# AILab-UniFI/GNN-TableExtraction

Hardware: AMD Instinct MI355X
Metric: nodes/sec (fwd+bwd node classification) on PubLayNet page graphs (higher is better)
Workload: dtype f32 (GEMM operands split exactly into 3 bf16 pieces, fp32 accumulate)

## Files before the change

### gnn-tableextraction_amd/_lib.py

```python
from __future__ import annotations

import ctypes
import os
from ctypes import POINTER, c_char_p, c_float, c_int, c_int64, c_uint64, c_void_p

_HERE = os.path.dirname(os.path.abspath(__file__))
LIB_PATH = os.environ.get("GTE_LIB_PATH") or os.path.join(_HERE, "libgte_hip.so")

SIGNATURES = {
    "gte_version": (c_int, []),
    "gte_last_error": (c_char_p, []),
    "gte_device_info": (c_int, [c_void_p, c_void_p, c_void_p, c_void_p, c_int]),
    "gte_spmm_csr": (c_int, [c_void_p, c_void_p, c_void_p, c_void_p, c_int64, c_void_p, c_int64,
                             c_int64, c_int64, c_int, c_int, c_void_p]),
    "gte_spmm_csr_accumulate": (c_int, [c_void_p, c_void_p, c_void_p, c_void_p, c_int64, c_void_p, c_int64,
                                        c_int64, c_int64, c_int, c_int, c_void_p]),
    "gte_spmm_csr_edge_workspace_bytes": (c_int64, [c_int64, c_int64]),
    "gte_spmm_csr_edge": (c_int, [c_void_p, c_void_p, c_void_p, c_void_p, c_int64, c_void_p, c_int64, c_int64, c_int64, c_int64, c_int,
                                  c_void_p, c_int64, c_void_p]),
    "gte_spmm_tile_rows": (c_int, []),
    "gte_spmm_csr_tiled": (c_int, [c_void_p, c_void_p, c_void_p, c_void_p, c_void_p, c_void_p, c_void_p, c_int64,
                                   c_void_p, c_int64, c_int64, c_int64, c_int, c_int, c_void_p]),
    "gte_coo_to_csr_workspace_bytes": (c_int64, [c_int64, c_int64]),
    "gte_coo_to_csr": (c_int, [c_void_p, c_void_p, c_void_p, c_void_p, c_int64, c_int64,
                               c_void_p, c_void_p, c_void_p, c_void_p, c_void_p, c_int64, c_void_p]),
    "gte_batch_csr": (c_int, [c_void_p, c_int64] + [c_void_p] * 10 + [c_int64, c_int64, c_void_p]),
    "gte_cast_bf16": (c_int, [c_void_p, c_int64, c_void_p, c_int64, c_int64, c_int64, c_int, c_void_p]),
    "gte_gemm_bf16_nt": (c_int, [c_void_p, c_int64, c_void_p, c_int64, c_void_p, c_int64, c_int64, c_int64, c_int64, c_void_p]),
    "gte_knn_max_k": (c_int, []),
    "gte_knn_max_page_nodes": (c_int, []),
    "gte_knn_select": (c_int, [c_void_p, c_void_p, c_void_p, c_int64, c_int64, c_int64, c_int, c_int, c_void_p, c_void_p]),
    "gte_visibility_select": (c_int, [c_void_p, c_void_p, c_void_p, c_int64, c_int64, c_int64, c_int, c_void_p, c_void_p]),
    "gte_knn_csr_workspace_bytes": (c_int64, [c_int64]),
    "gte_knn_csr": (c_int, [c_void_p, c_void_p, c_void_p, c_int64, c_int, c_int, c_int, c_void_p, c_void_p, c_void_p, c_void_p,
                            c_int64, c_void_p]),
    "gte_island_mask": (c_int, [c_void_p, c_void_p, c_void_p, c_int64, c_int, c_int, c_void_p, c_void_p, c_int64, c_void_p]),
    "gte_batch_assemble": (c_int, [c_void_p, c_int64, c_void_p, c_void_p, c_void_p, c_void_p, c_void_p, c_int64, c_int64,
                                   c_void_p, c_void_p, c_void_p, c_int64, c_void_p]),
    "gte_batch_assemble_rows": (c_int, [c_void_p, c_int64, c_void_p, c_void_p, c_void_p, c_void_p, c_void_p, c_int64, c_int64,
                                        c_void_p, c_void_p, c_void_p, c_int64, c_void_p, c_int64, c_int64, c_void_p]),
    "gte_batch_rows": (c_int, [c_void_p, c_int64, c_void_p, c_void_p, c_void_p, c_int64, c_void_p, c_int64, c_int64,
                               c_int64, c_void_p]),
    "gte_edge_weights_workspace_bytes": (c_int64, [c_int64, c_int64]),
    "gte_edge_weights_bbox": (c_int, [c_void_p, c_void_p, c_void_p, c_void_p, c_int64, c_int64, c_void_p, c_void_p,
                                      c_int64, c_void_p]),
    "gte_bbox_features": (c_int, [c_void_p, c_void_p, c_void_p, c_int64, c_int64, c_void_p]),
    "gte_inv_degree": (c_int, [c_void_p, c_void_p, c_int64, c_void_p]),
    "gte_sage_linear_fwd": (c_int, [c_void_p, c_int64, c_int64, c_void_p, c_int64, c_int64,
                                    c_void_p, c_int64, c_void_p, c_void_p, c_void_p, c_float, c_int,
                                    c_void_p, c_int64, c_void_p, c_void_p, c_int64, c_int64, c_int64, c_void_p]),
    "gte_sage_linear_fwd_fuses_ln": (c_int, [c_int64, c_int64]),
    "gte_sage_linear_fwd_p3": (c_int, [c_void_p, c_int64, c_int64, c_void_p, c_int64, c_int64,
                                       c_void_p, c_int64, c_void_p, c_void_p, c_void_p, c_float, c_int,
                                       c_void_p, c_int64, c_void_p, c_void_p, c_int64, c_void_p, c_int64, c_int64, c_int64, c_void_p]),
    "gte_sage_linear_dw_workspace_bytes": (c_int64, [c_int64, c_int64, c_int64, c_int64]),
    "gte_sage_linear_dw": (c_int, [c_void_p, c_int64, c_void_p, c_int64, c_int64, c_void_p, c_int64, c_int64, c_void_p,
                                   c_int64, c_int64, c_int64, c_void_p, c_int64, c_void_p]),
    "gte_spmm_csr_accumulate_ln_supported": (c_int, [c_int64]),
    "gte_spmm_csr_accumulate_ln": (c_int, [c_void_p, c_void_p, c_void_p, c_void_p, c_int64, c_void_p, c_int64, c_int64, c_int64,
                                           c_int, c_void_p, c_void_p, c_float, c_int, c_void_p, c_int64, c_void_p, c_void_p]),
    "gte_gemm_tail_workspace_bytes": (c_int64, []),
    "gte_gemm_set_tail_workspace": (c_int, [c_void_p, c_int64]),
    "gte_gemm_set_mode": (c_int, [c_int]),
    "gte_gemm_get_mode": (c_int, []),
    "gte_gemm_set_thread_mode": (c_int, [c_int]),
    "gte_p3_row_bytes": (c_int64, [c_int64]),
    "gte_p3_from_f32": (c_int, [c_void_p, c_int64, c_int64, c_int64, c_int, c_void_p, c_int64, c_void_p]),
    "gte_p3_to_f32": (c_int, [c_void_p, c_int64, c_int64, c_int64, c_void_p, c_int64, c_void_p]),
    "gte_p3_from_f32_batch": (c_int, [c_void_p, c_int, c_void_p]),
    "gte_spmm_csr_p3": (c_int, [c_void_p, c_void_p, c_void_p, c_void_p, c_int64, c_void_p, c_int64, c_int64, c_int64, c_int, c_void_p]),
    "gte_spmm_csr_accumulate_ln_p3": (c_int, [c_void_p, c_void_p, c_void_p, c_void_p, c_int64, c_void_p, c_int64, c_int64, c_int64,
                                              c_int, c_void_p, c_void_p, c_float, c_int, c_void_p, c_int64, c_void_p, c_int64,
                                              c_void_p, c_void_p]),
    "gte_ln_relu_bwd_p3": (c_int, [c_void_p, c_int64, c_void_p, c_int64, c_void_p, c_void_p, c_void_p, c_int,
                                   c_void_p, c_int64, c_void_p, c_int64, c_void_p, c_void_p, c_void_p, c_int64, c_int64,
                                   c_void_p, c_int64, c_void_p]),
    "gte_sage_smallk_bwd_supported": (c_int, [c_int64, c_int64]),
    "gte_sage_smallk_bwd_workspace_bytes": (c_int64, [c_int64, c_int64, c_int64]),
    "gte_sage_smallk_bwd": (c_int, [c_void_p, c_int64, c_void_p, c_int64, c_int64, c_void_p, c_int64, c_int64, c_void_p, c_int64,
                                    c_void_p, c_void_p, c_void_p, c_void_p, c_int, c_void_p, c_int64, c_void_p, c_void_p, c_void_p,
                                    c_int64, c_int64, c_void_p, c_int64, c_void_p]),
    "gte_gemm_p3_nt": (c_int, [c_void_p, c_int64, c_int64, c_void_p, c_int64, c_int64, c_void_p, c_int64, c_void_p, c_int64,
                               c_void_p, c_int64, c_int64, c_int64, c_int, c_int, c_void_p]),
    "gte_sage_narrow_bwd_ln_p3": (c_int, [c_void_p, c_int64, c_void_p, c_int64, c_void_p, c_int64, c_int64, c_void_p, c_int64, c_int64,
                                          c_void_p, c_int64, c_void_p, c_int64, c_void_p, c_int64, c_void_p, c_int64, c_void_p, c_int64,
                                          c_void_p, c_float, c_void_p, c_void_p, c_int64, c_void_p, c_void_p, c_void_p, c_int,
                                          c_void_p, c_void_p, c_void_p, c_void_p, c_int64, c_void_p]),
    "gte_sage_narrow_pad_supported": (c_int, [c_int64, c_int64, c_int64]),
    "gte_sage_narrow_fwd_pad": (c_int, [c_void_p, c_int64, c_int64, c_int64, c_void_p, c_int64, c_void_p, c_int64, c_void_p, c_int64,
                                        c_void_p, c_int64, c_int64, c_void_p]),
    "gte_sage_narrow_bwd_ln_p3_pad": (c_int, [c_void_p, c_int64, c_void_p, c_int64, c_void_p, c_int64, c_int64, c_int64, c_void_p, c_int64,
                                              c_int64, c_void_p, c_int64, c_void_p, c_int64, c_void_p, c_int64, c_void_p, c_int64, c_void_p,
                                              c_int64, c_void_p, c_float, c_void_p, c_void_p, c_int64, c_void_p, c_void_p, c_void_p, c_int,
                                              c_void_p, c_void_p, c_void_p, c_void_p, c_int64, c_void_p]),
    "gte_gemm_p3_nt_ln_bwd_supported": (c_int, [c_int64]),
    "gte_gemm_p3_nt_ln_bwd_workspace_bytes": (c_int64, [c_int64, c_int64]),
    "gte_gemm_p3_nt_ln_bwd": (c_int, [c_void_p, c_int64, c_int64, c_void_p, c_int64, c_int64, c_void_p, c_int64, c_void_p, c_int64,
                                      c_void_p, c_void_p, c_void_p, c_int, c_void_p, c_int64, c_void_p, c_int64, c_void_p, c_void_p,
                                      c_void_p, c_int64, c_int64, c_void_p, c_int64, c_void_p]),
    "gte_gemm_p3_nt_smallk_bwd_supported": (c_int, [c_int64, c_int64]),
    "gte_gemm_p3_nt_smallk_bwd_workspace_bytes": (c_int64, [c_int64, c_int64, c_int64]),
    "gte_gemm_p3_nt_smallk_bwd": (c_int, [c_void_p, c_int64, c_int64, c_void_p, c_int64, c_int64, c_void_p, c_int64, c_void_p, c_int64,
                                          c_int64, c_void_p, c_int64, c_int64, c_void_p, c_int64, c_void_p, c_void_p, c_void_p, c_void_p,
                                          c_int, c_void_p, c_int64, c_void_p, c_void_p, c_void_p, c_int64, c_int64, c_void_p, c_int64,
                                          c_void_p]),
    "gte_gemm_p3_nt_rows": (c_int, [c_void_p, c_int64, c_int64, c_void_p, c_int64, c_void_p, c_int64, c_void_p, c_int64,
                                    c_void_p, c_int64, c_int64, c_int64, c_int, c_int, c_void_p]),
    "gte_gemm_p3_tn_rows": (c_int, [c_void_p, c_int64, c_void_p, c_int64, c_void_p, c_int64, c_void_p, c_int64, c_int64, c_void_p,
                                    c_int64, c_int64, c_int64, c_int64, c_void_p, c_int64, c_void_p]),
    "gte_gemm_p3_nt_rows2": (c_int, [c_void_p, c_int64, c_void_p, c_int64, c_int64, c_void_p, c_int64, c_void_p, c_int64, c_void_p,
                                     c_int64, c_void_p, c_int64, c_int64, c_int64, c_int, c_int, c_void_p]),
    "gte_gemm_p3_tn_rows2": (c_int, [c_void_p, c_int64, c_void_p, c_int64, c_void_p, c_int64, c_void_p, c_int64, c_int64, c_void_p,
                                     c_int64, c_int64, c_int64, c_int64, c_void_p, c_int64, c_void_p]),
    "gte_gemm_p3_nt_ln_fwd_supported": (c_int, [c_int64]),
    "gte_gemm_p3_nt_ln_fwd": (c_int, [c_void_p, c_int64, c_int64, c_void_p, c_int64, c_int64, c_void_p, c_int64, c_void_p, c_void_p,
                                      c_void_p, c_float, c_int, c_void_p, c_int64, c_void_p, c_int64, c_void_p, c_int64, c_void_p,
                                      c_int64, c_int64, c_void_p]),
    "gte_gemm_p3_nt_rows2_ln_fwd": (c_int, [c_void_p, c_int64, c_void_p, c_int64, c_int64, c_void_p, c_int64, c_void_p, c_int64, c_void_p,
                                            c_void_p, c_void_p, c_float, c_int, c_void_p, c_int64, c_void_p, c_int64, c_void_p, c_int64,
                                            c_void_p, c_int64, c_int64, c_void_p]),
    "gte_gemm_p3_set_rows64": (c_int, [c_int]),
    "gte_gemm_p3_nt_plan": (c_int, [c_int64, c_int64, c_int64, c_int64, c_int, c_int, c_int, ctypes.POINTER(c_int)]),
    "gte_gemm_p3_set_nt_cfg": (c_int, [c_int]),
    "gte_gemm_p3_set_ln_rows": (c_int, [c_int]),
    "gte_batch_assemble_defer": (c_int, [c_int]),
    "gte_head_dlq_finish_workspace_bytes": (c_int64, [c_int64]),
    "gte_head_dlq_finish": (c_int, [c_void_p, c_void_p, c_void_p, c_void_p, c_int64, c_int64, c_int64, c_void_p, c_float, c_void_p,
                                    c_void_p, c_int64, c_void_p, c_void_p, c_int64, c_void_p]),
    "gte_gemm_p3_tn_workspace_bytes": (c_int64, [c_int64, c_int64, c_int64, c_int64]),
    "gte_gemm_p3_tn": (c_int, [c_void_p, c_int64, c_void_p, c_int64, c_void_p, c_int64, c_void_p, c_int64, c_int64, c_void_p,
                               c_int64, c_int64, c_int64, c_int64, c_void_p, c_int64, c_void_p]),
    "gte_adam_ticket_bytes": (c_int64, []),
    "gte_gcnsage_step": (c_int, [c_void_p, c_int, POINTER(c_int), c_void_p]),
    "gte_gcnsage_step_wide_layers": (c_int, [c_void_p]),
    "gte_gcnsage_forward": (c_int, [c_void_p, c_void_p]),
    "gte_fold_defer_begin": (c_int, [c_void_p]),
    "gte_fold_defer_flush": (c_int, []),
    "gte_fold_defer_flush_adam": (c_int, [c_void_p, c_void_p, c_void_p, c_void_p, c_int64, c_void_p, c_void_p, c_void_p, POINTER(c_int)]),
    "gte_fold_defer_flush_adam_images": (c_int, [c_void_p, c_void_p, c_void_p, c_void_p, c_int64, c_void_p, c_void_p, c_void_p, c_void_p,
                                                 c_int, POINTER(c_int)]),
    "gte_sage_transform_fwd": (c_int, [c_void_p, c_int64, c_int64, c_void_p, c_int64, c_void_p, c_int64, c_void_p, c_int64,
                                       c_int64, c_void_p]),
    "gte_sage_qform_dw_workspace_bytes": (c_int64, [c_int64, c_int64, c_int64]),
    "gte_sage_qform_dw": (c_int, [c_void_p, c_int64, c_void_p, c_int64, c_void_p, c_int64, c_int64, c_void_p, c_int64,
                                  c_int64, c_int64, c_void_p, c_int64, c_void_p]),
    "gte_sage_qform_dx": (c_int, [c_void_p, c_int64, c_void_p, c_int64, c_void_p, c_int64, c_int64, c_int64, c_void_p,
                                  c_int64, c_int64, c_void_p]),
    "gte_sage_narrow_supported": (c_int, [c_int64, c_int64]),
    "gte_sage_narrow_fwd": (c_int, [c_void_p, c_int64, c_int64, c_void_p, c_int64, c_void_p, c_int64, c_void_p, c_int64,
                                    c_void_p, c_int64, c_int64, c_void_p]),
    "gte_sage_narrow_fwd_ln_supported": (c_int, [c_int64, c_int64]),
    "gte_sage_narrow_fwd_ln": (c_int, [c_void_p, c_int64, c_int64, c_void_p, c_void_p, c_float, c_int, c_void_p, c_int64, c_void_p,
                                       c_void_p, c_int64, c_void_p, c_int64, c_void_p, c_int64, c_void_p, c_int64, c_int64,
                                       c_void_p]),
    "gte_sage_narrow_bwd_workspace_bytes": (c_int64, [c_int64, c_int64, c_int64]),
    "gte_sage_narrow_bwd": (c_int, [c_void_p, c_int64, c_void_p, c_int64, c_void_p, c_int64, c_int64, c_void_p, c_int64,
                                    c_int64, c_void_p, c_int64, c_void_p, c_int64, c_void_p, c_int64, c_void_p, c_int64,
                                    c_void_p]),
    "gte_head_supported": (c_int, [c_int64, c_int64]),
    "gte_head_agg_ce_workspace_bytes": (c_int64, [c_int64]),
    "gte_head_agg_ce": (c_int, [c_void_p, c_void_p, c_void_p, c_void_p, c_int64, c_void_p, c_int64, c_void_p, c_int, c_void_p,
                                c_int64, c_int64, c_int, c_void_p, c_int64, c_void_p, c_int64, c_void_p]),
    "gte_sage_narrow_bwd_ce": (c_int, [c_void_p, c_int64, c_void_p, c_int64, c_void_p, c_int64, c_int64, c_void_p, c_int64,
                                       c_int64, c_void_p, c_int64, c_void_p, c_int64, c_void_p, c_int64, c_void_p, c_int64,
                                       c_void_p, c_float, c_void_p, c_void_p]),
    "gte_sage_narrow_bwd_ln_workspace_bytes": (c_int64, [c_int64, c_int64]),
    "gte_ln_relu_fwd": (c_int, [c_void_p, c_int64, c_void_p, c_void_p, c_float, c_int, c_void_p, c_int64, c_void_p,
                                c_int64, c_int64, c_void_p]),
    "gte_ln_relu_fwd_p3": (c_int, [c_void_p, c_int64, c_void_p, c_void_p, c_float, c_int, c_void_p, c_int64, c_void_p, c_int64,
                                   c_void_p, c_int64, c_int64, c_void_p]),
    "gte_colsum_workspace_bytes": (c_int64, [c_int64, c_int64]),
    "gte_colsum": (c_int, [c_void_p, c_int64, c_int64, c_int64, c_void_p, c_void_p, c_int64, c_void_p]),
    "gte_ln_relu_bwd_workspace_bytes": (c_int64, [c_int64, c_int64]),
    "gte_ln_relu_bwd": (c_int, [c_void_p, c_int64, c_void_p, c_int64, c_void_p, c_void_p, c_void_p, c_int,
                                c_void_p, c_int64, c_void_p, c_void_p, c_void_p, c_int64, c_int64,
                                c_void_p, c_int64, c_void_p]),
    "gte_gemm_workspace_bytes": (c_int64, [c_int64, c_int64, c_int64]),
    "gte_gemm_f32": (c_int, [c_int, c_int, c_int64, c_int64, c_int64, c_void_p, c_int64, c_void_p, c_int64,
                             c_void_p, c_int64, c_int, c_void_p, c_int64, c_void_p]),
    "gte_gat_scores": (c_int, [c_void_p, c_int64, c_void_p, c_void_p, c_void_p, c_void_p, c_void_p, c_int64, c_int64,
                               c_int, c_int, c_void_p]),
    "gte_gat_aggregate_fwd": (c_int, [c_void_p, c_void_p, c_void_p, c_int64, c_int, c_void_p, c_void_p, c_void_p,
                                      c_void_p, c_int64, c_void_p, c_void_p, c_int64, c_int, c_int, c_void_p]),
    "gte_gat_aggregate_fwd_ex": (c_int, [c_void_p, c_void_p, c_void_p, c_int64, c_int, c_void_p, c_void_p, c_void_p,
                                         c_void_p, c_int64, c_void_p, c_void_p, c_int64, c_int, c_int, c_int, c_void_p, c_int64,
                                         c_void_p, c_int64, c_void_p, c_void_p]),
    "gte_gat_dout_prepare": (c_int, [c_void_p, c_int64, c_void_p, c_int64, c_void_p, c_int64, c_int64, c_int, c_int, c_int,
                                     c_void_p]),
    "gte_gat_bwd_workspace_bytes": (c_int64, [c_int64, c_int, c_int]),
    "gte_gat_aggregate_bwd": (c_int, [c_void_p] * 6 + [c_int64, c_int, c_void_p, c_int64] + [c_void_p] * 7 +
                              [c_int64] + [c_void_p] * 4 + [c_int64] + [c_void_p] * 3 + [c_int64, c_int, c_int,
                                                                                        c_void_p, c_int64, c_void_p]),
    "gte_gat_aggregate_bwd_ex": (c_int, [c_void_p] * 6 + [c_int64, c_int, c_void_p, c_int64] + [c_void_p] * 7 +
                                 [c_int64, c_void_p, c_int64, c_int, c_void_p, c_int64] + [c_void_p] * 4 + [c_int64] +
                                 [c_void_p] * 3 + [c_int64, c_int, c_int, c_void_p, c_int64, c_void_p]),
    "gte_weighted_ce_workspace_bytes": (c_int64, [c_int64]),
    "gte_weighted_ce": (c_int, [c_void_p, c_int64, c_void_p, c_int, c_void_p, c_int64, c_int, c_float,
                                c_void_p, c_int64, c_void_p, c_void_p, c_int64, c_void_p]),
    "gte_adam_step": (c_int, [c_void_p, c_void_p, c_void_p, c_void_p, c_int64, c_float, c_float, c_float,
                              c_float, c_float, c_int64, c_float, c_void_p]),
    "gte_adam_step_dev": (c_int, [c_void_p, c_void_p, c_void_p, c_void_p, c_int64, c_void_p, c_void_p, c_void_p, c_void_p]),
    "gte_adam_step_dev_images": (c_int, [c_void_p, c_void_p, c_void_p, c_void_p, c_int64, c_void_p, c_void_p, c_void_p, c_void_p,
                                         c_int, c_void_p, c_void_p]),
    "gte_dropout_set_wide": (c_int, [c_int]),
    "gte_dropout_get_wide": (c_int, []),
    "gte_dropout_mask": (c_int, [c_float, c_uint64, c_int, c_int64, c_int, c_int64, c_int64, c_void_p, c_int64, c_void_p]),
    "gte_dropout_mask_host": (c_int, [c_float, c_uint64, c_int, c_int64, c_int, c_int64, c_int64, c_void_p, c_int64]),
    "gte_spmm_dropout_p3": (c_int, [c_void_p, c_void_p, c_void_p, c_void_p, c_int64, c_void_p, c_int64, c_void_p, c_int64, c_int,
                                    c_float, c_uint64, c_int, c_void_p, c_int, c_void_p, c_int64, c_void_p, c_int64, c_int64, c_int64,
                                    c_void_p]),
    "gte_spmm_dropout_bwd": (c_int, [c_void_p, c_void_p, c_void_p, c_void_p, c_int64, c_int64, c_float, c_uint64, c_int, c_void_p,
                                     c_int, c_void_p, c_int64, c_int64, c_int64, c_void_p]),
}

class P3Desc(ctypes.Structure):
    _fields_ = [("src", c_void_p), ("ld", c_int64), ("rows", c_int64), ("cols", c_int64), ("transpose", c_int),
                ("dst", c_void_p), ("ldp", c_int64)]
# ... 91 lines not shown
```

### gnn-tableextraction_amd/csrc/gemm_p3.hip

```cpp
#include "gte_common.h"
#include "gemm_p3_host.h"
#include "p3.h"
#include "smallk_step.h"

#include <stdlib.h>
#include <type_traits>
#include <utility>

namespace {

typedef __bf16 bf16x8 __attribute__((ext_vector_type(8)));
typedef float f32x16 __attribute__((ext_vector_type(16)));
typedef short s16x4 __attribute__((ext_vector_type(4)));
typedef __attribute__((address_space(3))) void* lds_ptr_t;
constexpr unsigned SRD_FLAGS = 0x00020000u;

template <typename F, int... I>
__device__ __forceinline__ void static_for_impl(F&& f, std::integer_sequence<int, I...>) {
    (f(std::integral_constant<int, I>{}), ...);
}
template <int N, typename F>
__device__ __forceinline__ void static_for(F&& f) {
    static_for_impl(static_cast<F&&>(f), std::make_integer_sequence<int, N>{});
}

struct P3Gemm {
    const char* A1; const char* A2; const char* B;
    const char* An2; const char* Bn2;
    long long lda1, lda2, ldb, ldan2, ldbn2;
    long long bsa1, bsa2, bsb, bsan2, bsbn2;
    int KB1, KB2;
    int M, N, K;
    int Nseg;
    float* C; long long ldc;
    const float* bias; int bias_cols;
    int relu, accumulate;
    int splits, stages_per_split;
    float* slab;
    const int* rowsA; const int* rowsB; long long res_bytes;
    int rows64;
    int rows_both; long long res_bytes2;
    int wide_c;
    const float* ln_z; long long ln_ldz; const float* ln_stats; const float* ln_gamma; const float* ln_beta; int ln_relu;
    float* ln_dz; long long ln_lddz; char* ln_dzp3; long long ln_ldp3; float* ln_part;
    float* lnf_y; long long lnf_ldy; char* lnf_yp3; long long lnf_ldp; float* lnf_stats; float lnf_eps;
    const float* sk_x; long long sk_ldx; int sk_k1; const float* sk_ahn; long long sk_ldahn; int sk_k2;
    const float* sk_W; long long sk_ldw; const float* sk_bias; float* sk_part_dw;
};


__device__ __forceinline__ void dma16(__amdgpu_buffer_rsrc_t srd, char* dst, int voffset) {
    __builtin_amdgcn_raw_ptr_buffer_load_lds(srd, (lds_ptr_t)dst, 16, voffset, 0, 0, 0);
}

typedef const void __attribute__((address_space(1))) * global_cptr_t;
__device__ __forceinline__ void gdma16(const char* src, char* dst) {
    __builtin_amdgcn_global_load_lds((global_cptr_t)src, (lds_ptr_t)dst, 16, 0, 0);
}

struct __attribute__((packed, aligned(4))) f4u { float x, y, z, w; };

template <int TM, int TN>
struct Frags { bf16x8 a[3][TM], b[3][TN]; };

template <int TM, int TN>
__device__ __forceinline__ void products(f32x16 (&acc)[TM][TN], const Frags<TM, TN>& f) {
#ifndef P3_ORDER
#define P3_ORDER 0
#endif
#if P3_ORDER == 0
    constexpr int PA[6] = {0, 2, 1, 0, 1, 0};
    constexpr int PB[6] = {2, 0, 1, 1, 0, 0};
#pragma unroll
    for (int q = 0; q < 6; ++q)
#pragma unroll
        for (int a = 0; a < TM; ++a)
#pragma unroll
            for (int b = 0; b < TN; ++b)
                acc[a][b] = __builtin_amdgcn_mfma_f32_32x32x16_bf16(f.a[PA[q]][a], f.b[PB[q]][b], acc[a][b], 0, 0, 0);
#elif P3_ORDER == 1
    constexpr int PA[6] = {2, 1, 1, 0, 0, 0};
    constexpr int PB[6] = {0, 1, 0, 2, 1, 0};
#pragma unroll
    for (int a = 0; a < TM; ++a)
#pragma unroll
        for (int q = 0; q < 6; ++q)
#pragma unroll
            for (int b = 0; b < TN; ++b)
                acc[a][b] = __builtin_amdgcn_mfma_f32_32x32x16_bf16(f.a[PA[q]][a], f.b[PB[q]][b], acc[a][b], 0, 0, 0);
#else
    constexpr int PA[6] = {0, 1, 0, 2, 1, 0};
    constexpr int PB[6] = {2, 1, 1, 0, 0, 0};
#pragma unroll
    for (int b = 0; b < TN; ++b)
#pragma unroll
        for (int q = 0; q < 6; ++q)
#pragma unroll
            for (int a = 0; a < TM; ++a)
                acc[a][b] = __builtin_amdgcn_mfma_f32_32x32x16_bf16(f.a[PA[q]][a], f.b[PB[q]][b], acc[a][b], 0, 0, 0);
#endif
}

template <int TM, int TN>
__device__ __forceinline__ void keep_frags(const Frags<TM, TN>& f) {
#pragma unroll
    for (int pl = 0; pl < 3; ++pl) {
#pragma unroll
        for (int a = 0; a < TM; ++a) asm volatile("" ::"v"(f.a[pl][a]));
#pragma unroll
        for (int b = 0; b < TN; ++b) asm volatile("" ::"v"(f.b[pl][b]));
    }
}

template <int TM, int TN>
__device__ __forceinline__ void store_tile(const f32x16 (&acc)[TM][TN], float* outp, long long ldo, int M, int cols_total,
                                           int row0, int col0, int cols_valid_end, const float* bias, int bias_cols, int relu,
                                           int accumulate, int lane, int wide) {
    const int col_l = lane & 31, hrow = (lane >> 5) * 4;
    const int rb = wide ? row0 : 0;
    const int rows_w = wide ? min(M - rb, TM * 32) : M;
    const __amdgpu_buffer_rsrc_t c_srd = __builtin_amdgcn_make_buffer_rsrc(
        outp + (long long)rb * ldo, 0, rows_w > 0 ? (int)(((long long)(rows_w - 1) * ldo + cols_total) * 4) : 0, SRD_FLAGS);
    const int ld4 = (int)ldo * 4;
    const bool post = accumulate || relu;
#pragma unroll
    for (int b = 0; b < TN; ++b) {
        const int col = col0 + b * 32 + col_l;
// ... 467 lines not shown
#pragma unroll
            for (int k = 0; k < PD; ++k) request_row(k, k);
        }
        for (int sl = 0; sl < WM; ++sl) {
            asm volatile("s_barrier" ::: "memory");
            if (wm == sl) {
#pragma unroll
                for (int b = 0; b < TN; ++b)
#pragma unroll
                    for (int a = 0; a < TM; ++a)
#pragma unroll
                        for (int r = 0; r < 16; ++r)
                            tile[(a * 32 + hrow + (r & 3) + 8 * (r >> 2)) * LDT + wn * (TN * 32) + b * 32 + col_l] = acc[a][b][r];
            }
            asm volatile("s_waitcnt lgkmcnt(0)\n\ts_barrier" ::: "memory");
            const int row_base = m0 + sl * SR;
            constexpr int ROUNDS = (SR + RF * NW - 1) / (RF * NW);
#pragma unroll
            for (int rd = 0; rd < ROUNDS; ++rd) {
                const int rl = wave + rd * RF * NW;
                if (rl >= SR) break;
                float gy[RF][4], zz[RF][4], mean[RF], rstd[RF];
                bool rok[RF];
#pragma unroll
                for (int u = 0; u < RF; ++u) {
                    const int rloc = rl + u * NW, rg = row_base + rloc;
                    rok[u] = rloc < SR && rg < M;
                    const int rc = rok[u] ? rg : min(row_base, M - 1);
                    float4 a = make_float4(0.f, 0.f, 0.f, 0.f), bz = a;
                    if (okc) {
                        if (rok[u]) a = *reinterpret_cast<const float4*>(tile + rloc * LDT + j4);
                        if constexpr (!PRE) {
                            const f4u zt = *reinterpret_cast<const f4u*>(p.ln_z + (long long)rc * p.ln_ldz + j4);
                            bz = make_float4(zt.x, zt.y, zt.z, zt.w);
                        }
                    }
                    gy[u][0] = a.x; gy[u][1] = a.y; gy[u][2] = a.z; gy[u][3] = a.w;
                    if constexpr (PRE) {
                        const int k = rd * RF + u;
                        const int e_ = (k < RPW ? k : 0) % PD;
#pragma unroll
                        for (int e = 0; e < 4; ++e) zz[u][e] = zpre[e_][e];
                        mean[u] = mpre[e_]; rstd[u] = rpre[e_];
                        if (k + PD < RPW) request_row(e_, k + PD);
                    } else {
                        zz[u][0] = bz.x; zz[u][1] = bz.y; zz[u][2] = bz.z; zz[u][3] = bz.w;
                        mean[u] = p.ln_stats[rc]; rstd[u] = p.ln_stats[M + rc];
                    }
                }
                float dd[RF][4];
#pragma unroll
                for (int u = 0; u < RF; ++u) {
#pragma unroll
                    for (int e = 0; e < 4; ++e) dd[u][e] = 0.f;
                    if (!rok[u]) continue;
                    const long long rg = row_base + rl + u * NW;
                    float xh[4], g[4];
                    float a = 0.f, b = 0.f;
                    if constexpr (MSK) gte_ln_bwd_pre4m(gy[u], zz[u], mean[u], rstd[u], gam, bet, oke, p.ln_relu, xh, g, a, b);
                    else gte_ln_bwd_pre4(gy[u], zz[u], mean[u], rstd[u], gam, bet, okc, p.ln_relu, xh, g, a, b);
                    const float c1 = gte_group_sum<64>(a) * inv_n, c2 = gte_group_sum<64>(b) * inv_n;
                    if constexpr (MSK) gte_ln_bwd_post4m(g, xh, gam, rstd[u], c1, c2, oke, dd[u], s_dg, s_db, s_dbias);
                    else gte_ln_bwd_post4(g, xh, gam, rstd[u], c1, c2, okc, dd[u], s_dg, s_db, s_dbias);
                    if (okc && p.ln_dz) {
                        f4u o; o.x = dd[u][0]; o.y = dd[u][1]; o.z = dd[u][2]; o.w = dd[u][3];
                        *reinterpret_cast<f4u*>(p.ln_dz + rg * p.ln_lddz + j4) = o;
                    }
                }
                if (p.ln_dzp3) {
                    const bool odd = lane & 1;
                    const int col0 = 4 * (lane & ~1);
                    const bool im8 = MSK ? col0 < ((n + 15) & ~15) : col0 < n;
#pragma unroll
                    for (int u = 0; u < RF; u += 2) {
                        float x[8];
#pragma unroll
                        for (int e = 0; e < 4; ++e) {
                            const float got = gte_quad_swap1(odd ? dd[u][e] : dd[u + 1][e]);
                            x[e] = odd ? got : dd[u][e];
                            x[4 + e] = odd ? dd[u + 1][e] : got;
                        }
                        if (im8 && rok[odd ? u + 1 : u])
                            p3::store8(p.ln_dzp3 + (long long)(row_base + rl + (odd ? u + 1 : u) * NW) * p.ln_ldp3, col0, x);
                    }
                }
            }
        }
        asm volatile("s_waitcnt lgkmcnt(0)\n\ts_barrier" ::: "memory");
        float* red = reinterpret_cast<float*>(lds);
#pragma unroll
        for (int e = 0; e < 4; ++e) {
            red[(wave * 3 + 0) * 256 + j4 + e] = s_dg[e];
            red[(wave * 3 + 1) * 256 + j4 + e] = s_db[e];
            red[(wave * 3 + 2) * 256 + j4 + e] = s_dbias[e];
        }
        asm volatile("s_waitcnt lgkmcnt(0)\n\ts_barrier" ::: "memory");
        float* pp = p.ln_part + (long long)lb * 3 * n;
        for (int i = tid; i < 3 * 256; i += NW * 64) {
            const int q = i >> 8, j = i & 255;
            float v = 0.f;
#pragma unroll
            for (int w = 0; w < NW; ++w) v += red[(w * 3 + q) * 256 + j];
            if (j < n) pp[q * n + j] = v;
        }
    }
}

template <int WM, int WN, int TM, int TN, int NL, int LNB = 0, bool BIG = false>
__global__ void __launch_bounds__((WM * WN + NL) * 64, (WM * WN + NL + 3) / 4)
gemm_p3_nt_lw_kernel(const P3Gemm p) {
    constexpr int NW = WM * WN, NBUF = 3;
    constexpr int BM = WM * TM * 32, BN = WN * TN * 32;
    constexpr int A_INST = BM * 96 / 1024, B_INST = BN * 96 / 1024, N_INST = A_INST + B_INST;
    constexpr int A_BYTES = BM * 96;
    constexpr int NI = (N_INST + NL - 1) / NL;
    constexpr int STAGE = NI * NL * 1024;
    extern __shared__ __attribute__((aligned(16))) char lds[];

    const int tid = threadIdx.x, lane = tid & 63;
    const int wave = __builtin_amdgcn_readfirstlane(tid >> 6);

    const int tiles_n = (p.N + BN - 1) / BN;
    const unsigned lb = gte_xcd_remap(blockIdx.x, gridDim.x);
    const int tm = (int)(lb / (unsigned)tiles_n), tn = (int)(lb % (unsigned)tiles_n);
    const int m0 = tm * BM, n0 = tn * BN;
    const int T = p.KB1 + p.KB2;

    if (wave >= NW) {
        const int lw = wave - NW;
        const int rowsA = min(BM, p.M - m0), rowsB = min(BN, p.N - n0);
        const int lda1 = (int)p.lda1, lda2 = (int)(p.A2 ? p.lda2 : p.lda1), ldb = (int)p.ldb;
        const char* baseA1 = p.rowsA ? p.A1 : p.A1 + (long long)m0 * p.lda1;
        const char* baseA2 = p.A2 ? (p.rows_both ? p.A2 : p.A2 + (long long)m0 * p.lda2) : baseA1;
        const int recA1 = p.rowsA ? (int)(unsigned)p.res_bytes : rowsA * (int)p.lda1;
        const int recA2 = p.rows_both ? (int)(unsigned)p.res_bytes2 : rowsA * lda2;
        const char* baseB = p.B + (long long)n0 * p.ldb;
        const long long bsa1 = p.bsa1, bsa2 = p.A2 ? p.bsa2 : p.bsa1, bsb = p.bsb;
        constexpr int OOB = 0x7f000000;
        int vo1[NI], vo2[NI], isb[NI];
        static_for<NI>([&](auto I) {
            constexpr int i = decltype(I)::value;
            const int ii = i * NL + lw;
            const bool b = ii >= A_INST;
            const int s = (b ? ii - A_INST : ii) * 64 + lane, row = s / 6, part = s - row * 6, sp = part ^ ((row >> 3) & 1);
            isb[i] = b ? 1 : 0;
            vo1[i] = ii >= N_INST ? OOB : row * (b ? ldb : lda1) + sp * 16;
            vo2[i] = ii >= N_INST ? OOB : row * (b ? ldb : lda2) + sp * 16;
            if (p.rowsA && !b && ii < N_INST) {
                const int rr = row < rowsA ? p.rowsA[m0 + row] : -1;
                vo1[i] = rr < 0 ? (int)0xfffffff0u : (int)((unsigned)rr * (unsigned)lda1 + (unsigned)(sp * 16));
                if (p.rows_both) vo2[i] = rr < 0 ? (int)0xfffffff0u : (int)((unsigned)rr * (unsigned)lda2 + (unsigned)(sp * 16));
            }
        });
        const int KB1 = p.KB1;
        const char* ap[NI];
        long long ap2d[NI];
        if constexpr (BIG)
            static_for<NI>([&](auto I) {
                constexpr int i = decltype(I)::value;
                const int ii = i * NL + lw;
                const int s = ii * 64 + lane, row = s / 6, part = s - row * 6, sp = part ^ ((row >> 3) & 1);
                const int rr = (ii < A_INST) ? p.rowsA[m0 + (row < rowsA ? row : 0)] : 0;
                ap[i] = p.A1 + (long long)rr * p.lda1 + sp * 16;
                ap2d[i] = p.rows_both ? (long long)(reinterpret_cast<uintptr_t>(p.A2) + (unsigned long long)((long long)rr * p.lda2 + sp * 16)) -
                                            (long long)reinterpret_cast<uintptr_t>(ap[i]) : 0;
            });
// ... 188 lines not shown
    bf16x8 bq[4][3];
    auto load_b = [&](bf16x8 (&dst)[3], int t, bool valid) {
        const __amdgpu_buffer_rsrc_t sb = __builtin_amdgcn_make_buffer_rsrc(const_cast<char*>(baseB + (long long)min(t, T - 1) * bsb), 0,
                                                                            valid ? rowsB * 96 : 0, SRD_FLAGS);
        static_for<3>([&](auto PL) {
            constexpr int pl = decltype(PL)::value;
            dst[pl] = __builtin_bit_cast(bf16x8, __builtin_amdgcn_raw_buffer_load_b128(sb, b_vo + pl * 32, 0, 0));
        });
    };
    f32x16 acc[TM][1];
#pragma unroll
    for (int a = 0; a < TM; ++a)
#pragma unroll
        for (int e = 0; e < 16; ++e) acc[a][0][e] = 0.f;
    auto block = [&](const char* blk, const bf16x8 (&b)[3]) {
        bf16x8 fa[3][TM];
        static_for<3>([&](auto GQ) {
            constexpr int g = decltype(GQ)::value;
            constexpr int oa = g == 0 ? 0 : (g == 1 ? 2 : 1);
            static_for<TM>([&](auto A) {
                constexpr int a = decltype(A)::value;
                fa[oa][a] = *reinterpret_cast<const bf16x8*>(blk + a_rd + a * 32 * 96 + oa * 32);
            });
        });
#if P3_ABL & 8
#pragma unroll
        for (int pl = 0; pl < 3; ++pl) {
#pragma unroll
            for (int a = 0; a < TM; ++a) asm volatile("" ::"v"(fa[pl][a]));
            asm volatile("" ::"v"(b[pl]));
        }
#else
        constexpr int PA[6] = {0, 2, 1, 0, 1, 0}, PB[6] = {2, 0, 1, 1, 0, 0};
        static_for<6>([&](auto QQ) {
            constexpr int q = decltype(QQ)::value;
            static_for<TM>([&](auto A) {
                constexpr int a = decltype(A)::value;
                acc[a][0] = __builtin_amdgcn_mfma_f32_32x32x16_bf16(fa[PA[q]][a], b[PB[q]], acc[a][0], 0, 0, 0);
            });
        });
#endif
        __builtin_amdgcn_sched_barrier(0);
    };
    auto kfirst = [&](int s) { return s * SQ; };
    auto nvalid = [&](int s) { return s >= S ? 0 : min(SQ, T - s * SQ); };
    int k0 = 0, nv = nvalid(0);
    load_b(bq[0], 0, 0 < nv);
    load_b(bq[1], 1, 1 < nv);
    load_b(bq[2], 2, 2 < nv);
    asm volatile("s_barrier" ::: "memory");
#if P3_ABL & 16
    const long long c0 = __builtin_amdgcn_s_memtime(), r0 = __builtin_amdgcn_s_memrealtime();
#endif
    int rd = 0;
    for (int s = 0; s < S; ++s) {
        const char* slot = lds + rd * SLOT;
        const int k1 = kfirst(s + 1), nv1 = nvalid(s + 1);
        static_for<SQ>([&](auto J) {
            constexpr int j = decltype(J)::value;
            if constexpr (j + 3 < SQ) load_b(bq[(j + 3) & 3], k0 + j + 3, j + 3 < nv);
            else load_b(bq[(j + 3) & 3], k1 + j + 3 - SQ, j + 3 - SQ < nv1);
            block(slot + j * BLK, bq[j]);
        });
        asm volatile("s_waitcnt lgkmcnt(0)\n\ts_barrier" ::: "memory");
        rd = rd + 1 == NSLOT ? 0 : rd + 1;
        k0 = k1; nv = nv1;
    }
#if P3_ABL & 16
    if (tid == 0 && p.slab) {
        long long* st = reinterpret_cast<long long*>(p.slab) + 2 * blockIdx.x;
        st[0] = __builtin_amdgcn_s_memtime() - c0;
        st[1] = __builtin_amdgcn_s_memrealtime() - r0;
    }
#endif
#if P3_ABL & 32
    if (p.K != 12345) return;
#endif
    lw_epilogue<WM, WN, TM, TN, LNB>(acc, lds, p, m0, n0, lb, wave, lane, tid);
}

#ifndef P3_TN_ABL
#define P3_TN_ABL 0
#endif
template <int WM, int WN, int WGS, bool MAP = false, bool BIG = false>
__global__ void __launch_bounds__(WM * WN * 64, (WM * WN * WGS + 3) / 4)
gemm_p3_tn_kernel(const P3Gemm p) {
    static_assert(!BIG || MAP, "64-bit rows: the row-mapped kernel");
    static_assert(!MAP || (WM == 2 && WN == 2), "row map: the 128 x 128 tile");
    constexpr int NW = WM * WN, TM = 2, TN = 2;
    constexpr int BM = WM * 64, BN = WN * 64, NBA = BM / 16, NBB = BN / 16;
    constexpr int RSA = NBA * 96, RSB = NBB * 96;
    constexpr int A_BYTES = 16 * RSA, B_BYTES = 16 * RSB;
    constexpr int A_INST = A_BYTES / 1024, B_INST = B_BYTES / 1024, N_INST = A_INST + B_INST;
    constexpr int NI = (N_INST + NW - 1) / NW;
    constexpr int STAGE = NI * NW * 1024;
    static_assert((NBA & (NBA - 1)) == 0 && (NBB & (NBB - 1)) == 0 && NBA >= 8 && NBB >= 8, "blocks per row: a power of two >= 8");
    extern __shared__ __attribute__((aligned(16))) char lds[];

    const int tid = threadIdx.x, lane = tid & 63;
    const int wave = __builtin_amdgcn_readfirstlane(tid >> 6);
    const int wm = wave / WN, wn = wave % WN;

    const int nsegs = p.Nseg > 0 ? 2 : 1, seg_cols = p.Nseg > 0 ? p.Nseg : p.N;
    const int seg_tiles = (seg_cols + BN - 1) / BN, tiles_n = nsegs * seg_tiles, tiles_m = (p.M + BM - 1) / BM;
    const unsigned ntile = (unsigned)(tiles_m * tiles_n);
    const unsigned lu = gte_xcd_remap(blockIdx.x, gridDim.x);
    const int split = (int)(lu / ntile);
    const unsigned lb = lu % ntile;
    const int tm = (int)(lb / (unsigned)tiles_n), tn = (int)(lb % (unsigned)tiles_n);
    const int nseg = tn / seg_tiles;
    const int m0 = tm * BM, n0 = (tn % seg_tiles) * BN;
    const char* Am = (nseg && p.An2) ? p.An2 : p.A1;
    const char* Bm = (nseg && p.Bn2) ? p.Bn2 : p.B;
    const int lda = (int)((nseg && p.An2) ? p.ldan2 : p.lda1), ldb = (int)((nseg && p.Bn2) ? p.ldbn2 : p.ldb);

    const int total_stages = (p.K + 15) / 16;
    const int st_begin = split * p.stages_per_split;
    const int st_end = min(total_stages, st_begin + p.stages_per_split);
    const int coa = (m0 >> 4) * 96, cob = (n0 >> 4) * 96;

    constexpr int OOB = 0x7f000000;
    int vo[NI], isb[NI], kb[NI], vc[NI];
    static_for<NI>([&](auto I) {
        constexpr int i = decltype(I)::value;
        const int ii = i * NW + wave;
        const bool b = ii >= A_INST;
        const int nb = b ? NBB : NBA;
        const int s = (b ? ii - A_INST : ii) * 64 + lane, k = s / (6 * nb), w = s - k * (6 * nb), jb = w / 6, part = w - jb * 6;
        const int fb = (jb - 2 * (k & 3)) & (nb - 1);
        isb[i] = (b && ii < N_INST) ? 1 : 0;
        vo[i] = ii >= N_INST ? OOB : k * (b ? ldb : lda) + fb * 96 + part * 16;
        kb[i] = k;
        vc[i] = fb * 96 + part * 16;
    });
    const int* rmap = p.rowsB;
    int rid[3] = {0, 0, 0};
    if constexpr (MAP)
        if (st_begin < st_end) {
            rid[0] = rmap[st_begin * 16 + kb[3]];
            rid[1] = rmap[st_begin * 16 + kb[4]];
            rid[2] = rmap[st_begin * 16 + kb[5]];
        }
    auto issue = [&](int st, char* buf) {
        const int k0 = st * 16;
        const int rows = st < st_end ? min(16, p.K - k0) : 0;
        const __amdgpu_buffer_rsrc_t sa =
            __builtin_amdgcn_make_buffer_rsrc(const_cast<char*>(Am + (long long)k0 * lda + coa), 0, max(rows * lda - coa, 0), SRD_FLAGS);
        if constexpr (MAP) {
            {
                static_assert(!MAP || (A_INST == 12 && NI == 6), "row map: 128 x 128 tile");
                const int live = rows > 0 ? 1 : 0;
                const __amdgpu_buffer_rsrc_t sb = __builtin_amdgcn_make_buffer_rsrc(
                    const_cast<char*>(Bm + cob), 0, (int)(unsigned)max(p.res_bytes - cob, 0ll) * live, SRD_FLAGS);
                asm volatile("s_waitcnt vmcnt(6)" : "+v"(rid[0]), "+v"(rid[1]), "+v"(rid[2])::"memory");
                if constexpr (BIG) {
                    const char* g0 = Bm + cob + (long long)rid[0] * ldb + vc[3];
                    const char* g1 = Bm + cob + (long long)rid[1] * ldb + vc[4];
                    const char* g2 = Bm + cob + (long long)rid[2] * ldb + vc[5];
                    const int kn_ = st + 1 < st_end ? k0 + 16 : 0;
                    const int* r0 = rmap + kn_ + kb[3];
                    const int* r1 = rmap + kn_ + kb[4];
                    const int* r2 = rmap + kn_ + kb[5];
                    asm volatile("global_load_dword %0, %3, off\n\tglobal_load_dword %1, %4, off\n\tglobal_load_dword %2, %5, off"
                                 : "=&v"(rid[0]), "=&v"(rid[1]), "=&v"(rid[2])
                                 : "v"(r0), "v"(r1), "v"(r2), "v"(g0), "v"(g1), "v"(g2)
                                 : "memory");
                    dma16(sa, buf + (0 * NW + wave) * 1024, vo[0]);
                    dma16(sa, buf + (1 * NW + wave) * 1024, vo[1]);
                    dma16(sa, buf + (2 * NW + wave) * 1024, vo[2]);
                    gdma16(g0, buf + (3 * NW + wave) * 1024);
                    gdma16(g1, buf + (4 * NW + wave) * 1024);
                    gdma16(g2, buf + (5 * NW + wave) * 1024);
                    return;
                }
                const int o0 = (int)((unsigned)rid[0] * (unsigned)ldb + (unsigned)vc[3]);
                const int o1 = (int)((unsigned)rid[1] * (unsigned)ldb + (unsigned)vc[4]);
                const int o2 = (int)((unsigned)rid[2] * (unsigned)ldb + (unsigned)vc[5]);
                const int kn = st + 1 < st_end ? k0 + 16 : 0;
                const int* q0 = rmap + kn + kb[3];
                const int* q1 = rmap + kn + kb[4];
                const int* q2 = rmap + kn + kb[5];
                asm volatile("global_load_dword %0, %3, off\n\tglobal_load_dword %1, %4, off\n\tglobal_load_dword %2, %5, off"
                             : "=&v"(rid[0]), "=&v"(rid[1]), "=&v"(rid[2])
                             : "v"(q0), "v"(q1), "v"(q2), "v"(o0), "v"(o1), "v"(o2)
                             : "memory");
                dma16(sa, buf + (0 * NW + wave) * 1024, vo[0]);
                dma16(sa, buf + (1 * NW + wave) * 1024, vo[1]);
                dma16(sa, buf + (2 * NW + wave) * 1024, vo[2]);
                dma16(sb, buf + (3 * NW + wave) * 1024, o0);
                dma16(sb, buf + (4 * NW + wave) * 1024, o1);
                dma16(sb, buf + (5 * NW + wave) * 1024, o2);
                return;
            }
        }
        const __amdgpu_buffer_rsrc_t sb =
            __builtin_amdgcn_make_buffer_rsrc(const_cast<char*>(Bm + (long long)k0 * ldb + cob), 0, max(rows * ldb - cob, 0), SRD_FLAGS);
        static_for<NI>([&](auto I) {
            constexpr int i = decltype(I)::value;
            dma16(isb[i] ? sb : sa, buf + (i * NW + wave) * 1024, vo[i]);
        });
    };

    const int h = lane >> 5, g = (lane >> 4) & 1, q = (lane >> 2) & 3, pp = lane & 3;
    int a_rd[TM], b_rd[TN];
#pragma unroll
    for (int a = 0; a < TM; ++a) a_rd[a] = (8 * h + q) * RSA + ((2 * (wm * TM + a) + g + 2 * q) & (NBA - 1)) * 96 + pp * 8;
#pragma unroll
    for (int b = 0; b < TN; ++b) b_rd[b] = A_BYTES + (8 * h + q) * RSB + ((2 * (wn * TN + b) + g + 2 * q) & (NBB - 1)) * 96 + pp * 8;
    using F = Frags<TM, TN>;
    typedef char __attribute__((address_space(3))) * lds_char;
    const unsigned lds_base = (unsigned)(__SIZE_TYPE__)(lds_char)lds;
    static_assert(TM == 2 && TN == 2, "the waits below name four fragments per plane pair");
    auto read_pair = [&](F& f, unsigned sbase, auto PA_, auto PB_) {
        static_for<TM + TN>([&](auto X) {
            constexpr int x = decltype(X)::value;
            constexpr bool isb = x >= TM;
            constexpr int pc = isb ? decltype(PB_)::value : decltype(PA_)::value;
            constexpr int lo_off = pc * 32, hi_off = pc * 32 + 4 * (isb ? RSB : RSA);
            const unsigned at = sbase + (unsigned)(isb ? b_rd[isb ? x - TM : 0] : a_rd[isb ? 0 : x]);
            s16x4 lo, hi;
            asm volatile("ds_read_b64_tr_b16 %0, %1 offset:%2" : "=v"(lo) : "v"(at), "n"(lo_off) : "memory");
            asm volatile("ds_read_b64_tr_b16 %0, %1 offset:%2" : "=v"(hi) : "v"(at), "n"(hi_off) : "memory");
            const bf16x8 v = __builtin_bit_cast(bf16x8, __builtin_shufflevector(lo, hi, 0, 1, 2, 3, 4, 5, 6, 7));
            if constexpr (isb) f.b[pc][isb ? x - TM : 0] = v; else f.a[pc][isb ? 0 : x] = v;
        });
    };
    auto wait_pair = [&](F& f, auto N_, auto PA_, auto PB_) {
        constexpr int pa = decltype(PA_)::value, pb = decltype(PB_)::value;
        if constexpr (decltype(N_)::value == 8)
            asm volatile("s_waitcnt lgkmcnt(8)" : "+v"(f.a[pa][0]), "+v"(f.a[pa][1]), "+v"(f.b[pb][0]), "+v"(f.b[pb][1])::"memory");
        else
            asm volatile("s_waitcnt lgkmcnt(0)" : "+v"(f.a[pa][0]), "+v"(f.a[pa][1]), "+v"(f.b[pb][0]), "+v"(f.b[pb][1])::"memory");
    };
    f32x16 acc[TM][TN];
    auto mfma_pair = [&](const F& f, auto PA_, auto PB_) {
        constexpr int pa = decltype(PA_)::value, pb = decltype(PB_)::value;
#pragma unroll
        for (int a = 0; a < TM; ++a)
#pragma unroll
            for (int b = 0; b < TN; ++b) acc[a][b] = __builtin_amdgcn_mfma_f32_32x32x16_bf16(f.a[pa][a], f.b[pb][b], acc[a][b], 0, 0, 0);
    };
    using I0 = std::integral_constant<int, 0>; using I1 = std::integral_constant<int, 1>; using I2 = std::integral_constant<int, 2>;
    using I8 = std::integral_constant<int, 8>;
    auto stage_products = [&](int slot) {
        const unsigned sbase = lds_base + (unsigned)slot * STAGE;
        F f;
#if P3_TN_ABL & 4
        static_for<3>([&](auto PC) { f.a[PC.value][0] = f.a[PC.value][1] = f.b[PC.value][0] = f.b[PC.value][1] = bf16x8{}; });
        asm volatile("" : "+v"(f.a[0][0]), "+v"(f.b[0][0]));
#else
        read_pair(f, sbase, I0{}, I2{});
        read_pair(f, sbase, I2{}, I0{});
        wait_pair(f, I8{}, I0{}, I2{});
#endif
        __builtin_amdgcn_sched_barrier(0);
#if !(P3_TN_ABL & 2)
        mfma_pair(f, I0{}, I2{});
#endif
        __builtin_amdgcn_sched_barrier(0);
#if !(P3_TN_ABL & 4)
        read_pair(f, sbase, I1{}, I1{});
        wait_pair(f, I8{}, I2{}, I0{});
#endif
        __builtin_amdgcn_sched_barrier(0);
#if !(P3_TN_ABL & 2)
        mfma_pair(f, I2{}, I0{});
#endif
        __builtin_amdgcn_sched_barrier(0);
#if !(P3_TN_ABL & 4)
        wait_pair(f, I0{}, I1{}, I1{});
#endif
        __builtin_amdgcn_sched_barrier(0);
#if !(P3_TN_ABL & 2)
        mfma_pair(f, I1{}, I1{});
        mfma_pair(f, I0{}, I1{});
        mfma_pair(f, I1{}, I0{});
        mfma_pair(f, I0{}, I0{});
#else
        asm volatile("" ::"v"(f.a[0][0]), "v"(f.a[1][1]), "v"(f.a[2][0]), "v"(f.b[0][0]), "v"(f.b[1][1]), "v"(f.b[2][1]));
#endif
        __builtin_amdgcn_sched_barrier(0);
    };

#pragma unroll
    for (int a = 0; a < TM; ++a)
#pragma unroll
        for (int b = 0; b < TN; ++b)
#pragma unroll
            for (int e = 0; e < 16; ++e) acc[a][b][e] = 0.f;

    constexpr int NBUF = 3;
    int next = st_begin, wr = 0;
#pragma unroll
    for (int d = 0; d < NBUF - 1; ++d) {
        issue(next, lds + wr * STAGE);
        ++next;
        wr = wr + 1 == NBUF ? 0 : wr + 1;
    }
    wait_dma_barrier<(NBUF - 2) * NI>();
    int rd = 0;
    for (int st = st_begin; st < st_end; ++st) {
#if !(P3_TN_ABL & 1)
        issue(next, lds + wr * STAGE);
#endif
        ++next;
        wr = wr + 1 == NBUF ? 0 : wr + 1;
        stage_products(rd);
        wait_dma_barrier<(NBUF - 2) * NI>();
        rd = rd + 1 == NBUF ? 0 : rd + 1;
    }
    float* outp = p.splits > 1 ? p.slab + (long long)split * p.M * p.N : p.C;
    const long long ldo = p.splits > 1 ? p.N : p.ldc;
    const int cbase = nseg * seg_cols;
#if P3_TN_ABL & 8
    if (p.K == 12345)
#endif
    store_tile<TM, TN>(acc, outp, ldo, p.M, p.N, m0 + wm * TM * 32, cbase + n0 + wn * TN * 32, cbase + seg_cols, nullptr, 0,
                       p.splits > 1 ? 0 : p.relu, p.splits > 1 ? 0 : p.accumulate, lane, 0);
}

__global__ void __launch_bounds__(256)
p3_from_f32_kernel(const float* __restrict__ src, long long ld, int rows, int cols, int transpose, char* __restrict__ dst,
                   long long ldp, long long bsp) {
    const int hb = (int)((cols + 7) / 8);
    const int hbt = (int)p3::blocks(cols) * 2;
    const long long idx = (long long)blockIdx.x * 256 + threadIdx.x;
    if (idx >= (long long)rows * hbt) return;
    const int r = (int)(idx / hbt), j = (int)(idx - (long long)r * hbt);
    float x[8];
#pragma unroll
    for (int e = 0; e < 8; ++e) {
        const int c = j * 8 + e;
        x[e] = 0.f;
        if (j < hb && c < cols) x[e] = transpose ? src[(long long)c * ld + r] : src[(long long)r * ld + c];
    }
    p3::store8(dst + (long long)r * ldp + (long long)(j >> 1) * bsp, (j & 1) * 8, x);
}

constexpr int kMaxP3Batch = 16;
struct P3BatchArgs { gte_p3_desc d[kMaxP3Batch]; };
__global__ void __launch_bounds__(256)
p3_from_f32_batch_kernel(const P3BatchArgs a) {
    const gte_p3_desc d = a.d[blockIdx.y];
    const long long ldp = d.ldp < 0 ? 96 : d.ldp, bsp = d.ldp < 0 ? -d.ldp : 96;
    const int hb = (int)((d.cols + 7) / 8), hbt = (int)p3::blocks(d.cols) * 2;
    for (long long idx = (long long)blockIdx.x * 256 + threadIdx.x; idx < (long long)d.rows * hbt; idx += (long long)gridDim.x * 256) {
        const int r = (int)(idx / hbt), j = (int)(idx - (long long)r * hbt);
        float x[8];
#pragma unroll
        for (int e = 0; e < 8; ++e) {
            const long long c = j * 8 + e;
            x[e] = 0.f;
            if (j < hb && c < d.cols) x[e] = d.transpose ? d.src[c * d.ld + r] : d.src[(long long)r * d.ld + c];
        }
        p3::store8(reinterpret_cast<char*>(d.dst) + (long long)r * ldp + (long long)(j >> 1) * bsp, (j & 1) * 8, x);
    }
}

__global__ void __launch_bounds__(256)
p3_to_f32_kernel(const char* __restrict__ src, long long ldp, long long bsp, int rows, int cols, float* __restrict__ dst, long long ld) {
    const long long idx = (long long)blockIdx.x * 256 + threadIdx.x;
    if (idx >= (long long)rows * cols) return;
    const int r = (int)(idx / cols), c = (int)(idx - (long long)r * cols);
    dst[(long long)r * ld + c] = p3::load1(src + (long long)r * ldp + (long long)(c >> 4) * bsp, c & 15);
}

struct TnPlan { int splits, stages_per_split, splits_bound; };
TnPlan tn_plan(int64_t M, int64_t N, int64_t Nseg, int64_t K) {
    const int cus = gte::device_props().cus;
    const int64_t bm = 128, slots = 2 * cus;
    const int64_t tiles = gte::ceil_div(M, bm) * (Nseg > 0 ? 2 * gte::ceil_div(Nseg, 128) : gte::ceil_div(N, 128));
    const int64_t stages = gte::ceil_div(K > 0 ? K : 1, 16);
    int64_t splits = slots / tiles;
    static const int forced = GTE_MEASURE_INT("GTE_P3_TN_SPLITS", 0);
    if (forced > 0) splits = forced;
    static const int min_stages = GTE_MEASURE_INT("GTE_P3_TN_MIN_STAGES", 8);
    if (splits > stages / min_stages) splits = stages / min_stages;
    if (splits < 1) splits = 1;
    TnPlan pl;
    pl.splits_bound = (int)splits;
    pl.stages_per_split = (int)gte::ceil_div(stages, splits);
    pl.splits = (int)gte::ceil_div(stages, pl.stages_per_split);
    return pl;
}

template <typename K>
inline void set_lds_once(bool& done, K* kernel, int bytes) {
    if (done) return;
    (void)hipFuncSetAttribute(reinterpret_cast<const void*>(kernel), hipFuncAttributeMaxDynamicSharedMemorySize, bytes);
    done = true;
}

// ... 244 lines not shown
        gte::defer_fold(part + n, 3 * n, nb, 1, (int)n, outs[1], n);
        gte::defer_fold(part + 2 * n, 3 * n, nb, 1, (int)n, outs[2], n);
        return GTE_OK;
    }
    for (int i = 0; i < 3; ++i)
        if (outs[i])
            hipLaunchKernelGGL(p3_colsum_fold_kernel, dim3((unsigned)gte::ceil_div(n, 256)), dim3(256), 0, s, part + i * n, (long long)3 * n, nb,
                               (int)n, outs[i]);
    return gte::check_launch(what);
}
}

int gte::gemm_p3_nt(const P3NtOperands& op, const float* bias, int64_t bias_cols, float* c, int64_t ldc, int64_t m, int64_t n, int relu,
                    int accumulate, void* stream, const char* name) {
    const bool wide = gte::wide_forced() || (m + 256) * ldc * 4 >= ((int64_t)1 << 31);
    NtLimits lim = {};
    lim.max_ld = 1 << 22; lim.rows_ok = true;
    lim.own_sizes = n < 0 || n > INT32_MAX || op.k1 + op.k2 > INT32_MAX;
    lim.own_null = !c; lim.own_ld = ldc < n; lim.own_stride = wide && ldc >= (1 << 20);
    P3Gemm p = {};
    const int rc = nt_prepare(name, op, m, n, lim, p);
    if (rc != GTE_OK || p.M == 0) return rc;
    p.wide_c = wide ? 1 : 0;
    p.C = c; p.ldc = ldc; p.bias = bias; p.bias_cols = (int)bias_cols; p.relu = relu; p.accumulate = accumulate;
    return launch_nt(p, gte::as_stream(stream));
}

extern "C" int gte_gemm_p3_nt(const void* a1, int64_t lda1, int64_t k1, const void* a2, int64_t lda2, int64_t k2, const void* b,
                              int64_t ldb, const float* bias, int64_t bias_cols, float* c, int64_t ldc, int64_t m, int64_t n,
                              int relu, int accumulate, void* stream) {
    return gte::gemm_p3_nt({a1, lda1, k1, a2, lda2, k2, b, ldb, nullptr, 0}, bias, bias_cols, c, ldc, m, n, relu, accumulate, stream);
}

extern "C" int gte_gemm_p3_nt_rows(const void* a_res, int64_t ldpa, int64_t k, const int32_t* a_rows, int64_t n_res_rows, const void* b,
                                   int64_t ldpb, const float* bias, int64_t bias_cols, float* c, int64_t ldc, int64_t m, int64_t n,
                                   int relu, int accumulate, void* stream) {
    if (!a_rows) return gte::fail(GTE_ERR_INVALID_ARGUMENT, "gemm_p3_nt_rows: null row map");
    return gte::gemm_p3_nt({a_res, ldpa, k, nullptr, 0, 0, b, ldpb, a_rows, n_res_rows}, bias, bias_cols, c, ldc, m, n, relu, accumulate,
                           stream, "gemm_p3_nt_rows");
}

extern "C" int gte_gemm_p3_nt_rows2(const void* a_res, int64_t ldpa, const void* a2_res, int64_t ldpa2, int64_t k, const int32_t* a_rows,
                                    int64_t n_res_rows, const void* b, int64_t ldpb, const float* bias, int64_t bias_cols, float* c,
                                    int64_t ldc, int64_t m, int64_t n, int relu, int accumulate, void* stream) {
    if (!a_rows || !a2_res) return gte::fail(GTE_ERR_INVALID_ARGUMENT, "gemm_p3_nt_rows2: null row map / second image");
    return gte::gemm_p3_nt({a_res, ldpa, k, a2_res, ldpa2, k, b, ldpb, a_rows, n_res_rows}, bias, bias_cols, c, ldc, m, n, relu, accumulate,
                           stream, "gemm_p3_nt_rows2");
}

extern "C" int gte_gemm_p3_nt_plan(int64_t m, int64_t n, int64_t k1, int64_t k2, int weights_block_major, int epilogue, int cus,
                                   int* row_tile) {
    if (row_tile) *row_tile = 0;
    if (m <= 0 || n <= 0 || k1 <= 0 || k2 < 0 || (epilogue != 0 && epilogue != 1 && epilogue != 3 && epilogue != 4))
        return gte::fail(GTE_ERR_INVALID_ARGUMENT, "gemm_p3_nt_plan: bad arguments (epilogue: 0 plain, 1 / 3 LayerNorm backward, 4 LayerNorm forward)");
    P3Gemm p = {};
    p.M = (int)m; p.N = (int)n; p.KB1 = (int)p3::blocks(k1); p.KB2 = (int)p3::blocks(k2);
    p.bsa1 = p.bsa2 = 96;
    p.ldb = weights_block_major ? 96 : (p.KB1 + p.KB2) * 96; p.bsb = weights_block_major ? gte::round_up(n, 16) * 96 : 96;
    const NtPick k = nt_pick(p, epilogue, cus);
    const bool sq = k.family == NtFamily::sq;
    if (row_tile && n <= 256 && (epilogue != 0 || sq)) *row_tile = k.bm;
    return sq ? 1 : 0;
}

extern "C" int gte_gemm_p3_set_nt_cfg(int cfg) {
    if (cfg < -1 || cfg > 7) return gte::fail(GTE_ERR_INVALID_ARGUMENT, "gemm_p3_set_nt_cfg: -1 (chooser) or a configuration id 0 ... 7");
    g_nt_cfg = cfg;
    return GTE_OK;
}

extern "C" int gte_gemm_p3_set_ln_rows(int rows) {
    if (rows != 0 && rows != 32 && rows != 64 && rows != 96 && rows != 128)
        return gte::fail(GTE_ERR_INVALID_ARGUMENT, "gemm_p3_set_ln_rows: 0 (chooser), 32, 64, 96 or 128");
    g_ln_rows = rows;
    return GTE_OK;
}
extern "C" int gte_gemm_p3_nt_ln_bwd_supported(int64_t n) { return (n >= 1 && n <= 256) ? 1 : 0; }
extern "C" int64_t gte_gemm_p3_nt_ln_bwd_workspace_bytes(int64_t m, int64_t n) {
    if (m <= 0 || n <= 0) return 256;
    return gte::round_up(gte::ceil_div(m, 32) * 3 * n * 4, 256);
}
int gte::gemm_p3_nt_ln_bwd(const P3NtOperands& op, const float* z, int64_t ldz, const float* stats, const float* gamma, const float* beta,
                           int relu, float* dz, int64_t lddz, void* dzp3, int64_t ldp3, float* dgamma, float* dbeta, float* dbias,
                           int64_t m, int64_t n, void* workspace, int64_t workspace_bytes, void* stream) {
    const char* name = "gemm_p3_nt_ln_bwd";
    const int64_t n4 = gte::round_up(n, 4);
    NtLimits lim = {};
    lim.max_ld = 1 << 23; lim.below_2gb = true;
    lim.own_sizes = n <= 0 || op.k1 > INT32_MAX || op.k2 > INT32_MAX;
    lim.unsupported = gte_gemm_p3_nt_ln_bwd_supported(n) ? nullptr : "needs n <= 256";
    lim.own_null = !z || !stats || !gamma || !beta || (!dz && !dzp3) || !workspace;
    lim.own_ld = ldz < n4 || (dz && lddz < n4) || (dzp3 && (ldp3 < p3::row_bytes(n) || ldp3 % 16 != 0));
    P3Gemm p = {};
    int rc = nt_prepare(name, op, m, n, lim, p);
    if (rc != GTE_OK || p.M == 0) return rc;
    const int64_t need = gte_gemm_p3_nt_ln_bwd_workspace_bytes(m, n);
    if (workspace_bytes < need)
        return gte::fail(GTE_ERR_WORKSPACE_TOO_SMALL, "%s: needs %lld workspace bytes, got %lld", name, (long long)need, (long long)workspace_bytes);
    p.ln_z = z; p.ln_ldz = ldz; p.ln_stats = stats; p.ln_gamma = gamma; p.ln_beta = beta; p.ln_relu = relu;
    p.ln_dz = dz; p.ln_lddz = lddz; p.ln_dzp3 = reinterpret_cast<char*>(dzp3); p.ln_ldp3 = ldp3;
    p.ln_part = reinterpret_cast<float*>(workspace);
    hipStream_t s = gte::as_stream(stream);
    const NtPick k = nt_pick(p, n % 16 == 0 ? 1 : 3);
    if (n % 16 == 0) launch_one_column<1>(p, k, s); else launch_one_column<3>(p, k, s);
    rc = gte::check_launch(name);
    if (rc != GTE_OK) return rc;
    return fold_ln_partials("gemm_p3_nt_ln_bwd fold", p.ln_part, n, (int)gte::ceil_div(m, k.bm), dgamma, dbeta, dbias, s);
}
extern "C" int gte_gemm_p3_nt_ln_bwd(const void* a1, int64_t lda1, int64_t k1, const void* a2, int64_t lda2, int64_t k2, const void* b,
                                     int64_t ldb, const float* z, int64_t ldz, const float* stats, const float* gamma,
                                     const float* beta, int relu, float* dz, int64_t lddz, void* dzp3, int64_t ldp3, float* dgamma,
                                     float* dbeta, float* dbias, int64_t m, int64_t n, void* workspace, int64_t workspace_bytes,
                                     void* stream) {
    return gte::gemm_p3_nt_ln_bwd({a1, lda1, k1, a2, lda2, k2, b, ldb, nullptr, 0}, z, ldz, stats, gamma, beta, relu, dz, lddz, dzp3, ldp3,
                                  dgamma, dbeta, dbias, m, n, workspace, workspace_bytes, stream);
}

int gte::gemm_p3_nt_ln_fwd(const P3NtOperands& op, const float* bias, const float* gamma, const float* beta, float eps, int relu, float* z,
                           int64_t ldz, float* y, int64_t ldy, void* yp3, int64_t ldyp3, float* stats, int64_t m, int64_t n, void* stream,
                           const char* name) {
    const int64_t n4 = gte::round_up(n, 4);
    NtLimits lim = {};
    lim.max_ld = 1 << 22; lim.rows_ok = true;
    lim.own_sizes = n <= 0 || n > 256 || op.k1 > INT32_MAX || op.k2 > INT32_MAX;
    lim.own_null = !z || !gamma || !beta || (!y && !yp3);
    lim.own_ld = ldz < n4 || (y && ldy < n4) || (yp3 && (ldyp3 < p3::row_bytes(n) || ldyp3 % 16 != 0));
    P3Gemm p = {};
    const int rc = nt_prepare(name, op, m, n, lim, p);
    if (rc != GTE_OK || p.M == 0) return rc;
    p.C = z; p.ldc = ldz; p.bias = bias;
    p.ln_gamma = gamma; p.ln_beta = beta; p.ln_relu = relu;
    p.lnf_y = y; p.lnf_ldy = ldy; p.lnf_yp3 = reinterpret_cast<char*>(yp3); p.lnf_ldp = ldyp3; p.lnf_stats = stats; p.lnf_eps = eps;
    launch_one_column<4>(p, nt_pick(p, 4), gte::as_stream(stream));
    return gte::check_launch("gemm_p3_nt_ln_fwd");
}
extern "C" int gte_gemm_p3_nt_ln_fwd_supported(int64_t n) { return (n >= 1 && n <= 256) ? 1 : 0; }
extern "C" int gte_gemm_p3_nt_ln_fwd(const void* a1, int64_t lda1, int64_t k1, const void* a2, int64_t lda2, int64_t k2, const void* b,
                                     int64_t ldb, const float* bias, const float* gamma, const float* beta, float eps, int relu, float* z,
                                     int64_t ldz, float* y, int64_t ldy, void* yp3, int64_t ldyp3, float* stats, int64_t m, int64_t n,
                                     void* stream) {
    return gte::gemm_p3_nt_ln_fwd({a1, lda1, k1, a2, lda2, k2, b, ldb, nullptr, 0}, bias, gamma, beta, eps, relu, z, ldz, y, ldy, yp3, ldyp3,
                                  stats, m, n, stream);
}
extern "C" int gte_gemm_p3_nt_rows2_ln_fwd(const void* a_res, int64_t ldpa, const void* a2_res, int64_t ldpa2, int64_t k,
                                           const int32_t* a_rows, int64_t n_res_rows, const void* b, int64_t ldb, const float* bias,
                                           const float* gamma, const float* beta, float eps, int relu, float* z, int64_t ldz, float* y,
                                           int64_t ldy, void* yp3, int64_t ldyp3, float* stats, int64_t m, int64_t n, void* stream) {
    if (!a_rows || !a2_res) return gte::fail(GTE_ERR_INVALID_ARGUMENT, "gemm_p3_nt_rows2_ln_fwd: null row map / second image");
    return gte::gemm_p3_nt_ln_fwd({a_res, ldpa, k, a2_res, ldpa2, k, b, ldb, a_rows, n_res_rows}, bias, gamma, beta, eps, relu, z, ldz, y, ldy,
                                  yp3, ldyp3, stats, m, n, stream, "gemm_p3_nt_rows2_ln_fwd");
}

extern "C" int gte_gemm_p3_nt_smallk_bwd_supported(int64_t k_total, int64_t n) {
    return (n >= 4 && n <= 256 && n % 4 == 0 && k_total >= 1 && k_total <= 28) ? 1 : 0;
}
extern "C" int64_t gte_gemm_p3_nt_smallk_bwd_workspace_bytes(int64_t m, int64_t k_total, int64_t n) {
    if (m <= 0 || n <= 0 || k_total <= 0) return 256;
    return gte::round_up(gte::ceil_div(m, 128) * n * (k_total + 3) * 4, 256);
}
int gte::gemm_p3_nt_smallk_bwd(const P3NtOperands& op, const float* x, int64_t ldx, int64_t k1, const float* ahn, int64_t ldahn, int64_t k2,
                               const float* W, int64_t ldw, const float* bias, const float* gamma, const float* beta, const float* stats,
                               int relu, float* dW, int64_t lddw, float* dbias, float* dgamma, float* dbeta, int64_t m, int64_t n,
                               void* workspace, int64_t workspace_bytes, void* stream) {
    const char* name = "gemm_p3_nt_smallk_bwd";
    const int64_t K = k1 + k2;
    NtLimits lim = {};
    lim.max_ld = 1 << 23; lim.below_2gb = true;
    lim.own_sizes = n <= 0 || k1 <= 0 || k2 < 0 || op.k1 > INT32_MAX || op.k2 > INT32_MAX;
    lim.unsupported = gte_gemm_p3_nt_smallk_bwd_supported(K, n) ? nullptr : "needs n <= 256, n % 4 == 0, k1 + k2 <= 28";
    lim.own_null = !x || (k2 > 0 && !ahn) || !W || !bias || !gamma || !beta || !stats || !dW || !workspace;
    lim.own_ld = ldx < k1 || (k2 > 0 && ldahn < k2) || ldw < K || lddw < K;
    P3Gemm p = {};
    int rc = nt_prepare(name, op, m, n, lim, p);
    if (rc != GTE_OK || p.M == 0) return rc;
    const int64_t need = gte_gemm_p3_nt_smallk_bwd_workspace_bytes(m, K, n);
    if (workspace_bytes < need)
        return gte::fail(GTE_ERR_WORKSPACE_TOO_SMALL, "%s: needs %lld workspace bytes, got %lld", name, (long long)need, (long long)workspace_bytes);
    const int bm = 128;
    const int nb = (int)gte::ceil_div(m, bm);
    p.ln_stats = stats; p.ln_gamma = gamma; p.ln_beta = beta; p.ln_relu = relu;
    p.sk_x = x; p.sk_ldx = ldx; p.sk_k1 = (int)k1; p.sk_ahn = k2 > 0 ? ahn : nullptr; p.sk_ldahn = ldahn; p.sk_k2 = (int)k2;
    p.sk_W = W; p.sk_ldw = ldw; p.sk_bias = bias;
    p.sk_part_dw = reinterpret_cast<float*>(workspace);
    p.ln_part = p.sk_part_dw + (int64_t)nb * n * K;
    hipStream_t s = gte::as_stream(stream);
    constexpr int shm = 160 * 1024;
    static bool configured = false;
    set_lds_once(configured, &gemm_p3_nt_ring_kernel<2, 4, 2, 2, 3, 1, 2>, shm);
    hipLaunchKernelGGL((gemm_p3_nt_ring_kernel<2, 4, 2, 2, 3, 1, 2>), dim3((unsigned)nb), dim3(512), shm, s, p);
    rc = gte::check_launch(name);
    if (rc != GTE_OK) return rc;
    if (!gte::defer_fold(p.sk_part_dw, n * K, nb, (int)n, (int)K, dW, lddw)) {
        if (lddw != K) return gte::fail(GTE_ERR_UNSUPPORTED, "%s: outside a fold deferral dW must be packed (lddw == k1 + k2)", name);
        hipLaunchKernelGGL(p3_colsum_fold_kernel, dim3((unsigned)gte::ceil_div(n * K, 256)), dim3(256), 0, s, p.sk_part_dw, (long long)n * K,
                           nb, (int)(n * K), dW);
    }
    return fold_ln_partials("gemm_p3_nt_smallk_bwd fold", p.ln_part, n, nb, dgamma, dbeta, dbias, s);
}
extern "C" int gte_gemm_p3_nt_smallk_bwd(const void* a1, int64_t lda1, int64_t kg1, const void* a2, int64_t lda2, int64_t kg2,
                                         const void* b, int64_t ldb, const float* x, int64_t ldx, int64_t k1, const float* ahn,
                                         int64_t ldahn, int64_t k2, const float* W, int64_t ldw, const float* bias, const float* gamma,
                                         const float* beta, const float* stats, int relu, float* dW, int64_t lddw, float* dbias,
                                         float* dgamma, float* dbeta, int64_t m, int64_t n, void* workspace, int64_t workspace_bytes,
                                         void* stream) {
    return gte::gemm_p3_nt_smallk_bwd({a1, lda1, kg1, a2, lda2, kg2, b, ldb, nullptr, 0}, x, ldx, k1, ahn, ldahn, k2, W, ldw, bias, gamma, beta,
                                      stats, relu, dW, lddw, dbias, dgamma, dbeta, m, n, workspace, workspace_bytes, stream);
}

extern "C" int64_t gte_gemm_p3_tn_workspace_bytes(int64_t m, int64_t n, int64_t nseg, int64_t k) {
    if (m <= 0 || n <= 0) return 256;
    const TnPlan pl = tn_plan(m, n, nseg, k);
    return pl.splits_bound > 1 ? gte::round_up((int64_t)pl.splits_bound * m * n * 4, 256) : 256;
}

namespace {
__global__ void __launch_bounds__(256)
p3_fold_kernel(const float* __restrict__ slab, int splits, long long mn, int N, float* __restrict__ C, long long ldc) {
    const long long i = (long long)blockIdx.x * 256 + threadIdx.x;
    if (i >= mn) return;
    float s = 0.f;
    for (int k = 0; k < splits; ++k) s += slab[(long long)k * mn + i];
    const long long r = i / N;
    C[r * ldc + (i - r * N)] = s;
}
}

int gte::gemm_p3_tn(const P3TnOperands& o, float* c, int64_t ldc, int64_t m, int64_t n, int64_t k, void* workspace, int64_t workspace_bytes,
                    void* stream, const char* name) {
    const int64_t nseg = o.nseg;
    if (m <= 0 || n <= 0 || k < 0 || nseg < 0 || m > INT32_MAX || n > INT32_MAX || k > INT32_MAX || (nseg > 0 && n != 2 * nseg))
        return gte::fail(GTE_ERR_INVALID_ARGUMENT, "%s: bad sizes", name);
    if (!o.a || !o.b || !c) return gte::fail(GTE_ERR_INVALID_ARGUMENT, "%s: null pointer", name);
    const int64_t bcols = nseg > 0 ? nseg : n;
    if (o.lda < p3::row_bytes(m) || o.ldb < p3::row_bytes(bcols) || (o.a2 && o.lda2 < p3::row_bytes(m)) ||
        (o.b2 && o.ldb2 < p3::row_bytes(bcols)) || ldc < n)
        return gte::fail(GTE_ERR_INVALID_ARGUMENT, "%s: leading dimension too small", name);
    if (o.lda >= (1 << 23) || o.ldb >= (1 << 23) || o.lda2 >= (1 << 23) || o.ldb2 >= (1 << 23) || (m + 128) * n * 4 >= ((int64_t)1 << 31) ||
        (m + 128) * ldc * 4 >= ((int64_t)1 << 31))
        return gte::fail(GTE_ERR_UNSUPPORTED, "%s: row strides must be < 8 MB and the output < 2 GB", name);
    hipStream_t s = gte::as_stream(stream);
    if (k == 0) {
        for (int64_t r = 0; r < m; ++r)
            if (hipMemsetAsync(c + r * ldc, 0, (size_t)n * 4, s) != hipSuccess) return gte::fail(GTE_ERR_LAUNCH, "%s: memset failed", name);
        return GTE_OK;
    }
    const TnPlan pl = tn_plan(m, n, nseg, k);
    P3Gemm p = {};
    p.A1 = (const char*)o.a; p.lda1 = o.lda; p.An2 = (const char*)o.a2; p.ldan2 = o.lda2;
    p.B = (const char*)o.b; p.ldb = o.ldb; p.Bn2 = (const char*)o.b2; p.ldbn2 = o.ldb2;
    p.Nseg = (int)nseg; p.M = (int)m; p.N = (int)n; p.K = (int)k; p.C = c; p.ldc = ldc;
    p.splits = pl.splits; p.stages_per_split = pl.stages_per_split;
    if (o.rows) {
        if (o.b2 && o.ldb2 != o.ldb) return gte::fail(GTE_ERR_UNSUPPORTED, "%s: both resident images need the same row stride", name);
        if (o.n_res_rows <= 0) return gte::fail(GTE_ERR_INVALID_ARGUMENT, "%s: empty resident image", name);
        p.rowsB = o.rows; p.res_bytes = o.n_res_rows * o.ldb;
        p.rows64 = rows64_needed((o.n_res_rows + 1) * o.ldb);
    }
    if (pl.splits > 1) {
        const int64_t need = (int64_t)pl.splits * m * n * 4;
        if (!workspace || workspace_bytes < need)
            return gte::fail(GTE_ERR_WORKSPACE_TOO_SMALL, "%s: split-K needs %lld workspace bytes, got %lld", name, (long long)need,
                             (long long)workspace_bytes);
        p.slab = reinterpret_cast<float*>(workspace);
    }
    const int64_t tiles = gte::ceil_div(m, 128) * (nseg > 0 ? 2 * gte::ceil_div(nseg, 128) : gte::ceil_div(n, 128));
    constexpr int shm_small = 3 * 6 * 4 * 1024;
    static bool configured[3] = {};
    set_lds_once(configured[0], &gemm_p3_tn_kernel<2, 2, 2>, shm_small);
    set_lds_once(configured[1], &gemm_p3_tn_kernel<2, 2, 2, true>, shm_small);
    set_lds_once(configured[2], &gemm_p3_tn_kernel<2, 2, 2, true, true>, shm_small);
    const dim3 grid((unsigned)(tiles * pl.splits));
    if (p.rowsB && p.rows64) hipLaunchKernelGGL((gemm_p3_tn_kernel<2, 2, 2, true, true>), grid, dim3(256), shm_small, s, p);
    else if (p.rowsB) hipLaunchKernelGGL((gemm_p3_tn_kernel<2, 2, 2, true>), grid, dim3(256), shm_small, s, p);
    else hipLaunchKernelGGL((gemm_p3_tn_kernel<2, 2, 2>), grid, dim3(256), shm_small, s, p);
    int rc = gte::check_launch("gemm_p3_tn");
    if (rc != GTE_OK || pl.splits <= 1) return rc;
    const int64_t mn = m * n;
    if (gte::defer_fold(p.slab, mn, pl.splits, (int)m, (int)n, c, ldc)) return GTE_OK;
    hipLaunchKernelGGL(p3_fold_kernel, dim3((unsigned)gte::ceil_div(mn, 256)), dim3(256), 0, s, p.slab, pl.splits, (long long)mn, (int)n,
                       c, (long long)ldc);
    return gte::check_launch("gemm_p3_tn fold");
}

extern "C" int gte_gemm_p3_tn(const void* a, int64_t lda, const void* a2, int64_t lda2, const void* b, int64_t ldb, const void* b2,
                              int64_t ldb2, int64_t nseg, float* c, int64_t ldc, int64_t m, int64_t n, int64_t k, void* workspace,
                              int64_t workspace_bytes, void* stream) {
    return gte::gemm_p3_tn({a, lda, a2, lda2, b, ldb, b2, ldb2, nseg, nullptr, 0}, c, ldc, m, n, k, workspace, workspace_bytes, stream);
}

extern "C" int gte_gemm_p3_tn_rows(const void* a, int64_t ldpa, const void* a2, int64_t ldpa2, const void* b_res, int64_t ldpb,
                                   const int32_t* b_rows, int64_t n_res_rows, int64_t nseg, float* c, int64_t ldc, int64_t m, int64_t n,
                                   int64_t k, void* workspace, int64_t workspace_bytes, void* stream) {
    if (!b_rows) return gte::fail(GTE_ERR_INVALID_ARGUMENT, "gemm_p3_tn_rows: null row map");
    return gte::gemm_p3_tn({a, ldpa, a2, ldpa2, b_res, ldpb, nullptr, 0, nseg, b_rows, n_res_rows}, c, ldc, m, n, k, workspace, workspace_bytes,
                           stream, "gemm_p3_tn_rows");
}

extern "C" int gte_gemm_p3_tn_rows2(const void* a, int64_t ldpa, const void* b_res, int64_t ldpb, const void* b2_res, int64_t ldpb2,
                                    const int32_t* b_rows, int64_t n_res_rows, int64_t nseg, float* c, int64_t ldc, int64_t m, int64_t n,
                                    int64_t k, void* workspace, int64_t workspace_bytes, void* stream) {
    if (!b_rows || !b2_res || nseg <= 0) return gte::fail(GTE_ERR_INVALID_ARGUMENT, "gemm_p3_tn_rows2: null row map / second image, or nseg <= 0");
    return gte::gemm_p3_tn({a, ldpa, nullptr, 0, b_res, ldpb, b2_res, ldpb2, nseg, b_rows, n_res_rows}, c, ldc, m, n, k, workspace,
                           workspace_bytes, stream, "gemm_p3_tn_rows2");
}
```

### gnn-tableextraction_amd/csrc/gemm_p3_host.h

```cpp
#pragma once
#include <stdint.h>

namespace gte {

struct P3NtOperands {
    const void* a1; int64_t lda1, k1;
    const void* a2; int64_t lda2, k2;
    const void* b; int64_t ldb;
    const int32_t* rows; int64_t n_res_rows;
};

struct P3TnOperands {
    const void* a; int64_t lda; const void* a2; int64_t lda2;
    const void* b; int64_t ldb; const void* b2; int64_t ldb2; int64_t nseg;
    const int32_t* rows; int64_t n_res_rows;
};

int gemm_p3_nt(const P3NtOperands& op, const float* bias, int64_t bias_cols, float* c, int64_t ldc, int64_t m, int64_t n, int relu,
               int accumulate, void* stream, const char* name = "gemm_p3_nt");
int gemm_p3_nt_ln_fwd(const P3NtOperands& op, const float* bias, const float* gamma, const float* beta, float eps, int relu, float* z,
                      int64_t ldz, float* y, int64_t ldy, void* yp3, int64_t ldyp3, float* stats, int64_t m, int64_t n, void* stream,
                      const char* name = "gemm_p3_nt_ln_fwd");
int gemm_p3_nt_ln_bwd(const P3NtOperands& op, const float* z, int64_t ldz, const float* stats, const float* gamma, const float* beta,
                      int relu, float* dz, int64_t lddz, void* dzp3, int64_t ldp3, float* dgamma, float* dbeta, float* dbias, int64_t m,
                      int64_t n, void* workspace, int64_t workspace_bytes, void* stream);
int gemm_p3_nt_smallk_bwd(const P3NtOperands& op, const float* x, int64_t ldx, int64_t k1, const float* ahn, int64_t ldahn, int64_t k2,
                          const float* W, int64_t ldw, const float* bias, const float* gamma, const float* beta, const float* stats,
                          int relu, float* dW, int64_t lddw, float* dbias, float* dgamma, float* dbeta, int64_t m, int64_t n,
                          void* workspace, int64_t workspace_bytes, void* stream);
int gemm_p3_tn(const P3TnOperands& op, float* c, int64_t ldc, int64_t m, int64_t n, int64_t k, void* workspace, int64_t workspace_bytes,
               void* stream, const char* name = "gemm_p3_tn");

}
```

### gnn-tableextraction_amd/csrc/step.hip

```cpp
#include "gte_common.h"
#include "gemm_p3_host.h"

#include <stdlib.h>

namespace {

#define GTE_TRY(call)            \
    do {                         \
        const int rc_ = (call);  \
        if (rc_ != GTE_OK) return rc_; \
    } while (0)

inline int64_t ldf(const gte_step_layer& L) { return L.ldf > 0 ? L.ldf : L.fout; }
inline int64_t ld_lg(const gte_step_plan& p) { return p.ld_lg > 0 ? p.ld_lg : p.n_classes; }

bool head_gemm_fused(const gte_step_plan& p) {
    return p.out_gemm && (p.fuse_ln_dx & 4) && p.n_classes <= 16 && ld_lg(p) >= 32 && p.n_nodes > 0 &&
           p.ws_ce_bytes >= gte_head_agg_ce_workspace_bytes(p.n_nodes) && p.ws_cs_bytes >= gte_head_dlq_finish_workspace_bytes(p.n_nodes);
}


bool narrow_padded(const gte_step_plan& p) {
    return !p.out_gemm && p.out_fin % 8 != 0 && p.ld_h_out > p.out_fin && gte_sage_narrow_pad_supported(p.out_fin, p.ld_h_out, p.n_classes);
}

inline int64_t c16(int64_t v) { return (v + 15) / 16 * 16; }
bool layer_wide(const gte_step_plan& p, int i) {
    const gte_step_layer& L = p.layer[i];
    if (L.kind != GTE_LAYER_DROPOUT) return false;
    if (gte::wide_forced()) return true;
    const int64_t ld = c16(L.fout) > c16(L.fin) ? c16(L.fout) : c16(L.fin);
    return (p.n_nodes + 256) * 2 * ld * 4 >= ((int64_t)1 << 31);
}

inline bool two_images(const gte_step_layer& L) { return L.kind != GTE_LAYER_PLANES; }
inline const int32_t* rows_of(const gte_step_layer& L) { return (L.kind == GTE_LAYER_PLANES || L.kind == GTE_LAYER_CACHED) ? L.h_rows : nullptr; }
inline gte::P3NtOperands fwd_operands(const gte_step_layer& L) {
    const bool two = two_images(L);
    return {L.hp, L.ldp_h, L.fin, two ? L.ahnp : nullptr, two ? L.ldp_ahn : 0, two ? L.fin : 0, L.wimg_fwd, L.ldp_wfwd, rows_of(L), L.n_res_rows};
}
inline gte::P3TnOperands dw_operands(const gte_step_layer& L) {
    const bool two = two_images(L);
    return {L.dzp, L.ldp_o, two ? nullptr : L.qp, two ? 0 : L.ldp_o, L.hp, L.ldp_h, two ? L.ahnp : nullptr, two ? L.ldp_ahn : 0, L.fin,
            rows_of(L), L.n_res_rows};
}
inline int layer_dw(const gte_step_layer& L, int64_t n, void* st) {
    return gte::gemm_p3_tn(dw_operands(L), L.gW, 2 * L.fin, L.fout, 2 * L.fin, n, L.ws_dw, L.ws_dw_bytes, st);
}

int forward_hidden(const gte_step_plan& p, void* st, bool fwd_only = false) {
    const int64_t n = p.n_nodes;
    if (p.n_wimg_descs > 0 && !p.wimg_fresh) {
        const gte_p3_desc* d = reinterpret_cast<const gte_p3_desc*>(p.wimg_descs);
        for (int k = 0; k < p.n_wimg_descs; k += 16)
            GTE_TRY(gte_p3_from_f32_batch(d + k, p.n_wimg_descs - k < 16 ? p.n_wimg_descs - k : 16, st));
    }
    auto mark = [&](int k) {
        if (p.fwd_events && p.fwd_events[k]) (void)hipEventRecord(reinterpret_cast<hipEvent_t>(p.fwd_events[k]), gte::as_stream(st));
    };
    auto y_unread = [&](int i) {
        if (i + 1 < p.n_hidden) return p.layer[i + 1].kind == GTE_LAYER_PLANES && !p.layer[i + 1].make_hp;
        return fwd_only && p.out_gemm != 0;
    };
    for (int i = 0; i < p.n_hidden; ++i) {
        const gte_step_layer& L = p.layer[i];
        const int64_t ld = ldf(L);
        const gte::WideScope wide(layer_wide(p, i));
        if (L.kind == GTE_LAYER_SMALLK) {
            GTE_TRY(gte_spmm_csr(p.indptr, p.indices, p.w_in, L.x, L.ldx, L.ahn, L.fin, n, L.fin, GTE_F32, GTE_REDUCE_MEAN, st));
            float* zs = gte_sage_smallk_bwd_supported(2 * L.fin, L.fout) ? nullptr : L.t;
            if (L.yp)
                GTE_TRY(gte_sage_linear_fwd_p3(L.x, L.ldx, L.fin, L.ahn, L.fin, L.fin, L.W, 2 * L.fin, L.bias, L.gamma, L.beta, L.eps, L.relu,
                                               zs, L.fout, L.stats, L.y, L.fout, L.yp, L.ldp_y, n, L.fout, st));
            else
                GTE_TRY(gte_sage_linear_fwd(L.x, L.ldx, L.fin, L.ahn, L.fin, L.fin, L.W, 2 * L.fin, L.bias, L.gamma, L.beta, L.eps, L.relu, zs,
                                            L.fout, L.stats, L.y, L.fout, n, L.fout, st));
            continue;
        }
        if (two_images(L)) {
            if (L.kind == GTE_LAYER_DROPOUT) {
                GTE_TRY(gte_spmm_dropout_p3(p.indptr, p.indices, p.w_in, L.x, L.ldx, L.xp, L.ldp_x, L.h_rows, L.n_res_rows, i == 0,
                                            p.dropout_p, p.dropout_seed, p.rank, p.step_counter, i + 1, L.hp, L.ldp_h, L.ahnp,
                                            L.ldp_ahn, n, L.fin, st));
            } else if (L.kind == GTE_LAYER_AGGFIRST) {
                GTE_TRY(gte_p3_from_f32(L.x, L.ldx, n, L.fin, 0, L.hp, L.ldp_h, st));
                GTE_TRY(gte_spmm_csr_p3(p.indptr, p.indices, p.w_in, L.x, L.ldx, L.ahnp, L.ldp_ahn, n, L.fin, GTE_REDUCE_MEAN, st));
            }
            mark(2 * i);
            float* const y = (L.kind == GTE_LAYER_CACHED && L.yp && (fwd_only || y_unread(i))) ? nullptr : L.y;
            if ((p.fuse_ln_dx & 16) && gte_gemm_p3_nt_ln_fwd_supported(L.fout)) {
                GTE_TRY(gte::gemm_p3_nt_ln_fwd(fwd_operands(L), L.bias, L.gamma, L.beta, L.eps, L.relu, L.t, ld, y, ld, L.yp, L.ldp_y, L.stats, n,
                                               L.fout, st));
                mark(2 * i + 1);
                continue;
            }
            GTE_TRY(gte::gemm_p3_nt(fwd_operands(L), L.bias, L.fout, L.t, ld, n, L.fout, 0, 0, st));
            mark(2 * i + 1);
            GTE_TRY(gte_ln_relu_fwd_p3(L.t, ld, L.gamma, L.beta, L.eps, L.relu, y, ld, L.yp, L.ldp_y, L.stats, n, L.fout, st));
            continue;
        }
        if (L.make_hp) GTE_TRY(gte_p3_from_f32(L.x, L.ldx, n, L.fin, 0, L.hp, L.ldp_h, st));
        mark(2 * i);
        GTE_TRY(gte::gemm_p3_nt(fwd_operands(L), L.bias, L.fout, L.t, 2 * ld, n, 2 * ld, 0, 0, st));
        mark(2 * i + 1);
        float* const y = (L.yp && y_unread(i)) ? nullptr : L.y;
        GTE_TRY(gte_spmm_csr_accumulate_ln_p3(p.indptr, p.indices, p.w_in, L.t + ld, 2 * ld, L.t, 2 * ld, n, L.fout,
                                              GTE_REDUCE_MEAN, L.gamma, L.beta, L.eps, L.relu, y, ld, L.yp, L.ldp_y, L.stats, st));
    }
    return GTE_OK;
}

int forward_out_products(const gte_step_plan& p, void* st) {
    const int64_t n = p.n_nodes, C = p.n_classes, lg = ld_lg(p);
    if (p.out_gemm)
        return gte_gemm_p3_nt(p.hp_out, p.ldp_hout, p.out_fin, nullptr, 0, 0, p.wimg_out_fwd, p.ldp_wout_fwd, p.b_out, C, p.logits, lg, n,
                              32, 0, 0, st);
    if (narrow_padded(p))
        return gte_sage_narrow_fwd_pad(p.h_out, p.ld_h_out, p.out_fin, p.ld_h_out, p.W_out, 2 * p.out_fin, p.b_out, C, p.logits, lg, p.tn,
                                       lg, n, st);
    return gte_sage_narrow_fwd(p.h_out, p.ld_h_out, p.out_fin, p.W_out, 2 * p.out_fin, p.b_out, C, p.logits, lg, p.tn, lg, n, st);
}

int forward(const gte_step_plan& p, void* st) {
    const int64_t n = p.n_nodes;
    GTE_TRY(forward_hidden(p, st));
    const int64_t C = p.n_classes, lg = ld_lg(p);
    GTE_TRY(forward_out_products(p, st));
    if (p.out_gemm) {
        if (head_gemm_fused(p))
            return gte_head_agg_ce(p.indptr, p.indices, p.w_in, p.tn, lg, p.logits, lg, p.labels, p.labels_f32, p.class_weights, n, C,
                                   GTE_REDUCE_MEAN, p.dl, lg, p.ws_ce, p.ws_ce_bytes, st);
        GTE_TRY(gte_spmm_csr_accumulate(p.indptr, p.indices, p.w_in, p.tn, lg, p.logits, lg, n, C, GTE_F32, GTE_REDUCE_MEAN, st));
        return gte_weighted_ce(p.logits, lg, p.labels, p.labels_f32, p.class_weights, n, (int)C, p.grad_scale, p.dl, lg, p.out3, p.ws_ce,
                               p.ws_ce_bytes, st);
    }
    GTE_TRY(gte_head_agg_ce(p.indptr, p.indices, p.w_in, p.tn, lg, p.logits, lg, p.labels, p.labels_f32, p.class_weights, n, C,
                            GTE_REDUCE_MEAN, p.dl, lg, p.ce_part, p.ce_part_bytes, st));
    return GTE_OK;
}

bool smallk_in_dx(const gte_step_plan& p) {
    if (!(p.fuse_ln_dx & 8) || p.n_hidden < 2) return false;
    const gte_step_layer& B = p.layer[0];
    const gte_step_layer& L = p.layer[1];
    return B.kind == GTE_LAYER_SMALLK && L.kind == GTE_LAYER_PLANES && gte_sage_smallk_bwd_supported(2 * B.fin, B.fout) &&
           gte_gemm_p3_nt_smallk_bwd_supported(2 * B.fin, L.fin) && ldf(B) == B.fout;
}

inline const float* z_of(const gte_step_layer& L) { return L.t; }
inline int64_t ldz_of(const gte_step_layer& L) { return L.kind == GTE_LAYER_PLANES ? 2 * ldf(L) : ldf(L); }

int backward_a(const gte_step_plan& p, void* st) {
    static const bool keep_dz0 = GTE_MEASURE_INT("GTE_STEP_KEEP_DZ0", 0) != 0;
    const int64_t n = p.n_nodes, C = p.n_classes, lg = ld_lg(p);
    bool ln_done = false, smallk_done = false;
    const gte_step_layer& T = p.layer[p.n_hidden - 1];
    const gte::WideScope wide_out(layer_wide(p, p.n_hidden - 1));
    if (p.out_gemm) {
        GTE_TRY(gte_spmm_csr(p.rindptr, p.rindices, p.w_out, p.dl, lg, p.q_out, lg, n, C, GTE_F32, GTE_REDUCE_SUM, st));
        if (head_gemm_fused(p)) {
            GTE_TRY(gte_head_dlq_finish(nullptr, nullptr, nullptr, p.dl, lg, n, C, p.ws_ce, p.grad_scale, p.out3, p.dlqp, p.ldp_dlq,
                                        p.gb_out, p.ws_cs, p.ws_cs_bytes, st));
        } else {
            GTE_TRY(gte_p3_from_f32(p.dl, lg, n, 32, 0, p.dlqp, p.ldp_dlq, st));
            GTE_TRY(gte_colsum(p.dl, lg, n, C, p.gb_out, p.ws_cs, p.ws_cs_bytes, st));
        }
        GTE_TRY(gte_gemm_p3_tn(p.dlqp, p.ldp_dlq, static_cast<const char*>(p.dlqp) + 96, p.ldp_dlq, p.hp_out, p.ldp_hout, nullptr, 0,
                               p.out_fin, p.gW_out, 2 * p.out_fin, C, 2 * p.out_fin, n, p.ws_out, p.ws_out_bytes, st));
        if ((p.fuse_ln_dx & 1) && T.kind != GTE_LAYER_SMALLK && gte_gemm_p3_nt_ln_bwd_supported(p.out_fin) && T.dy == p.dh_out &&
            (n + 256) * p.ldp_dlq < ((int64_t)1 << 31) &&
            (p.out_fin % 16 == 0 || ldf(T) >= ((p.out_fin + 3) & ~(int64_t)3))) {
            GTE_TRY(gte_gemm_p3_nt_ln_bwd(p.dlqp, p.ldp_dlq, 32, nullptr, 0, 0, p.wimg_out_bwd, p.ldp_wout_bwd, z_of(T), ldz_of(T), T.stats,
                                          T.gamma, T.beta, T.relu, T.dy, ldf(T), T.dzp, T.ldp_o, T.ggamma, T.gbeta, T.gbias, n, p.out_fin,
                                          T.ws_ln, T.ws_ln_bytes, st));
            ln_done = true;
        } else {
            GTE_TRY(gte_gemm_p3_nt(p.dlqp, p.ldp_dlq, 32, nullptr, 0, 0, p.wimg_out_bwd, p.ldp_wout_bwd, nullptr, 0, p.dh_out, p.ld_h_out, n,
                                   p.out_fin, 0, 0, st));
        }
    } else if (narrow_padded(p)) {
        GTE_TRY(gte_spmm_csr(p.rindptr, p.rindices, p.w_out, p.dl, C, p.q_out, C, n, C, GTE_F32, GTE_REDUCE_SUM, st));
        GTE_TRY(gte_sage_narrow_bwd_ln_p3_pad(p.dl, C, p.q_out, C, p.h_out, p.ld_h_out, p.out_fin, p.ld_h_out, p.W_out, 2 * p.out_fin, C,
                                              p.dh_out, p.ld_h_out, T.dzp, T.ldp_o, p.gW_out, 2 * p.out_fin, p.gb_out, n, p.ws_nar,
                                              p.ws_nar_bytes, p.ce_part, p.grad_scale, p.out3, z_of(T), ldz_of(T), T.stats, T.gamma, T.beta,
                                              T.relu, T.ggamma, T.gbeta, T.gbias, T.ws_ln, T.ws_ln_bytes, st));
        ln_done = true;
    } else if ((p.fuse_ln_dx & 2) && T.kind == GTE_LAYER_PLANES && T.fout % 16 == 0 && gte_head_supported(p.out_fin, C)) {
        GTE_TRY(gte_spmm_csr(p.rindptr, p.rindices, p.w_out, p.dl, C, p.q_out, C, n, C, GTE_F32, GTE_REDUCE_SUM, st));
        GTE_TRY(gte_sage_narrow_bwd_ln_p3(p.dl, C, p.q_out, C, p.h_out, p.ld_h_out, p.out_fin, p.W_out, 2 * p.out_fin, C,
                                          p.dh_out, p.ld_h_out, T.dzp, T.ldp_o, p.gW_out, 2 * p.out_fin, p.gb_out, n, p.ws_nar, p.ws_nar_bytes,
                                          p.ce_part, p.grad_scale, p.out3, T.t, 2 * ldf(T), T.stats, T.gamma, T.beta, T.relu, T.ggamma,
                                          T.gbeta, T.gbias, T.ws_ln, T.ws_ln_bytes, st));
        ln_done = true;
    } else {
        GTE_TRY(gte_spmm_csr(p.rindptr, p.rindices, p.w_out, p.dl, C, p.q_out, C, n, C, GTE_F32, GTE_REDUCE_SUM, st));
        GTE_TRY(gte_sage_narrow_bwd_ce(p.dl, C, p.q_out, C, p.h_out, p.ld_h_out, p.out_fin, p.W_out, 2 * p.out_fin, C, p.dh_out, p.ld_h_out,
                                       p.gW_out, 2 * p.out_fin, p.gb_out, n, p.ws_nar, p.ws_nar_bytes, p.ce_part, p.grad_scale, p.out3, st));
    }
    for (int i = p.n_hidden - 1; i >= 0; --i) {
        const gte_step_layer& L = p.layer[i];
        const int64_t ld = ldf(L);
        const gte::WideScope wide(layer_wide(p, i));
        if (L.kind == GTE_LAYER_SMALLK) {
            if (smallk_done) continue;
            if (!gte_sage_smallk_bwd_supported(2 * L.fin, L.fout))
                GTE_TRY(gte_ln_relu_bwd(L.dy, L.fout, L.t, L.fout, L.stats, L.gamma, L.beta, L.relu, L.dy, L.fout, L.ggamma, L.gbeta, L.gbias, n,
                                        L.fout, L.ws_ln, L.ws_ln_bytes, st));
            continue;
        }
        if (!ln_done)
            GTE_TRY(gte_ln_relu_bwd_p3(L.dy, ld, z_of(L), ldz_of(L), L.stats, L.gamma, L.beta, L.relu, L.dy, ld, L.dzp, L.ldp_o, L.ggamma,
                                       L.gbeta, L.gbias, n, L.fout, L.ws_ln, L.ws_ln_bytes, st));
        ln_done = false;
        if (L.kind == GTE_LAYER_AGGFIRST || L.kind == GTE_LAYER_CACHED) break;
        if (L.kind == GTE_LAYER_DROPOUT) {
            if (i == 0) break;
            GTE_TRY(layer_dw(L, n, st));
            GTE_TRY(gte_gemm_p3_nt(L.dzp, L.ldp_o, L.fout, nullptr, 0, 0, L.wimg_bwd, L.ldp_wbwd, nullptr, 0, L.g, L.ldg, n, L.ldg, 0, 0, st));
            const gte_step_layer& B = p.layer[i - 1];
            GTE_TRY(gte_spmm_dropout_bwd(p.rindptr, p.rindices, p.w_out, L.g, L.ldg, L.ldg / 2, p.dropout_p, p.dropout_seed, p.rank,
                                         p.step_counter, i + 1, B.dy, ldf(B), n, L.fin, st));
            continue;
        }
        GTE_TRY(gte_spmm_csr_p3(p.rindptr, p.rindices, p.w_out, L.dy, ld, L.qp, L.ldp_o, n, L.fout, GTE_REDUCE_SUM, st));
        if (i == 0) break;
        GTE_TRY(gte_gemm_p3_tn(L.dzp, L.ldp_o, L.qp, L.ldp_o, L.hp, L.ldp_h, nullptr, 0, L.fin, L.gW, 2 * L.fin, L.fout, 2 * L.fin, n, L.ws_dw,
                               L.ws_dw_bytes, st));
        const gte_step_layer& B = p.layer[i - 1];
        if (i == 1 && smallk_in_dx(p)) {
            smallk_done = true;
            break;
        } else if ((p.fuse_ln_dx & 1) && B.kind != GTE_LAYER_SMALLK && gte_gemm_p3_nt_ln_bwd_supported(L.fin) &&
                   (L.fin % 16 == 0 || ldf(B) >= ((L.fin + 3) & ~(int64_t)3))) {
            GTE_TRY(gte_gemm_p3_nt_ln_bwd(L.dzp, L.ldp_o, L.fout, L.qp, L.ldp_o, L.fout, L.wimg_bwd, L.ldp_wbwd, z_of(B), ldz_of(B), B.stats,
                                          B.gamma, B.beta, B.relu, (B.kind == GTE_LAYER_CACHED && B.dzp && !keep_dz0) ? nullptr : B.dy, ldf(B), B.dzp, B.ldp_o,
                                          B.ggamma, B.gbeta, B.gbias, n, L.fin, B.ws_ln, B.ws_ln_bytes, st));
            ln_done = true;
        } else {
            GTE_TRY(gte_gemm_p3_nt(L.dzp, L.ldp_o, L.fout, L.qp, L.ldp_o, L.fout, L.wimg_bwd, L.ldp_wbwd, nullptr, 0, B.dy, ldf(B), n, L.fin, 0,
                                   0, st));
        }
    }
    return GTE_OK;
}

int backward_b(const gte_step_plan& p, void* st) {
    const int64_t n = p.n_nodes;
    const gte_step_layer& L = p.layer[0];
    const gte::WideScope wide(layer_wide(p, 0));
    if (smallk_in_dx(p)) {
        const gte_step_layer& U = p.layer[1];
        return gte_gemm_p3_nt_smallk_bwd(U.dzp, U.ldp_o, U.fout, U.qp, U.ldp_o, U.fout, U.wimg_bwd, U.ldp_wbwd, L.x, L.ldx, L.fin, L.ahn,
                                         L.fin, L.fin, L.W, 2 * L.fin, L.bias, L.gamma, L.beta, L.stats, L.relu, L.gW, 2 * L.fin, L.gbias,
                                         L.ggamma, L.gbeta, n, U.fin, L.ws_dw, L.ws_dw_bytes, st);
    }
    if (L.kind == GTE_LAYER_SMALLK && gte_sage_smallk_bwd_supported(2 * L.fin, L.fout))
        return gte_sage_smallk_bwd(L.dy, L.fout, L.x, L.ldx, L.fin, L.ahn, L.fin, L.fin, L.W, 2 * L.fin, L.bias, L.gamma, L.beta, L.stats,
                                   L.relu, L.gW, 2 * L.fin, L.gbias, L.ggamma, L.gbeta, n, L.fout, L.ws_dw, L.ws_dw_bytes, st);
    if (L.kind == GTE_LAYER_SMALLK)
        return gte_sage_linear_dw(L.dy, L.fout, L.x, L.ldx, L.fin, L.ahn, L.fin, L.fin, L.gW, 2 * L.fin, L.fout, n, L.ws_dw, L.ws_dw_bytes, st);
    return layer_dw(L, n, st);
}

int flush(const gte_step_plan& p, int* adam_fused) {
    if (adam_fused) *adam_fused = 0;
    if (p.param) {
        int fused = 0;
        const bool img = p.wimg_in_fold && p.n_wimg_descs > 0;
        const int rc = gte_fold_defer_flush_adam_images(p.param, p.grad, p.exp_avg, p.exp_avg_sq, p.n_param, p.hyper, p.step_counter, p.ticket,
                                                        img ? reinterpret_cast<const gte_p3_desc*>(p.wimg_descs) : nullptr,
                                                        img ? p.n_wimg_descs : 0, &fused);
        if (adam_fused) *adam_fused = fused;
        return rc;
    }
    return gte_fold_defer_flush();
}

int check_plan(const gte_step_plan& p) {
    if (p.n_hidden < 1 || p.n_hidden > 7 || p.n_nodes < 0) return gte::fail(GTE_ERR_INVALID_ARGUMENT, "gcnsage_step: bad plan");
    for (int i = 0; i < p.n_hidden; ++i) {
        const gte_step_layer& L = p.layer[i];
        if (L.kind != GTE_LAYER_PLANES && L.kind != GTE_LAYER_SMALLK && L.kind != GTE_LAYER_AGGFIRST && L.kind != GTE_LAYER_CACHED &&
            L.kind != GTE_LAYER_DROPOUT)
            return gte::fail(GTE_ERR_INVALID_ARGUMENT, "gcnsage_step: layer kind");
        if ((L.kind == GTE_LAYER_DROPOUT) != (p.dropout_p != 0.f))
            return gte::fail(GTE_ERR_INVALID_ARGUMENT, "gcnsage_step: a plan with dropout_p != 0 runs every hidden layer as GTE_LAYER_DROPOUT, "
                                                       "and only such a plan");
        if (L.kind == GTE_LAYER_DROPOUT) {
            if (!(p.dropout_p > 0.f && p.dropout_p < 1.f) || !p.step_counter || !L.hp || !L.ahnp || !L.wimg_fwd || !L.dzp)
                return gte::fail(GTE_ERR_INVALID_ARGUMENT, "gcnsage_step: a dropout layer needs 0 < dropout_p < 1, the step counter, its "
                                                           "operand / weight / dz images");
            if (i == 0 ? (!L.x == !L.xp) : (!L.x || !L.g || !L.wimg_bwd || L.ldg != 2 * ((L.fin + 15) / 16 * 16)))
                return gte::fail(GTE_ERR_INVALID_ARGUMENT, "gcnsage_step: dropout layer input (layer 0: x or xp) / G [n][2 ceil16(fin)] / "
                                                           "backward weight image");
            if (i > 0 && (!p.layer[i - 1].y || !p.layer[i - 1].dy))
                return gte::fail(GTE_ERR_INVALID_ARGUMENT, "gcnsage_step: the layer below a dropout layer writes y as fp32 rows");
        }
        if (L.kind == GTE_LAYER_CACHED && (!L.hp || !L.ahnp || (L.h_rows && L.n_res_rows <= 0)))
            return gte::fail(GTE_ERR_INVALID_ARGUMENT, "gcnsage_step: a cached-aggregate layer needs the images of the input and of its aggregate");
        if (L.kind != GTE_LAYER_PLANES && L.kind != GTE_LAYER_DROPOUT && i != 0)
            return gte::fail(GTE_ERR_UNSUPPORTED, "gcnsage_step: a short-input / aggregate-first layer must be layer 0");
        if (!L.gamma || !L.beta || !L.bias) return gte::fail(GTE_ERR_UNSUPPORTED, "gcnsage_step: hidden layers need bias and LayerNorm");
        if (L.ldf != 0 && (L.ldf < L.fout || L.ldf % 4 != 0)) return gte::fail(GTE_ERR_INVALID_ARGUMENT, "gcnsage_step: ldf < fout or not a multiple of 4");
        if (L.kind == GTE_LAYER_SMALLK && ldf(L) != L.fout) return gte::fail(GTE_ERR_UNSUPPORTED, "gcnsage_step: a short-input layer takes unpadded rows");
    }
    if (p.out_gemm && (p.n_classes > 16 || ld_lg(p) != 32 || !p.hp_out || !p.wimg_out_fwd || !p.wimg_out_bwd || !p.dlqp || p.tn != p.logits + 16 ||
                       p.q_out != p.dl + 16))
        return gte::fail(GTE_ERR_INVALID_ARGUMENT, "gcnsage_step: the GEMM output layer needs n_classes <= 16, [n][32] logits / dl buffers and its images");
    if (p.n_nodes == 0) return gte::fail(GTE_ERR_UNSUPPORTED, "gcnsage_step: empty batch");
    if (p.dropout_p != 0.f && p.n_nodes > GTE_DROPOUT_MAX_ROWS)
        return gte::fail(GTE_ERR_UNSUPPORTED, "gcnsage_step: %lld nodes; a dropout plan holds at most 2^30 rows (32-bit row indices and "
                                              "mask row words; no byte bound on its buffers)", (long long)p.n_nodes);
    return GTE_OK;
}

}

extern "C" int gte_gcnsage_step_wide_layers(const gte_step_plan* plan) {
    if (!plan) return gte::fail(GTE_ERR_INVALID_ARGUMENT, "gcnsage_step_wide_layers: null plan");
    const gte_step_plan& p = *plan;
    if (p.n_hidden < 1 || p.n_hidden > 7 || p.n_nodes < 0) return gte::fail(GTE_ERR_INVALID_ARGUMENT, "gcnsage_step_wide_layers: bad plan");
    int mask = 0;
    for (int i = 0; i < p.n_hidden; ++i)
        if (layer_wide(p, i)) mask |= 1 << i;
    return mask;
}

extern "C" int gte_gcnsage_step(const gte_step_plan* plan, int phase, int* adam_fused, void* stream) {
    if (!plan) return gte::fail(GTE_ERR_INVALID_ARGUMENT, "gcnsage_step: null plan");
    const gte_step_plan& p = *plan;
    if (phase < 0 || phase > 2) return gte::fail(GTE_ERR_INVALID_ARGUMENT, "gcnsage_step: phase must be 0, 1 or 2");
    GTE_TRY(check_plan(p));
    if (phase != 2) {
        GTE_TRY(gte_gemm_set_tail_workspace(p.tail_ws, p.tail_ws ? p.tail_ws_bytes : 0));
        int rc = forward(p, stream);
        if (rc == GTE_OK) rc = gte_fold_defer_begin(stream);
        if (rc == GTE_OK) {
            rc = backward_a(p, stream);
            if (rc != GTE_OK) (void)gte_fold_defer_flush();
        }
        if (rc != GTE_OK) { (void)gte_gemm_set_tail_workspace(nullptr, 0); return rc; }
        if (phase == 1) return GTE_OK;
    }
    int rc = backward_b(p, stream);
    if (rc != GTE_OK) { (void)gte_fold_defer_flush(); (void)gte_gemm_set_tail_workspace(nullptr, 0); return rc; }
    rc = flush(p, adam_fused);
    (void)gte_gemm_set_tail_workspace(nullptr, 0);
    return rc;
}

extern "C" int gte_gcnsage_forward(const gte_step_plan* plan, void* stream) {
    if (!plan) return gte::fail(GTE_ERR_INVALID_ARGUMENT, "gcnsage_forward: null plan");
    const gte_step_plan& p = *plan;
    GTE_TRY(check_plan(p));
    if (p.dropout_p != 0.f)
        return gte::fail(GTE_ERR_UNSUPPORTED, "gcnsage_forward: the forward alone is the evaluation forward and applies no dropout; "
                                             "the plan has dropout_p != 0");
    GTE_TRY(gte_gemm_set_tail_workspace(p.tail_ws, p.tail_ws ? p.tail_ws_bytes : 0));
    const int64_t n = p.n_nodes, C = p.n_classes;
    int rc = forward_hidden(p, stream, true);
    if (rc == GTE_OK) rc = forward_out_products(p, stream);
    if (rc == GTE_OK)
        rc = gte_spmm_csr_accumulate(p.indptr, p.indices, p.w_in, p.tn, ld_lg(p), p.logits, ld_lg(p), n, C, GTE_F32, GTE_REDUCE_MEAN, stream);
    (void)gte_gemm_set_tail_workspace(nullptr, 0);
    return rc;
}
```

### gnn-tableextraction_amd/models/engine.py

```python
from __future__ import annotations

import ctypes
import os
from typing import Optional

import numpy as np
import torch

from .. import ops


class TrainStep:
    def __init__(self, model: torch.nn.Module, lr: float = 0.01, weight_decay: float = 5e-4,
                 class_weights: Optional[torch.Tensor] = None, betas=(0.9, 0.999), eps: float = 1e-8,
                 process_group=None, distributed: bool = False):
        self.model = model
        self.lr, self.weight_decay, self.betas, self.eps = lr, weight_decay, betas, eps
        self.class_weights = class_weights
        self.distributed = distributed
        self.group = process_group
        params = [p for p in model.parameters() if p.requires_grad]
        dev = params[0].device
        total = sum(p.numel() for p in params)
        self.flat_param = torch.empty(total, dtype=torch.float32, device=dev)
# ... 126 lines not shown
        self.fwd_events = None
        self._fwd_ev_arr = None
        if self.dropout_p > 0 and self._plan_kinds(model.layers[0].in_feats, 0) is None:
            raise ValueError(f"FusedGcnSageStep: dropout {self.dropout_p} runs on the one-call plan, which does not cover this model / "
                             "configuration; use TrainStep")

    def _alloc(self, cap: int, f0: int):
        dev = self.flat_param.device
        new = lambda *s: torch.empty(*s, dtype=torch.float32, device=dev)
        layers = self.model.layers
        dims = [f0] + [l.out_feats for l in layers]
        tf = [self._transform_first(l, dims[i]) for i, l in enumerate(layers)]
        qf = [self._qform(i, l, dims[i]) for i, l in enumerate(layers)]
        b = {"cap": cap,
             "ahn": [None if tf[i] else new(cap, dims[i]) for i in range(len(layers))],
             "t": [new(cap, 2 * dims[i + 1]) if tf[i] else None for i in range(len(layers))],
             "z": [new(cap, dims[i + 1]) if (isinstance(l.lynorm, nn.LayerNorm) and not tf[i]) else None
                   for i, l in enumerate(layers)],
             "stats": [new(2 * cap) if isinstance(l.lynorm, nn.LayerNorm) else None for l in layers],
             "y": [new(cap, dims[i + 1]) for i in range(len(layers))],
             "dy": [new(cap, dims[i + 1]) for i in range(len(layers))],
             "dahn": new(cap, max([dims[i] for i in range(1, len(layers)) if not qf[i] and not self._narrow(layers[i], dims[i])]
                                  + [1])),
             "tn": new(cap, dims[-1]), "q": new(cap, dims[-1]),
             "out3": new(3)}
        lib = self.lib
        pl = [self._planes_layer(i, l, dims[i]) for i, l in enumerate(layers)]
        b["pl"] = pl
        b["hp"] = [ops.P3.empty(cap, dims[i], dev) if pl[i] else None for i in range(len(layers))]
        b["dzp"] = [ops.P3.empty(cap, dims[i + 1], dev) if pl[i] else None for i in range(len(layers))]
        b["qp"] = [ops.P3.empty(cap, dims[i + 1], dev) if pl[i] else None for i in range(len(layers))]
        b["ws_p3"] = [torch.empty(int(lib.gte_gemm_p3_tn_workspace_bytes(dims[i + 1], 2 * dims[i], dims[i], cap)), dtype=torch.uint8,
                                  device=dev) if pl[i] else None for i in range(len(layers))]
        for i in range(len(layers)):
            if pl[i] and b["t"][i] is None:
                b["t"][i] = new(cap, 2 * dims[i + 1])
        ws = max([lib.gte_weighted_ce_workspace_bytes(cap)] +
                 [lib.gte_ln_relu_bwd_workspace_bytes(cap, d) for d in dims[1:]] +
                 [lib.gte_gemm_workspace_bytes(dims[i + 1], dims[i], cap) for i in range(len(layers))] +
                 [lib.gte_sage_narrow_bwd_workspace_bytes(cap, min(dims[-2], 256), min(dims[-1], 16))])
        b["ws"] = torch.empty(int(ws), dtype=torch.uint8, device=dev)
        b["ws_ln"] = [torch.empty(int(max(lib.gte_ln_relu_bwd_workspace_bytes(cap, dims[i + 1]),
                                          lib.gte_gemm_p3_nt_ln_bwd_workspace_bytes(cap, dims[i + 1]),
                                          lib.gte_sage_narrow_bwd_ln_workspace_bytes(cap, min(dims[i + 1], 256)))),
                                  dtype=torch.uint8, device=dev) for i in range(len(layers))]
        b["ce_part"] = torch.empty(int(lib.gte_head_agg_ce_workspace_bytes(cap)), dtype=torch.uint8, device=dev)
        b["ws_nar"] = torch.empty(int(lib.gte_sage_narrow_bwd_workspace_bytes(cap, min(dims[-2], 256), min(dims[-1], 16))),
                                  dtype=torch.uint8, device=dev)
        b["ws_dw"] = [torch.empty(int(self._ws_dw_bytes(i, dims, cap)), dtype=torch.uint8, device=dev) for i in range(len(layers))]
        return b

    def _ws_dw_bytes(self, i: int, dims, cap: int) -> int:
        lib = self.lib
        need = [lib.gte_sage_linear_dw_workspace_bytes(dims[i + 1], dims[i], dims[i], cap),
                lib.gte_sage_qform_dw_workspace_bytes(dims[i + 1], dims[i], cap)]
        if i == 0 and lib.gte_sage_smallk_bwd_supported(2 * dims[0], dims[1]):
            need.append(lib.gte_sage_smallk_bwd_workspace_bytes(cap, 2 * dims[0], dims[1]))
        if i == 0 and len(dims) > 2 and lib.gte_gemm_p3_nt_smallk_bwd_supported(2 * dims[0], dims[1]):
            need.append(lib.gte_gemm_p3_nt_smallk_bwd_workspace_bytes(cap, 2 * dims[0], dims[1]))
        return max(need)

    def _alloc_plan(self, cap: int, f0: int, kinds, out_gemm: bool):
        dev, lib = self.flat_param.device, self.lib
        layers = list(self.model.layers)
        dims = [f0] + [l.out_feats for l in layers]
        nh = len(layers) - 1
        ld = [_c16(d) for d in dims[1:nh + 1]]
        z32 = lambda *s: torch.zeros(*s, dtype=torch.float32, device=dev)
        u8 = lambda nbytes: torch.empty(int(nbytes), dtype=torch.uint8, device=dev)

        def img(rows, cols):
            t = ops.P3.empty(rows, cols, dev)
            t.data.zero_()
            return t
        b = {"cap": cap, "ld": ld}
        b["t"] = [z32(cap, 2 * ld[i]) if kinds[i] == LAYER_PLANES else z32(cap, ld[i]) for i in range(nh)]
        b["y"] = [z32(cap, ld[i]) for i in range(nh)]
        b["dy"] = [z32(cap, ld[i]) for i in range(nh)]
        b["stats"] = [z32(2 * cap) for _ in range(nh)]
        b["ahn"] = [z32(cap, dims[0]) if kinds[i] == LAYER_SMALLK else None for i in range(nh)]
        b["ahnp"] = [img(cap, dims[i]) if kinds[i] in (LAYER_AGGFIRST, LAYER_DROPOUT) else None for i in range(nh)]
        b["g"] = [z32(cap, 2 * _c16(dims[i])) if (kinds[i] == LAYER_DROPOUT and i > 0) else None for i in range(nh)]
        b["hp"] = [img(cap, dims[i]) if kinds[i] not in (LAYER_SMALLK, LAYER_CACHED) else None for i in range(nh)]
        b["dzp"] = [img(cap, dims[i + 1]) if kinds[i] != LAYER_SMALLK else None for i in range(nh)]
        b["qp"] = [img(cap, dims[i + 1]) if kinds[i] == LAYER_PLANES else None for i in range(nh)]
        b["ws_dw"] = [u8(lib.gte_gemm_p3_tn_workspace_bytes(dims[i + 1], 2 * dims[i], dims[i], cap) if kinds[i] != LAYER_SMALLK
                         else self._ws_dw_bytes(i, dims, cap)) for i in range(nh)]
        b["ws_ln"] = [u8(max(lib.gte_ln_relu_bwd_workspace_bytes(cap, dims[i + 1]),
                             lib.gte_gemm_p3_nt_ln_bwd_workspace_bytes(cap, dims[i + 1]) if dims[i + 1] <= 256 else 0,
                             lib.gte_sage_narrow_bwd_ln_workspace_bytes(cap, min(_c16(dims[i + 1]), 256)))) for i in range(nh)]
        C = dims[-1]
        b["out3"] = z32(3)
        if out_gemm:
            b["hp_out"] = img(cap, dims[-2])
            b["t_out"], b["dlq"] = z32(cap, 32), z32(cap, 32)
            b["dlqp"] = img(cap + 8, 32)
            b["ws_out"] = u8(lib.gte_gemm_p3_tn_workspace_bytes(C, 2 * dims[-2], dims[-2], cap))
            b["ws_ce"] = u8(max(lib.gte_weighted_ce_workspace_bytes(cap), lib.gte_head_agg_ce_workspace_bytes(cap)))
            b["ws_cs"] = u8(max(lib.gte_colsum_workspace_bytes(cap, C), lib.gte_head_dlq_finish_workspace_bytes(cap)))
        else:
            b["logits"], b["tn"], b["q"], b["dl"] = z32(cap, C), z32(cap, C), z32(cap, C), z32(cap, C)
            b["ce_part"] = u8(lib.gte_head_agg_ce_workspace_bytes(cap))
            b["ws_nar"] = u8(lib.gte_sage_narrow_bwd_workspace_bytes(cap, min(_c16(dims[-2]), 256), min(C, 16)))
        return b

    def _private_set(self, key, n: int, alloc):
        k2 = (self._private_key, key)
        full = self._graph_bufs.get(k2)
        if full is None:
            full = self._graph_bufs[k2] = alloc(n)
        if full["cap"] < n:
            raise RuntimeError(f"captured batch buffers hold {full['cap']} nodes; asked for {n} (a captured batch must not change)")
        return full

    @staticmethod
    def _plan_key(f0: int, kinds, out_gemm: bool):
        return ("gen", f0, tuple(kinds), bool(out_gemm))

    def _buffers_plan(self, n: int, f0: int, kinds, out_gemm: bool):
        key = self._plan_key(f0, kinds, out_gemm)
        if self._private_key is not None:
            return self._private_set(key, n, lambda m: self._alloc_plan(m, f0, kinds, out_gemm))
        full = self._bufs.get(key)
        if full is None or full["cap"] < n:
            cap = max(-(-int(n * 1.125) // 4096) * 4096, getattr(self, "_reserved", {}).get(f0, 0))
            self._bufs.pop(key, None)
            full = self._bufs[key] = self._alloc_plan(cap, f0, kinds, out_gemm)
        return full

    def plan_buffers(self, batch, private_key=None):
        xp = getattr(batch, "feat_p3", None)
        n, f0 = (xp.rows, xp.cols) if xp is not None else batch.ndata['feat'].shape
        kinds = self._plan_kinds(f0, n, self._batch_cached(batch))
        if kinds is None:
            return None
        out_gemm = self._plan_mode(kinds, f0)[1]
        key = self._plan_key(f0, kinds, out_gemm)
        full = self._bufs.get(key) if private_key is None else self._graph_bufs.get((private_key, key))
        return None if full is None else (full, kinds, out_gemm)

    def _buffers(self, n: int, f0: int):
        key = (f0, self._planes_on())
        if self._private_key is not None:
            full = self._private_set(key, n, lambda m: self._alloc(m, f0))
        else:
            full = self._bufs.get(key)
            if full is None or full["cap"] < n:
                cap = max(-(-int(n * 1.125) // 4096) * 4096, getattr(self, "_reserved", {}).get(f0, 0))
                self._bufs = {k: v for k, v in self._bufs.items() if k[0] != f0}
                full = self._bufs[key] = self._alloc(cap, f0)
        v = lambda t: None if t is None else t[:n]
        return {"ahn": [v(t) for t in full["ahn"]], "t": [v(t) for t in full["t"]], "z": [v(t) for t in full["z"]],
                "stats": [None if t is None else t[:2 * n] for t in full["stats"]], "y": [v(t) for t in full["y"]],
                "dy": [v(t) for t in full["dy"]], "dahn": v(full["dahn"]), "tn": v(full["tn"]), "q": v(full["q"]),
                "out3": full["out3"], "ws": full["ws"], "ws_ln": full["ws_ln"], "ws_nar": full["ws_nar"],
                "ce_part": full["ce_part"],
                "ws_dw": full["ws_dw"], "pl": full["pl"], "ws_p3": full["ws_p3"], "_full": full,
                "hp": [None if t is None else t.view_rows(n) for t in full["hp"]],
                "dzp": [None if t is None else t.view_rows(n) for t in full["dzp"]],
                "qp": [None if t is None else t.view_rows(n) for t in full["qp"]]}

    def reserve(self, n_nodes: int, f0: int, cached: bool = False) -> None:
        cap = -(-int(n_nodes) // 4096) * 4096
        if not hasattr(self, "_reserved"):
            self._reserved = {}
        self._reserved[f0] = max(self._reserved.get(f0, 0), cap)
        if self._plan_kinds(f0, 0, cached) is not None:
# ... 77 lines not shown
        st = _lib.current_stream()
        for k in range(0, len(descs), 16):
            chunk = descs[k:k + 16]
            arr = (_lib.P3Desc * len(chunk))(*chunk)
            _lib.check(self.lib.gte_p3_from_f32_batch(ctypes.addressof(arr), len(chunk), st), "gte_p3_from_f32_batch")

    def _smallk_bwd(self, i: int, layer, fin: int) -> bool:
        return (i == 0 and isinstance(layer.lynorm, nn.LayerNorm) and layer.linear.bias is not None
                and not self._transform_first(layer, fin) and not self._planes_layer(i, layer, fin, 1 << 20)
                and bool(self.lib.gte_sage_linear_fwd_fuses_ln(2 * fin, layer.out_feats))
                and bool(self.lib.gte_sage_smallk_bwd_supported(2 * fin, layer.out_feats)))

    def _cached_layer0(self, L, fin: int) -> bool:
        return (self.cache_input_agg and self.general_planes and self._planes_on() and isinstance(L.lynorm, nn.LayerNorm)
                and L.linear.bias is not None and (L.activation is None or _is_relu(L.activation))
                and 128 <= L.out_feats <= 1024)

    def wants_agg_image(self, f0: int, train: bool = True) -> bool:
        L = self.model.layers[0]
        if train and self.dropout_p > 0:
            return False
        return (len(self.model.layers) >= 2 and self._cached_layer0(L, f0)
                and self._layer_kind(0, L, f0, train=train) in (LAYER_PLANES, LAYER_AGGFIRST))

    def wants_resident_images(self, f0: int, train: bool = True) -> bool:
        if train and self.dropout_p > 0:
            return self._layer_kind(0, self.model.layers[0], f0) == LAYER_DROPOUT
        return self.wants_p3_features(f0, train) or self.wants_agg_image(f0, train)

    def _layer_kind(self, i: int, L, fin: int, n: int = 0, cached: bool = False, train: bool = True):
        fout = L.out_feats
        if train and self.dropout_p > 0:
            ok = (isinstance(L.lynorm, nn.LayerNorm) and L.linear.bias is not None and (L.activation is None or _is_relu(L.activation))
                  and self.general_planes and fout <= 1024)
            return LAYER_DROPOUT if ok else None
        if not (self._planes_on() and isinstance(L.lynorm, nn.LayerNorm) and L.linear.bias is not None
                and (L.activation is None or _is_relu(L.activation))):
            return None
        up = LAYER_CACHED if (i == 0 and cached and self._cached_layer0(L, fin)) else LAYER_PLANES
        if self._planes_layer(i, L, fin, n):
            return up
        if (i == 0 and not self._transform_first(L, fin) and fout % 16 == 0
                and bool(self.lib.gte_sage_linear_fwd_fuses_ln(2 * fin, fout)) and not ops.use_tiled(n, fin, None)):
            return LAYER_SMALLK
        if not self.general_planes or fout > 1024:
            return None
        return up if (i > 0 or 4 * fout <= 5 * fin) else (LAYER_CACHED if up == LAYER_CACHED else LAYER_AGGFIRST)

    def _plan_kinds(self, f0: int, n: int, cached: bool = False, train: bool = True):
        layers = list(self.model.layers)
        drop = train and self.dropout_p > 0
        if (not self.use_c_step or not (drop or self._planes_on()) or len(layers) < 2 or len(layers) > 8 or ops._timers is not None):
            return None
        dims = [f0] + [l.out_feats for l in layers]
        last = len(layers) - 1
        Lo = layers[last]
        if (isinstance(Lo.lynorm, nn.LayerNorm) or Lo.activation is not None or Lo.linear.bias is None or Lo.use_pp
                or not 1 <= Lo.out_feats <= 16 or not self.fused_head):
            return None
        if not self.general_planes and not (self._narrow(Lo, dims[last]) and self._fused_head(last, Lo, dims[last])):
            return None
        kinds = []
        for i, L in enumerate(layers[:-1]):
            k = self._layer_kind(i, L, dims[i], n, cached, train)
            if k is None:
                return None
            if k not in (LAYER_SMALLK, LAYER_DROPOUT) and (n + 256) * 2 * _c16(L.out_feats) * 4 >= (1 << 31):
                return None
            kinds.append(k)
        if drop and n > DROPOUT_MAX_ROWS:
            return None
        return kinds

    def wide_layers(self, g) -> int:
        xp = getattr(g, "feat_p3", None)
        n, f0 = (xp.rows, xp.cols) if xp is not None else g.ndata['feat'].shape
        kinds = self._plan_kinds(f0, n, self._batch_cached(g))
        if kinds is None or self.dropout_p == 0:
            return 0
        plan = self._bind_plan(g, kinds, with_adam=bool(self._fuse_adam_req))[0]
        rc = int(self.lib.gte_gcnsage_step_wide_layers(ctypes.addressof(plan)))
        if rc < 0:
            _lib.check(rc, "gte_gcnsage_step_wide_layers")
        return rc

    def attach_feature_image(self, g) -> bool:
        if getattr(g, "feat_p3", None) is not None:
            return True
        x = g.ndata.get('feat')
        if x is None or not x.is_cuda or not self.wants_resident_images(x.shape[1]):
            return False
        x = ops._row_major(x.to(torch.float32))
        g.feat_p3 = ops.p3_from_f32(x)
        if self.wants_agg_image(x.shape[1]):
            csr = g.in_csr()
            g.agg_p3 = ops.spmm_csr_p3(csr.indptr, csr.indices, g.in_weights(g.edata.get("feat")), x, x.shape[0], mean=True)
        return True

    @staticmethod
    def _batch_cached(g) -> bool:
        xp, ap = getattr(g, "feat_p3", None), getattr(g, "agg_p3", None)
        return xp is not None and ap is not None and (xp.row_map is None) == (ap.row_map is None)

    def _plan_mode(self, kinds, f0: int):
        layers = list(self.model.layers)
        dims = [f0] + [l.out_feats for l in layers]
        last = len(layers) - 1
        out_gemm = not (self._narrow(layers[last], dims[last]) and
                        (self._fused_head(last, layers[last], dims[last]) or self._narrow_padded(layers[last], dims[last])))
        gen = out_gemm or any(k in (LAYER_AGGFIRST, LAYER_CACHED, LAYER_DROPOUT)
                              or (k == LAYER_PLANES and not self._planes_layer(i, layers[i], dims[i])) for i, k in enumerate(kinds))
        return gen, out_gemm

    def _weight_images_gen(self, dims, kinds, out_gemm: bool):
        key = self._plan_key(dims[0], kinds, out_gemm)
        hit = self._wimg.get(key)
        if hit is not None:
            return hit
        dev = self.flat_param.device
        layers = list(self.model.layers)

        def img(rows, cols):
            t = ops.P3.empty(rows, cols, dev, block_major=self.block_major_weights)
            t.data.zero_()
            return t
        imgs, descs = {}, []
        for i, k in enumerate(kinds):
            L = layers[i]
            fin, fout = dims[i], L.out_feats
            W = L.linear.weight
            wp, ldw = W.data_ptr(), W.stride(0)
            if k == LAYER_PLANES:
                ld = _c16(fout)
                fwd = img(2 * ld, fin)
                descs.append(_lib.P3Desc(wp, ldw, fout, fin, 0, fwd.at(0, 0), fwd.ldp))
                descs.append(_lib.P3Desc(wp + 4 * fin, ldw, fout, fin, 0, fwd.at(ld, 0), fwd.ldp))
                bwd = None
                if i > 0:
                    bwd = img(fin, 2 * ld)
                    descs.append(_lib.P3Desc(wp, ldw, fin, fout, 1, bwd.at(0, 0), bwd.ldp))
                    descs.append(_lib.P3Desc(wp + 4 * fin, ldw, fin, fout, 1, bwd.at(0, ld // 16), bwd.ldp))
                imgs[i] = (fwd, bwd)
            elif k in (LAYER_AGGFIRST, LAYER_CACHED, LAYER_DROPOUT):
                kp = _c16(fin)
                fwd = img(fout, 2 * kp)
                descs.append(_lib.P3Desc(wp, ldw, fout, fin, 0, fwd.at(0, 0), fwd.ldp))
                descs.append(_lib.P3Desc(wp + 4 * fin, ldw, fout, fin, 0, fwd.at(0, kp // 16), fwd.ldp))
                bwd = None
                if k == LAYER_DROPOUT and i > 0:
                    bwd = img(2 * kp, fout)
                    descs.append(_lib.P3Desc(wp, ldw, fin, fout, 1, bwd.at(0, 0), bwd.ldp))
                    descs.append(_lib.P3Desc(wp + 4 * fin, ldw, fin, fout, 1, bwd.at(kp, 0), bwd.ldp))
                imgs[i] = (fwd, bwd)
        if out_gemm:
            Lo = layers[-1]
            H, C = dims[-2], Lo.out_feats
            W = Lo.linear.weight
            wp, ldw = W.data_ptr(), W.stride(0)
            fwd, bwd = img(32, H), img(H, 32)
            descs.append(_lib.P3Desc(wp, ldw, C, H, 0, fwd.at(0, 0), fwd.ldp))
            descs.append(_lib.P3Desc(wp + 4 * H, ldw, C, H, 0, fwd.at(16, 0), fwd.ldp))
            descs.append(_lib.P3Desc(wp, ldw, H, C, 1, bwd.at(0, 0), bwd.ldp))
            descs.append(_lib.P3Desc(wp + 4 * H, ldw, H, C, 1, bwd.at(0, 1), bwd.ldp))
            imgs["out"] = (fwd, bwd)
        if len(descs) > 32:
            raise _lib.GteError("gte_gcnsage_step: more than 32 weight images")
# ... 22 lines not shown
        cached = plans.get(with_adam)
        if cached is None:
            imgs, arr, n_desc = self._weight_images_gen(dims, kinds, out_gemm)
            plan = _lib.StepPlan()
            plan.n_hidden = nh
            gs = self._gslice
            for i, L in enumerate(layers[:-1]):
                sl = plan.layer[i]
                fin, fout = dims[i], L.out_feats
                sl.kind, sl.fin, sl.fout, sl.ldf = kinds[i], fin, fout, b["ld"][i]
                sl.W, sl.bias, sl.gamma, sl.beta = P(L.linear.weight), P(L.linear.bias), P(L.lynorm.weight), P(L.lynorm.bias)
                sl.eps, sl.relu = float(L.lynorm.eps), int(L.activation is not None)
                sl.gW, sl.gbias = P(gs[id(L.linear.weight)]), P(gs[id(L.linear.bias)])
                sl.ggamma, sl.gbeta = P(gs[id(L.lynorm.weight)]), P(gs[id(L.lynorm.bias)])
                last_hidden = i == nh - 1
                nxt_img = (not last_hidden and kinds[i + 1] == LAYER_PLANES) or (last_hidden and out_gemm)
                if nxt_img:
                    yp = b["hp_out"] if last_hidden else b["hp"][i + 1]
                    sl.yp, sl.ldp_y = P(yp.data), yp.ldp
                sl.y = P(b["y"][i]) if (last_hidden and not out_gemm) or not nxt_img else None
                sl.t, sl.stats, sl.dy = P(b["t"][i]), P(b["stats"][i]), P(b["dy"][i])
                sl.ws_ln, sl.ws_ln_bytes = P(b["ws_ln"][i]), b["ws_ln"][i].numel()
                sl.ws_dw, sl.ws_dw_bytes = P(b["ws_dw"][i]), b["ws_dw"][i].numel()
                if kinds[i] == LAYER_SMALLK:
                    sl.ahn = P(b["ahn"][i])
                    continue
                wf, wb = imgs[i]
                sl.wimg_fwd, sl.ldp_wfwd = P(wf.data), wf.ldp
                if wb is not None:
                    sl.wimg_bwd, sl.ldp_wbwd = P(wb.data), wb.ldp
                sl.dzp, sl.ldp_o = P(b["dzp"][i].data), b["dzp"][i].ldp
                if kinds[i] == LAYER_CACHED:
                    continue
                sl.hp, sl.ldp_h = P(b["hp"][i].data), b["hp"][i].ldp
                if kinds[i] == LAYER_DROPOUT:
                    sl.ahnp, sl.ldp_ahn = P(b["ahnp"][i].data), b["ahnp"][i].ldp
                    if i > 0:
                        sl.x, sl.ldx = P(b["y"][i - 1]), b["ld"][i - 1]
                        sl.g, sl.ldg = P(b["g"][i]), b["g"][i].shape[1]
                    continue
                if kinds[i] == LAYER_PLANES:
                    sl.qp = P(b["qp"][i].data)
                else:
                    sl.ahnp, sl.ldp_ahn = P(b["ahnp"][i].data), b["ahnp"][i].ldp
            Lo = layers[-1]
            C = Lo.out_feats
            plan.out_fin, plan.n_classes = dims[-2], C
            plan.W_out, plan.b_out = P(Lo.linear.weight), P(Lo.linear.bias)
            plan.gW_out, plan.gb_out = P(gs[id(Lo.linear.weight)]), P(gs[id(Lo.linear.bias)])
            plan.ld_h_out = b["ld"][-1]
            plan.dh_out = P(b["dy"][-1])
            if out_gemm:
                wf, wb = imgs["out"]
                plan.out_gemm, plan.ld_lg = 1, 32
                plan.hp_out, plan.ldp_hout = P(b["hp_out"].data), b["hp_out"].ldp
                plan.wimg_out_fwd, plan.ldp_wout_fwd = P(wf.data), wf.ldp
                plan.wimg_out_bwd, plan.ldp_wout_bwd = P(wb.data), wb.ldp
                plan.logits, plan.tn = P(b["t_out"]), P(b["t_out"]) + 64
                plan.dl, plan.q_out = P(b["dlq"]), P(b["dlq"]) + 64
                plan.dlqp, plan.ldp_dlq = P(b["dlqp"].data), b["dlqp"].ldp
                plan.ws_out, plan.ws_out_bytes = P(b["ws_out"]), b["ws_out"].numel()
                plan.ws_ce, plan.ws_ce_bytes = P(b["ws_ce"]), b["ws_ce"].numel()
                plan.ws_cs, plan.ws_cs_bytes = P(b["ws_cs"]), b["ws_cs"].numel()
            else:
                plan.h_out = P(b["y"][-1])
                plan.logits, plan.tn, plan.q_out, plan.dl = P(b["logits"]), P(b["tn"]), P(b["q"]), P(b["dl"])
                plan.ce_part, plan.ce_part_bytes = P(b["ce_part"]), b["ce_part"].numel()
                plan.ws_nar, plan.ws_nar_bytes = P(b["ws_nar"]), b["ws_nar"].numel()
            plan.out3 = P(b["out3"])
            plan.wimg_descs, plan.n_wimg_descs = ctypes.addressof(arr), n_desc
            if with_adam:
                plan.param, plan.grad, plan.exp_avg, plan.exp_avg_sq = (P(self.flat_param), P(self.flat_grad), P(self.exp_avg),
                                                                        P(self.exp_avg_sq))
                plan.n_param = self.flat_param.numel()
                plan.hyper, plan.step_counter, plan.ticket = P(self._hyper), P(self._step_dev), P(self._ticket)
            if self._tail_ws is None:
                self._tail_ws = torch.empty(int(lib.gte_gemm_tail_workspace_bytes()), dtype=torch.uint8, device=self.flat_param.device)
            if self.tail_split:
                plan.tail_ws, plan.tail_ws_bytes = P(self._tail_ws), self._tail_ws.numel()
            cached = plans[with_adam] = (plan, arr, ctypes.c_int(0))
        plan, _arr, fused = cached
        plan.class_weights = P(self.class_weights)
        plan.fuse_ln_dx = (int(self.fuse_ln_dx) | (2 if self.fuse_ln_narrow else 0) | (8 if self.fuse_smallk_dx else 0)
                           | (4 if self.fuse_head_gemm else 0) | (16 if self.fuse_ln_fwd else 0))
        L0 = plan.layer[0]
        if kinds[0] == LAYER_DROPOUT:
            if xp is not None:
                L0.xp, L0.ldp_x, L0.x, L0.ldx = P(xp.data), xp.ldp, None, 0
                L0.h_rows, L0.n_res_rows = (P(xp.row_map), xp.res_rows) if xp.row_map is not None else (None, 0)
            else:
                L0.xp, L0.ldp_x, L0.h_rows, L0.n_res_rows = None, 0, None, 0
                L0.x, L0.ldx = P(x), ops._ld(x)
            self._adam_state()
            plan.dropout_p, plan.dropout_seed, plan.rank = float(self.dropout_p), self.dropout_seed, self.rank
            plan.step_counter = P(self._step_dev)
        elif kinds[0] == LAYER_CACHED:
            ap = getattr(g, "agg_p3", None)
            if xp is None or ap is None:
                raise _lib.GteError("a cached-aggregate input layer needs feat_p3 and agg_p3 (resident images behind a row map, or the graph's own)")
            L0.hp, L0.ldp_h, L0.make_hp, L0.x = P(xp.data), xp.ldp, 0, None
            L0.ahnp, L0.ldp_ahn = P(ap.data), ap.ldp
            L0.h_rows, L0.n_res_rows = (P(xp.row_map), xp.res_rows) if xp.row_map is not None else (None, 0)
        elif kinds[0] == LAYER_PLANES:
            if xp is not None:
                L0.hp, L0.ldp_h, L0.make_hp, L0.x = P(xp.data), xp.ldp, 0, None
                L0.h_rows, L0.n_res_rows = (P(xp.row_map), xp.res_rows) if xp.row_map is not None else (None, 0)
            else:
                L0.hp, L0.ldp_h, L0.make_hp = P(b["hp"][0].data), b["hp"][0].ldp, 1
                L0.h_rows, L0.n_res_rows = None, 0
                L0.x, L0.ldx = P(x), ops._ld(x)
        else:
            if x is None:
                if 'feat' not in g.ndata:
                    g.ndata['feat'] = ops.p3_to_f32(xp)
                x = ops._row_major(g.ndata['feat'])
            L0.x, L0.ldx = P(x), ops._ld(x)
        plan.indptr, plan.indices, plan.w_in = P(csr.indptr), P(csr.indices), P(w_in)
        plan.rindptr, plan.rindices, plan.w_out = P(rcsr.indptr), P(rcsr.indices), P(w_out)
        plan.n_nodes = n
        C = layers[-1].out_feats
        view = {"out3": b["out3"], "_wkey": self._plan_key(f0, kinds, out_gemm),
                "logits": b["t_out"][:n, :C] if out_gemm else b["logits"][:n]}
        return plan, fused, view, n, (csr, rcsr, w_in, w_out, self.class_weights)

    def _c_step(self, g, labels, grad_scale, kinds, with_adam: bool):
        lib, P = self.lib, _lib.ptr
        st = _lib.current_stream()
        plan, fused, b, n, keep = self._bind_plan(g, kinds, with_adam)
        _arr = plan.wimg_descs
        lab = labels if labels.dtype in (torch.float32, torch.int64) else labels.to(torch.int64)
        plan.labels, plan.labels_f32 = P(lab), int(lab.dtype == torch.float32)
        plan.grad_scale = float(grad_scale)
        if self.fwd_events:
            for e in self.fwd_events:
                if not e.cuda_event:
                    e.record()
            self._fwd_ev_arr = (ctypes.c_void_p * len(self.fwd_events))(*[e.cuda_event for e in self.fwd_events])
            plan.fwd_events = ctypes.addressof(self._fwd_ev_arr)
        else:
            plan.fwd_events = None
        capturing = torch.cuda.is_current_stream_capturing()
        sig = self._param_sig()
        sig = (sig, b["_wkey"])
        plan.wimg_fresh = int(self.wimg_in_fold and not capturing and self._wimg_sig == sig)
        plan.wimg_in_fold = int(self.wimg_in_fold and with_adam and not capturing)
        self._wimg_sig = None
        addr = ctypes.addressof(plan)
        if self.before_last_gemm is not None:
            _lib.check(lib.gte_gcnsage_step(addr, 1, ctypes.byref(fused), st), "gte_gcnsage_step")
            try:
                self.before_last_gemm()
                _lib.check(lib.gte_gcnsage_step(addr, 2, ctypes.byref(fused), st), "gte_gcnsage_step")
            except BaseException:
                lib.gte_fold_defer_flush()
                lib.gte_gemm_set_tail_workspace(None, 0)
                self._wimg_sig = None
                raise
        else:
            _lib.check(lib.gte_gcnsage_step(addr, 0, ctypes.byref(fused), st), "gte_gcnsage_step")
        self._adam_fused = bool(fused.value & 1)
        if not capturing and ((fused.value & 2) or not with_adam):
            self._wimg_sig = sig
        self._keep = (lab,) + tuple(keep)
        self._last_wimg = ((plan.wimg_descs, int(plan.n_wimg_descs), b["_wkey"], _arr, dict(self._wimg))
                           if not capturing and not (fused.value & 1) else None)
        return b["out3"]

# ... 568 lines not shown
```

### include/gte.h

```cpp
#ifndef GTE_H_
#define GTE_H_

#include <stdint.h>

#ifdef __cplusplus
extern "C" {
#endif

#define GTE_VERSION 400

enum gte_status {
    GTE_OK = 0,
    GTE_ERR_INVALID_ARGUMENT = -1,
    GTE_ERR_LAUNCH = -2,
    GTE_ERR_WORKSPACE_TOO_SMALL = -3,
    GTE_ERR_UNSUPPORTED = -4,
};

enum gte_reduce { GTE_REDUCE_SUM = 0, GTE_REDUCE_MEAN = 1 };
enum gte_dtype { GTE_F32 = 0, GTE_BF16 = 1 };

int gte_version(void);
const char* gte_last_error(void);
int gte_device_info(int* compute_units, int* wave_size, int* lds_bytes, char* arch_name, int arch_name_len);
// ... 73 lines not shown
int gte_sage_linear_fwd(const float* a1, int64_t lda1, int64_t k1,
                        const float* a2, int64_t lda2, int64_t k2,
                        const float* W, int64_t ldw, const float* bias,
                        const float* gamma, const float* beta, float eps, int relu,
                        float* z_save, int64_t ldz, float* stats,
                        float* y, int64_t ldy, int64_t M, int64_t n_out, void* stream);
int gte_sage_linear_fwd_fuses_ln(int64_t k_total, int64_t n_out);

int64_t gte_sage_linear_dw_workspace_bytes(int64_t n_out, int64_t k1, int64_t k2, int64_t n_nodes);
int gte_sage_linear_dw(const float* dz, int64_t lddz, const float* x1, int64_t ldx1, int64_t k1,
                       const float* x2, int64_t ldx2, int64_t k2, float* dW, int64_t lddw,
                       int64_t n_out, int64_t n_nodes, void* workspace, int64_t workspace_bytes, void* stream);

int gte_spmm_csr_accumulate_ln_supported(int64_t n_feat);
int gte_spmm_csr_accumulate_ln(const int32_t* indptr, const int32_t* indices, const float* eweight, const float* x,
                               int64_t ldx, float* z, int64_t ldz, int64_t n_rows, int64_t n_feat, int reduce,
                               const float* gamma, const float* beta, float eps, int relu, float* y, int64_t ldy,
                               float* stats, void* stream);

int64_t gte_gemm_tail_workspace_bytes(void);
int gte_gemm_set_tail_workspace(void* workspace, int64_t workspace_bytes);

#define GTE_GEMM_F32 0
#define GTE_GEMM_SPLIT_BF16 1
int gte_gemm_set_mode(int mode);
int gte_gemm_get_mode(void);
int gte_gemm_set_thread_mode(int mode);

int64_t gte_p3_row_bytes(int64_t cols);
int gte_p3_from_f32(const float* src, int64_t ld, int64_t rows, int64_t cols, int transpose, void* dst, int64_t ldp,
                    void* stream);
int gte_p3_to_f32(const void* src, int64_t ldp, int64_t rows, int64_t cols, float* dst, int64_t ld, void* stream);
typedef struct gte_p3_desc {
    const float* src; int64_t ld;
    int64_t rows, cols;
    int transpose;
    void* dst; int64_t ldp;
} gte_p3_desc;
int gte_p3_from_f32_batch(const gte_p3_desc* descs, int n, void* stream);
int gte_sage_linear_fwd_p3(const float* a1, int64_t lda1, int64_t k1, const float* a2, int64_t lda2, int64_t k2, const float* W,
                           int64_t ldw, const float* bias, const float* gamma, const float* beta, float eps, int relu,
                           float* z_save, int64_t ldz, float* stats, float* y , int64_t ldy, void* yp3,
                           int64_t ldyp3, int64_t M, int64_t n_out, void* stream);
int gte_sage_smallk_bwd_supported(int64_t k_total, int64_t n_out);
int64_t gte_sage_smallk_bwd_workspace_bytes(int64_t n_nodes, int64_t k_total, int64_t n_out);
int gte_sage_smallk_bwd(const float* dy, int64_t lddy, const float* a1, int64_t lda1, int64_t k1, const float* a2, int64_t lda2,
                        int64_t k2, const float* W, int64_t ldw, const float* bias, const float* gamma, const float* beta,
                        const float* stats, int relu, float* dW, int64_t lddw, float* dbias, float* dgamma, float* dbeta,
                        int64_t n_nodes, int64_t n_out, void* workspace, int64_t workspace_bytes, void* stream);
int gte_spmm_csr_p3(const int32_t* indptr, const int32_t* indices, const float* eweight, const float* x, int64_t ldx,
                    void* outp3, int64_t ldp, int64_t n_rows, int64_t n_feat, int reduce, void* stream);
int gte_spmm_csr_accumulate_ln_p3(const int32_t* indptr, const int32_t* indices, const float* eweight, const float* x,
                                  int64_t ldx, float* z, int64_t ldz, int64_t n_rows, int64_t n_feat, int reduce,
                                  const float* gamma, const float* beta, float eps, int relu, float* y, int64_t ldy,
                                  void* yp3, int64_t ldyp3, float* stats, void* stream);
int gte_ln_relu_bwd_p3(const float* dy, int64_t lddy, const float* z, int64_t ldz, const float* stats, const float* gamma,
                       const float* beta, int relu, float* dz, int64_t lddz, void* dzp3, int64_t ldp3, float* dgamma,
                       float* dbeta, float* dbias, int64_t M, int64_t n_out, void* workspace, int64_t workspace_bytes,
                       void* stream);
int gte_gemm_p3_nt(const void* a1, int64_t ldpa1, int64_t k1, const void* a2, int64_t ldpa2, int64_t k2, const void* b,
                   int64_t ldpb, const float* bias, int64_t bias_cols, float* c, int64_t ldc, int64_t m, int64_t n, int relu,
                   int accumulate, void* stream);
int gte_gemm_p3_nt_rows(const void* a_res, int64_t ldpa, int64_t k, const int32_t* a_rows, int64_t n_res_rows, const void* b,
                        int64_t ldpb, const float* bias, int64_t bias_cols, float* c, int64_t ldc, int64_t m, int64_t n,
                        int relu, int accumulate, void* stream);
int gte_gemm_p3_nt_rows2(const void* a_res, int64_t ldpa, const void* a2_res, int64_t ldpa2, int64_t k, const int32_t* a_rows,
                         int64_t n_res_rows, const void* b, int64_t ldpb, const float* bias, int64_t bias_cols, float* c, int64_t ldc,
                         int64_t m, int64_t n, int relu, int accumulate, void* stream);
int gte_gemm_p3_nt_ln_fwd_supported(int64_t n);
int gte_gemm_p3_nt_ln_fwd(const void* a1, int64_t ldpa1, int64_t k1, const void* a2, int64_t ldpa2, int64_t k2, const void* b,
                          int64_t ldpb, const float* bias, const float* gamma, const float* beta, float eps, int relu, float* z,
                          int64_t ldz, float* y, int64_t ldy, void* yp3, int64_t ldyp3, float* stats, int64_t m, int64_t n,
                          void* stream);
int gte_gemm_p3_nt_rows2_ln_fwd(const void* a_res, int64_t ldpa, const void* a2_res, int64_t ldpa2, int64_t k, const int32_t* a_rows,
                                int64_t n_res_rows, const void* b, int64_t ldpb, const float* bias, const float* gamma,
                                const float* beta, float eps, int relu, float* z, int64_t ldz, float* y, int64_t ldy, void* yp3,
                                int64_t ldyp3, float* stats, int64_t m, int64_t n, void* stream);
int gte_gemm_p3_nt_ln_bwd_supported(int64_t n);
int64_t gte_gemm_p3_nt_ln_bwd_workspace_bytes(int64_t m, int64_t n);
int gte_gemm_p3_nt_ln_bwd(const void* a1, int64_t ldpa1, int64_t k1, const void* a2, int64_t ldpa2, int64_t k2, const void* b,
                          int64_t ldpb, const float* z, int64_t ldz, const float* stats, const float* gamma, const float* beta,
                          int relu, float* dz, int64_t lddz, void* dzp3, int64_t ldp3, float* dgamma, float* dbeta, float* dbias,
                          int64_t m, int64_t n, void* workspace, int64_t workspace_bytes, void* stream);
int gte_gemm_p3_nt_smallk_bwd_supported(int64_t k_total, int64_t n);
int64_t gte_gemm_p3_nt_smallk_bwd_workspace_bytes(int64_t m, int64_t k_total, int64_t n);
int gte_gemm_p3_nt_smallk_bwd(const void* a1, int64_t ldpa1, int64_t kg1, const void* a2, int64_t ldpa2, int64_t kg2, const void* b,
                              int64_t ldpb, const float* x, int64_t ldx, int64_t k1, const float* ahn, int64_t ldahn, int64_t k2,
                              const float* W, int64_t ldw, const float* bias, const float* gamma, const float* beta,
                              const float* stats, int relu, float* dW, int64_t lddw, float* dbias, float* dgamma, float* dbeta,
                              int64_t m, int64_t n, void* workspace, int64_t workspace_bytes, void* stream);
int64_t gte_gemm_p3_tn_workspace_bytes(int64_t m, int64_t n, int64_t nseg, int64_t k);
int gte_gemm_p3_tn(const void* a, int64_t ldpa, const void* a2, int64_t ldpa2, const void* b, int64_t ldpb, const void* b2,
                   int64_t ldpb2, int64_t nseg, float* c, int64_t ldc, int64_t m, int64_t n, int64_t k, void* workspace,
                   int64_t workspace_bytes, void* stream);

int gte_gemm_p3_tn_rows(const void* a, int64_t ldpa, const void* a2, int64_t ldpa2, const void* b_res, int64_t ldpb,
                        const int32_t* b_rows, int64_t n_res_rows, int64_t nseg, float* c, int64_t ldc, int64_t m, int64_t n,
                        int64_t k, void* workspace, int64_t workspace_bytes, void* stream);
int gte_gemm_p3_tn_rows2(const void* a, int64_t ldpa, const void* b_res, int64_t ldpb, const void* b2_res, int64_t ldpb2,
                         const int32_t* b_rows, int64_t n_res_rows, int64_t nseg, float* c, int64_t ldc, int64_t m, int64_t n,
                         int64_t k, void* workspace, int64_t workspace_bytes, void* stream);
int64_t gte_head_dlq_finish_workspace_bytes(int64_t n_nodes);
int gte_head_dlq_finish(const int32_t* rindptr, const int32_t* rindices, const float* w_out, const float* dlq, int64_t lddlq,
                        int64_t n_nodes, int64_t n_classes, const void* ce_partial, float grad_scale, float* out3, void* dlqp3,
                        int64_t ldp, float* gbias, void* workspace, int64_t workspace_bytes, void* stream);
int gte_gemm_p3_nt_plan(int64_t m, int64_t n, int64_t k1, int64_t k2, int weights_block_major, int epilogue, int cus, int* row_tile);
int gte_gemm_p3_set_nt_cfg(int cfg);
int gte_gemm_p3_set_ln_rows(int rows);
int gte_gemm_p3_set_rows64(int mode);
int gte_batch_assemble_rows(const int32_t* pages, int64_t n_batch, const int32_t* node_off, const int32_t* b_node_off,
                            const gte_batch_arrays* in_edges, const gte_batch_arrays* out_edges, const float* feat,
                            int64_t ld_feat, int64_t n_cols, float* feat_out, const float* label, float* label_out,
                            int64_t n_out, int32_t* row_map, int64_t row_map_pad, int64_t n_res_rows, void* stream);

int gte_dropout_mask(float p, uint64_t seed, int rank, int64_t step, int site, int64_t n_rows, int64_t n_cols, uint8_t* mask,
                     int64_t ldm, void* stream);
int gte_dropout_mask_host(float p, uint64_t seed, int rank, int64_t step, int site, int64_t n_rows, int64_t n_cols, uint8_t* mask,
                          int64_t ldm);
#define GTE_DROPOUT_MAX_ROWS ((int64_t)1 << 30)
int gte_dropout_set_wide(int mode);
int gte_dropout_get_wide(void);
int gte_spmm_dropout_p3(const int32_t* indptr, const int32_t* indices, const float* eweight, const float* x, int64_t ldx,
                        const void* xp, int64_t ldpx, const int32_t* x_rows, int64_t n_res_rows, int in_dropout, float p, uint64_t seed,
                        int rank, const int64_t* step_counter, int site, void* selfp3, int64_t ldp_self, void* aggp3, int64_t ldp_agg,
                        int64_t n_rows, int64_t n_feat, void* stream);
int gte_spmm_dropout_bwd(const int32_t* rindptr, const int32_t* rindices, const float* w_out, const float* g, int64_t ldg,
                         int64_t agg_col, float p, uint64_t seed, int rank, const int64_t* step_counter, int site, float* dx,
                         int64_t lddx, int64_t n_rows, int64_t n_feat, void* stream);

enum gte_layer_kind { GTE_LAYER_PLANES = 0, GTE_LAYER_SMALLK = 1, GTE_LAYER_AGGFIRST = 2, GTE_LAYER_CACHED = 3, GTE_LAYER_DROPOUT = 4 };
typedef struct gte_step_layer {
    int kind;
    int64_t fin, fout;
    const float* W; const float* bias; const float* gamma; const float* beta; float eps; int relu;
    float* gW; float* gbias; float* ggamma; float* gbeta;
    void* wimg_fwd; int64_t ldp_wfwd;
    void* wimg_bwd; int64_t ldp_wbwd;
    const float* x; int64_t ldx;
    void* hp; int64_t ldp_h;
    const int32_t* h_rows; int64_t n_res_rows;
    int make_hp;
    float* ahn;
    float* t;
    float* stats;
    float* y;
    void* yp; int64_t ldp_y;
    float* dy;
    void* dzp; void* qp; int64_t ldp_o;
    void* ws_ln; int64_t ws_ln_bytes;
    void* ws_dw; int64_t ws_dw_bytes;
    int64_t ldf;
    void* ahnp; int64_t ldp_ahn;
    const void* xp; int64_t ldp_x;
    float* g; int64_t ldg;
} gte_step_layer;
typedef struct gte_step_plan {
    int n_hidden;
    gte_step_layer layer[7];
    int64_t out_fin, n_classes;
    const float* W_out; const float* b_out; float* gW_out; float* gb_out;
    const float* h_out; int64_t ld_h_out;
    float* logits; float* tn; float* q_out; float* dl; float* dh_out;
    void* ce_part; int64_t ce_part_bytes; void* ws_nar; int64_t ws_nar_bytes;
    const int32_t* indptr; const int32_t* indices; const float* w_in;
    const int32_t* rindptr; const int32_t* rindices; const float* w_out;
    int64_t n_nodes;
    const void* labels; int labels_f32; const float* class_weights; float grad_scale; float* out3;
    const void* wimg_descs; int n_wimg_descs;
    float* param; float* grad; float* exp_avg; float* exp_avg_sq; int64_t n_param;
    float* hyper; int64_t* step_counter; uint32_t* ticket;
    void* tail_ws; int64_t tail_ws_bytes;
    int fuse_ln_dx;
    int wimg_fresh;
    int wimg_in_fold;
    int out_gemm; int64_t ld_lg;
    void* hp_out; int64_t ldp_hout;
    void* wimg_out_fwd; int64_t ldp_wout_fwd;
    void* wimg_out_bwd; int64_t ldp_wout_bwd;
    void* dlqp; int64_t ldp_dlq;
    void* ws_out; int64_t ws_out_bytes;
    void* ws_ce; int64_t ws_ce_bytes;
    void* ws_cs; int64_t ws_cs_bytes;
    void* const* fwd_events;
    float dropout_p; uint64_t dropout_seed; int rank;
} gte_step_plan;
int gte_gcnsage_step_wide_layers(const gte_step_plan* plan);
int gte_gcnsage_step(const gte_step_plan* plan, int phase, int* adam_fused, void* stream);
int gte_gcnsage_forward(const gte_step_plan* plan, void* stream);

int gte_fold_defer_begin(void* stream);
int gte_fold_defer_flush(void);
int gte_fold_defer_flush_adam(float* param, float* grad, float* exp_avg, float* exp_avg_sq, int64_t n, float* state,
                              int64_t* step_counter, unsigned* ticket, int* fused);
int gte_fold_defer_flush_adam_images(float* param, float* grad, float* exp_avg, float* exp_avg_sq, int64_t n, float* state,
                                     int64_t* step_counter, unsigned* ticket, const gte_p3_desc* images, int n_images, int* fused);

int gte_sage_transform_fwd(const float* x, int64_t ldx, int64_t n_feat, const float* W, int64_t ldw, const float* bias,
                           int64_t n_out, float* t, int64_t ldt, int64_t n_nodes, void* stream);
int64_t gte_sage_qform_dw_workspace_bytes(int64_t n_out, int64_t n_feat, int64_t n_nodes);
int gte_sage_qform_dw(const float* dz, int64_t lddz, const float* q, int64_t ldq, const float* x, int64_t ldx,
                      int64_t n_feat, float* dW, int64_t lddw, int64_t n_out, int64_t n_nodes, void* workspace,
                      int64_t workspace_bytes, void* stream);
int gte_sage_qform_dx(const float* dz, int64_t lddz, const float* q, int64_t ldq, const float* W, int64_t ldw,
                      int64_t n_feat, int64_t n_out, float* dx, int64_t lddx, int64_t n_nodes, void* stream);

int gte_sage_narrow_supported(int64_t n_feat, int64_t n_out);
int gte_sage_narrow_fwd(const float* h, int64_t ldh, int64_t n_feat, const float* W, int64_t ldw, const float* bias,
                        int64_t n_out, float* t_self, int64_t ld_self, float* t_neigh, int64_t ld_neigh,
                        int64_t n_nodes, void* stream);
int gte_sage_narrow_fwd_ln_supported(int64_t n_feat, int64_t n_out);
int gte_sage_narrow_fwd_ln(const float* z, int64_t ldz, int64_t n_feat, const float* gamma, const float* beta, float eps,
                           int relu, float* y, int64_t ldy, float* stats, const float* W, int64_t ldw, const float* bias,
                           int64_t n_out, float* t_self, int64_t ld_self, float* t_neigh, int64_t ld_neigh, int64_t n_nodes,
                           void* stream);
int64_t gte_sage_narrow_bwd_workspace_bytes(int64_t n_nodes, int64_t n_feat, int64_t n_out);
int gte_sage_narrow_bwd(const float* dl, int64_t lddl, const float* q, int64_t ldq, const float* h, int64_t ldh,
                        int64_t n_feat, const float* W, int64_t ldw, int64_t n_out, float* dh, int64_t lddh,
                        float* dW, int64_t lddw, float* dbias, int64_t n_nodes,
                        void* workspace, int64_t workspace_bytes, void* stream);

int gte_head_supported(int64_t n_feat, int64_t n_classes);
int64_t gte_head_agg_ce_workspace_bytes(int64_t n_nodes);
int gte_head_agg_ce(const int32_t* indptr, const int32_t* indices, const float* eweight, const float* t_neigh,
                    int64_t ld_neigh, float* logits, int64_t ld_logits, const void* labels, int labels_f32,
                    const float* class_weight, int64_t n_nodes, int64_t n_classes, int reduce, float* dl_unscaled,
                    int64_t lddl, void* ce_partial, int64_t ce_partial_bytes, void* stream);
int gte_sage_narrow_bwd_ce(const float* dl_unscaled, int64_t lddl, const float* q_unscaled, int64_t ldq, const float* h,
                           int64_t ldh, int64_t n_feat, const float* W, int64_t ldw, int64_t n_out, float* dh,
                           int64_t lddh, float* dW, int64_t lddw, float* dbias, int64_t n_nodes, void* workspace,
                           int64_t workspace_bytes, const void* ce_partial, float grad_scale, float* out3, void* stream);

int64_t gte_sage_narrow_bwd_ln_workspace_bytes(int64_t n_nodes, int64_t n_feat);
int gte_sage_narrow_bwd_ln_p3(const float* dl, int64_t lddl, const float* q, int64_t ldq, const float* h, int64_t ldh,
                              int64_t n_feat, const float* W, int64_t ldw, int64_t n_out, float* dz_below, int64_t lddz,
                              void* dzp3, int64_t ldp3, float* dW, int64_t lddw, float* dbias, int64_t n_nodes, void* workspace,
                              int64_t workspace_bytes, const void* ce_partial, float grad_scale, float* out3,
                              const float* z_below, int64_t ldz, const float* stats_below, const float* gamma_below,
                              const float* beta_below, int relu_below, float* dgamma_below, float* dbeta_below,
                              float* dbias_below, void* ln_workspace, int64_t ln_workspace_bytes, void* stream);
int gte_sage_narrow_pad_supported(int64_t n_feat, int64_t n_pad, int64_t n_out);
int gte_sage_narrow_fwd_pad(const float* h, int64_t ldh, int64_t n_feat, int64_t n_pad, const float* W, int64_t ldw, const float* bias,
                            int64_t n_out, float* t_self, int64_t ld_self, float* t_neigh, int64_t ld_neigh, int64_t n_nodes,
                            void* stream);
int gte_sage_narrow_bwd_ln_p3_pad(const float* dl, int64_t lddl, const float* q, int64_t ldq, const float* h, int64_t ldh,
                                  int64_t n_feat, int64_t n_pad, const float* W, int64_t ldw, int64_t n_out, float* dz_below,
                                  int64_t lddz, void* dzp3, int64_t ldp3, float* dW, int64_t lddw, float* dbias, int64_t n_nodes,
                                  void* workspace, int64_t workspace_bytes, const void* ce_partial, float grad_scale, float* out3,
                                  const float* z_below, int64_t ldz, const float* stats_below, const float* gamma_below,
                                  const float* beta_below, int relu_below, float* dgamma_below, float* dbeta_below,
                                  float* dbias_below, void* ln_workspace, int64_t ln_workspace_bytes, void* stream);

int gte_ln_relu_fwd(const float* z, int64_t ldz, const float* gamma, const float* beta, float eps, int relu,
                    float* y, int64_t ldy, float* stats, int64_t M, int64_t n_out, void* stream);

int gte_ln_relu_fwd_p3(const float* z, int64_t ldz, const float* gamma, const float* beta, float eps, int relu, float* y,
                       int64_t ldy, void* yp3, int64_t ldyp3, float* stats, int64_t M, int64_t n_out, void* stream);

int64_t gte_ln_relu_bwd_workspace_bytes(int64_t M, int64_t n_out);
int gte_ln_relu_bwd(const float* dy, int64_t lddy, const float* z, int64_t ldz, const float* stats,
                    const float* gamma, const float* beta, int relu,
                    float* dz, int64_t lddz, float* dgamma, float* dbeta, float* dbias,
                    int64_t M, int64_t n_out, void* workspace, int64_t workspace_bytes, void* stream);

int64_t gte_gemm_workspace_bytes(int64_t M, int64_t N, int64_t K);
int gte_gemm_f32(int trans_a, int trans_b, int64_t M, int64_t N, int64_t K,
                 const float* A, int64_t lda, const float* B, int64_t ldb,
                 float* C, int64_t ldc, int accumulate,
                 void* workspace, int64_t workspace_bytes, void* stream);

// ... 53 lines not shown
```

Measured before the change: 49.37 million.

## Emit layer-0 dz in k-block-major transposed image for the weight-gradient GEMM

The fused LN-backward GEMM can now write layer 0's dz as a transposed, 16-row block-major bf16x3 image. A new transposed-A variant of the row-mapped TN GEMM reads that image directly into registers with buffer loads and stages only B through LDS. The goal is to cut LDS traffic and stage size for the layer-0 weight-gradient GEMM. In exchange it adds a transpose epilogue with an extra barrier, pads the dz buffer, and routes through new hand-scheduled asm with tight waitcnt assumptions.

```diff
diff --git a/gnn-tableextraction_amd/_lib.py b/gnn-tableextraction_amd/_lib.py
--- a/gnn-tableextraction_amd/_lib.py
+++ b/gnn-tableextraction_amd/_lib.py
@@ -98,6 +98,9 @@
     "gte_gemm_p3_nt_ln_bwd": (c_int, [c_void_p, c_int64, c_int64, c_void_p, c_int64, c_int64, c_void_p, c_int64, c_void_p, c_int64,
                                       c_void_p, c_void_p, c_void_p, c_int, c_void_p, c_int64, c_void_p, c_int64, c_void_p, c_void_p,
                                       c_void_p, c_int64, c_int64, c_void_p, c_int64, c_void_p]),
+    "gte_gemm_p3_nt_ln_bwd_t": (c_int, [c_void_p, c_int64, c_int64, c_void_p, c_int64, c_int64, c_void_p, c_int64, c_void_p, c_int64,
+                                        c_void_p, c_void_p, c_void_p, c_int, c_void_p, c_int64, c_void_p, c_int64, c_void_p, c_int64,
+                                        c_void_p, c_void_p, c_void_p, c_int64, c_int64, c_void_p, c_int64, c_void_p]),
     "gte_gemm_p3_nt_smallk_bwd_supported": (c_int, [c_int64, c_int64]),
     "gte_gemm_p3_nt_smallk_bwd_workspace_bytes": (c_int64, [c_int64, c_int64, c_int64]),
     "gte_gemm_p3_nt_smallk_bwd": (c_int, [c_void_p, c_int64, c_int64, c_void_p, c_int64, c_int64, c_void_p, c_int64, c_void_p, c_int64,
@@ -112,6 +115,9 @@
                                      c_int64, c_void_p, c_int64, c_int64, c_int64, c_int, c_int, c_void_p]),
     "gte_gemm_p3_tn_rows2": (c_int, [c_void_p, c_int64, c_void_p, c_int64, c_void_p, c_int64, c_void_p, c_int64, c_int64, c_void_p,
                                      c_int64, c_int64, c_int64, c_int64, c_void_p, c_int64, c_void_p]),
+    "gte_gemm_p3_tn_rows2_t": (c_int, [c_void_p, c_int64, c_void_p, c_int64, c_void_p, c_int64, c_void_p, c_int64, c_int64, c_void_p,
+                                       c_int64, c_int64, c_int64, c_int64, c_void_p, c_int64, c_void_p]),
+    "gte_gemm_p3_tn_plan": (c_int, [c_int64, c_int64, c_int64, c_int64, c_void_p]),
     "gte_gemm_p3_nt_ln_fwd_supported": (c_int, [c_int64]),
     "gte_gemm_p3_nt_ln_fwd": (c_int, [c_void_p, c_int64, c_int64, c_void_p, c_int64, c_int64, c_void_p, c_int64, c_void_p, c_void_p,
                                       c_void_p, c_float, c_int, c_void_p, c_int64, c_void_p, c_int64, c_void_p, c_int64, c_void_p,
@@ -133,6 +139,8 @@
     "gte_adam_ticket_bytes": (c_int64, []),
     "gte_gcnsage_step": (c_int, [c_void_p, c_int, POINTER(c_int), c_void_p]),
     "gte_gcnsage_step_wide_layers": (c_int, [c_void_p]),
+    "gte_gcnsage_step_dzt_layers": (c_int, [c_void_p]),
+    "gte_gcnsage_step_set_dzt": (c_int, [c_int]),
     "gte_gcnsage_forward": (c_int, [c_void_p, c_void_p]),
     "gte_fold_defer_begin": (c_int, [c_void_p]),
     "gte_fold_defer_flush": (c_int, []),
diff --git a/gnn-tableextraction_amd/csrc/gemm_p3.hip b/gnn-tableextraction_amd/csrc/gemm_p3.hip
--- a/gnn-tableextraction_amd/csrc/gemm_p3.hip
+++ b/gnn-tableextraction_amd/csrc/gemm_p3.hip
@@ -36,6 +36,7 @@
     const float* bias; int bias_cols;
     int relu, accumulate;
     int splits, stages_per_split;
+    int a_t;
     float* slab;
     const int* rowsA; const int* rowsB; long long res_bytes;
     int rows64;
@@ -43,6 +44,7 @@
     int wide_c;
     const float* ln_z; long long ln_ldz; const float* ln_stats; const float* ln_gamma; const float* ln_beta; int ln_relu;
     float* ln_dz; long long ln_lddz; char* ln_dzp3; long long ln_ldp3; float* ln_part;
+    char* ln_dzt3; long long ln_bst3;
     float* lnf_y; long long lnf_ldy; char* lnf_yp3; long long lnf_ldp; float* lnf_stats; float lnf_eps;
     const float* sk_x; long long sk_ldx; int sk_k1; const float* sk_ahn; long long sk_ldahn; int sk_k2;
     const float* sk_W; long long sk_ldw; const float* sk_bias; float* sk_part_dw;
@@ -676,6 +678,28 @@
                         }
                         if (im8 && rok[odd ? u + 1 : u])
                             p3::store8(p.ln_dzp3 + (long long)(row_base + rl + (odd ? u + 1 : u) * NW) * p.ln_ldp3, col0, x);
+                    }
+                }
+                if (p.ln_dzt3 && okc) {
+#pragma unroll
+                    for (int u = 0; u < RF; ++u)
+                        if (rl + u * NW < SR)
+                            *reinterpret_cast<float4*>(tile + (rl + u * NW) * LDT + j4) = make_float4(dd[u][0], dd[u][1], dd[u][2], dd[u][3]);
+                }
+            }
+            if (p.ln_dzt3) {
+                asm volatile("s_waitcnt lgkmcnt(0)\n\ts_barrier" ::: "memory");
+                const int cg = (n + 63) >> 6;
+                for (int it = wave; it < (SR / 16) * cg; it += NW) {
+                    const int b = it / cg, c = (it - b * cg) * 64 + lane;
+                    const int r0 = row_base + b * 16;
+                    if (r0 < M && c < n) {
+                        float x0[8], x1[8];
+#pragma unroll
+                        for (int r = 0; r < 8; ++r) { x0[r] = tile[(b * 16 + r) * LDT + c]; x1[r] = tile[(b * 16 + 8 + r) * LDT + c]; }
+                        char* dst = p.ln_dzt3 + (long long)(r0 >> 4) * p.ln_bst3 + (long long)c * 96;
+                        p3::store8(dst, 0, x0);
+                        p3::store8(dst, 8, x1);
                     }
                 }
             }
@@ -1030,17 +1054,19 @@
 #ifndef P3_TN_ABL
 #define P3_TN_ABL 0
 #endif
-template <int WM, int WN, int WGS, bool MAP = false, bool BIG = false>
+template <int WM, int WN, int WGS, bool MAP = false, bool BIG = false, bool AT = false>
 __global__ void __launch_bounds__(WM * WN * 64, (WM * WN * WGS + 3) / 4)
 gemm_p3_tn_kernel(const P3Gemm p) {
     static_assert(!BIG || MAP, "64-bit rows: the row-mapped kernel");
+    static_assert(!AT || (MAP && !BIG), "transposed A: the row-mapped kernel on 32-bit offsets");
     static_assert(!MAP || (WM == 2 && WN == 2), "row map: the 128 x 128 tile");
     constexpr int NW = WM * WN, TM = 2, TN = 2;
     constexpr int BM = WM * 64, BN = WN * 64, NBA = BM / 16, NBB = BN / 16;
     constexpr int RSA = NBA * 96, RSB = NBB * 96;
-    constexpr int A_BYTES = 16 * RSA, B_BYTES = 16 * RSB;
+    constexpr int A_BYTES = AT ? 0 : 16 * RSA, B_BYTES = 16 * RSB;
     constexpr int A_INST = A_BYTES / 1024, B_INST = B_BYTES / 1024, N_INST = A_INST + B_INST;
     constexpr int NI = (N_INST + NW - 1) / NW;
+    constexpr int BI = A_INST / NW;
     constexpr int STAGE = NI * NW * 1024;
     static_assert((NBA & (NBA - 1)) == 0 && (NBB & (NBB - 1)) == 0 && NBA >= 8 && NBB >= 8, "blocks per row: a power of two >= 8");
     extern __shared__ __attribute__((aligned(16))) char lds[];
@@ -1085,18 +1111,59 @@
     int rid[3] = {0, 0, 0};
     if constexpr (MAP)
         if (st_begin < st_end) {
-            rid[0] = rmap[st_begin * 16 + kb[3]];
-            rid[1] = rmap[st_begin * 16 + kb[4]];
-            rid[2] = rmap[st_begin * 16 + kb[5]];
-        }
+            rid[0] = rmap[st_begin * 16 + kb[BI + 0]];
+            rid[1] = rmap[st_begin * 16 + kb[BI + 1]];
+            rid[2] = rmap[st_begin * 16 + kb[BI + 2]];
+        }
+    typedef unsigned u32x4 __attribute__((ext_vector_type(4)));
+    const int at_vo = (m0 + wm * TM * 32 + (lane & 31)) * 96 + (lane >> 5) * 16;
+    auto load_a = [&](bf16x8 (&d)[3][TM], int st) {
+        static_assert(TM == 2, "two fragments per plane");
+        const unsigned long long base = reinterpret_cast<unsigned long long>(p.A1) + (unsigned long long)min(st, total_stages - 1) * (unsigned long long)p.bsa1;
+        u32x4 srd;
+        srd.x = (unsigned)base; srd.y = (unsigned)(base >> 32) & 0xffffu; srd.z = st < st_end ? (unsigned)p.M * 96u : 0u; srd.w = SRD_FLAGS;
+        asm volatile("s_nop 4\n\t"
+                     "buffer_load_dwordx4 %0, %6, %7, 0 offen\n\t"
+                     "buffer_load_dwordx4 %1, %6, %7, 0 offen offset:3072\n\t"
+                     "buffer_load_dwordx4 %2, %6, %7, 0 offen offset:64\n\t"
+                     "buffer_load_dwordx4 %3, %6, %7, 0 offen offset:3136\n\t"
+                     "buffer_load_dwordx4 %4, %6, %7, 0 offen offset:32\n\t"
+                     "buffer_load_dwordx4 %5, %6, %7, 0 offen offset:3104"
+                     : "=&v"(d[0][0]), "=&v"(d[0][1]), "=&v"(d[2][0]), "=&v"(d[2][1]), "=&v"(d[1][0]), "=&v"(d[1][1])
+                     : "v"(at_vo), "s"(srd)
+                     : "memory");
+    };
+    auto issue_at = [&](int st, char* buf, bf16x8 (&anext)[3][TM]) {
+        const int k0 = st * 16;
+        const int live = st < st_end ? 1 : 0;
+        const __amdgpu_buffer_rsrc_t sb = __builtin_amdgcn_make_buffer_rsrc(
+            const_cast<char*>(Bm + cob), 0, (int)(unsigned)max(p.res_bytes - cob, 0ll) * live, SRD_FLAGS);
+        asm volatile("s_waitcnt vmcnt(9)" : "+v"(rid[0]), "+v"(rid[1]), "+v"(rid[2])::"memory");
+        const int o0 = (int)((unsigned)rid[0] * (unsigned)ldb + (unsigned)vc[0]);
+        const int o1 = (int)((unsigned)rid[1] * (unsigned)ldb + (unsigned)vc[1]);
+        const int o2 = (int)((unsigned)rid[2] * (unsigned)ldb + (unsigned)vc[2]);
+        const int kn = st + 1 < st_end ? k0 + 16 : 0;
+        const int* q0 = rmap + kn + kb[0];
+        const int* q1 = rmap + kn + kb[1];
+        const int* q2 = rmap + kn + kb[2];
+        asm volatile("global_load_dword %0, %3, off\n\tglobal_load_dword %1, %4, off\n\tglobal_load_dword %2, %5, off"
+                     : "=&v"(rid[0]), "=&v"(rid[1]), "=&v"(rid[2])
+                     : "v"(q0), "v"(q1), "v"(q2), "v"(o0), "v"(o1), "v"(o2)
+                     : "memory");
+        dma16(sb, buf + (0 * NW + wave) * 1024, o0);
+        dma16(sb, buf + (1 * NW + wave) * 1024, o1);
+        dma16(sb, buf + (2 * NW + wave) * 1024, o2);
+        load_a(anext, st + 1);
+    };
     auto issue = [&](int st, char* buf) {
+        if constexpr (AT) return; else {
         const int k0 = st * 16;
         const int rows = st < st_end ? min(16, p.K - k0) : 0;
         const __amdgpu_buffer_rsrc_t sa =
             __builtin_amdgcn_make_buffer_rsrc(const_cast<char*>(Am + (long long)k0 * lda + coa), 0, max(rows * lda - coa, 0), SRD_FLAGS);
         if constexpr (MAP) {
             {
-                static_assert(!MAP || (A_INST == 12 && NI == 6), "row map: 128 x 128 tile");
+                static_assert(!MAP || AT || (A_INST == 12 && NI == 6), "row map: 128 x 128 tile");
                 const int live = rows > 0 ? 1 : 0;
                 const __amdgpu_buffer_rsrc_t sb = __builtin_amdgcn_make_buffer_rsrc(
                     const_cast<char*>(Bm + cob), 0, (int)(unsigned)max(p.res_bytes - cob, 0ll) * live, SRD_FLAGS);
@@ -1147,6 +1214,7 @@
             constexpr int i = decltype(I)::value;
             dma16(isb[i] ? sb : sa, buf + (i * NW + wave) * 1024, vo[i]);
         });
+        }
     };
 
     const int h = lane >> 5, g = (lane >> 4) & 1, q = (lane >> 2) & 3, pp = lane & 3;
@@ -1230,6 +1298,48 @@
         __builtin_amdgcn_sched_barrier(0);
     };
 
+    auto read_b = [&](F& f, unsigned sbase, auto PB_) {
+        constexpr int pc = decltype(PB_)::value;
+        static_for<TN>([&](auto X) {
+            constexpr int x = decltype(X)::value;
+            const unsigned at = sbase + (unsigned)b_rd[x];
+            s16x4 lo, hi;
+            asm volatile("ds_read_b64_tr_b16 %0, %1 offset:%2" : "=v"(lo) : "v"(at), "n"(pc * 32) : "memory");
+            asm volatile("ds_read_b64_tr_b16 %0, %1 offset:%2" : "=v"(hi) : "v"(at), "n"(pc * 32 + 4 * RSB) : "memory");
+            f.b[pc][x] = __builtin_bit_cast(bf16x8, __builtin_shufflevector(lo, hi, 0, 1, 2, 3, 4, 5, 6, 7));
+        });
+    };
+    auto wait_b = [&](F& f, auto N_, auto PB_) {
+        constexpr int pb = decltype(PB_)::value;
+        if constexpr (decltype(N_)::value == 4) asm volatile("s_waitcnt lgkmcnt(4)" : "+v"(f.b[pb][0]), "+v"(f.b[pb][1])::"memory");
+        else asm volatile("s_waitcnt lgkmcnt(0)" : "+v"(f.b[pb][0]), "+v"(f.b[pb][1])::"memory");
+    };
+    using I4 = std::integral_constant<int, 4>;
+    auto stage_products_at = [&](int slot, bf16x8 (&fa)[3][TM]) {
+        const unsigned sbase = lds_base + (unsigned)slot * STAGE;
+        F f;
+        read_b(f, sbase, I2{});
+        read_b(f, sbase, I0{});
+        asm volatile("s_waitcnt vmcnt(36)" : "+v"(fa[0][0]), "+v"(fa[0][1]), "+v"(fa[1][0]), "+v"(fa[1][1]), "+v"(fa[2][0]), "+v"(fa[2][1])::"memory");
+        static_for<3>([&](auto PC) { f.a[PC.value][0] = fa[PC.value][0]; f.a[PC.value][1] = fa[PC.value][1]; });
+        wait_b(f, I4{}, I2{});
+        __builtin_amdgcn_sched_barrier(0);
+        mfma_pair(f, I0{}, I2{});
+        __builtin_amdgcn_sched_barrier(0);
+        read_b(f, sbase, I1{});
+        wait_b(f, I4{}, I0{});
+        __builtin_amdgcn_sched_barrier(0);
+        mfma_pair(f, I2{}, I0{});
+        __builtin_amdgcn_sched_barrier(0);
+        wait_b(f, I0{}, I1{});
+        __builtin_amdgcn_sched_barrier(0);
+        mfma_pair(f, I1{}, I1{});
+        mfma_pair(f, I0{}, I1{});
+        mfma_pair(f, I1{}, I0{});
+        mfma_pair(f, I0{}, I0{});
+        __builtin_amdgcn_sched_barrier(0);
+    };
+
 #pragma unroll
     for (int a = 0; a < TM; ++a)
 #pragma unroll
@@ -1237,6 +1347,28 @@
 #pragma unroll
             for (int e = 0; e < 16; ++e) acc[a][b][e] = 0.f;
 
+    if constexpr (AT) {
+        static_assert(NI == 3 && STAGE == 12 * 1024, "transposed A: the stage image is B's 12 KB");
+        bf16x8 aq[4][3][TM];
+        load_a(aq[0], st_begin);
+        issue_at(st_begin, lds, aq[1]);
+        issue_at(st_begin + 1, lds + STAGE, aq[2]);
+        wait_dma_barrier<18>();
+        int rd = 0, wr = 2;
+        for (int st = st_begin; st < st_end; st += 4) {
+            static_for<4>([&](auto J) {
+                constexpr int j = decltype(J)::value;
+                if (st + j < st_end) {
+                    issue_at(st + j + 2, lds + wr * STAGE, aq[(j + 3) & 3]);
+                    wr = wr == 2 ? 0 : wr + 1;
+                    stage_products_at(rd, aq[j]);
+                    wait_dma_barrier<18>();
+                    rd = rd == 2 ? 0 : rd + 1;
+                }
+            });
+        }
+        asm volatile("s_waitcnt vmcnt(0)" ::: "memory");
+    } else {
     constexpr int NBUF = 3;
     int next = st_begin, wr = 0;
 #pragma unroll
@@ -1256,6 +1388,7 @@
         stage_products(rd);
         wait_dma_barrier<(NBUF - 2) * NI>();
         rd = rd + 1 == NBUF ? 0 : rd + 1;
+    }
     }
     float* outp = p.splits > 1 ? p.slab + (long long)split * p.M * p.N : p.C;
     const long long ldo = p.splits > 1 ? p.N : p.ldc;
@@ -1666,15 +1799,16 @@
 }
 int gte::gemm_p3_nt_ln_bwd(const P3NtOperands& op, const float* z, int64_t ldz, const float* stats, const float* gamma, const float* beta,
                            int relu, float* dz, int64_t lddz, void* dzp3, int64_t ldp3, float* dgamma, float* dbeta, float* dbias,
-                           int64_t m, int64_t n, void* workspace, int64_t workspace_bytes, void* stream) {
+                           int64_t m, int64_t n, void* workspace, int64_t workspace_bytes, void* stream, void* dzt3, int64_t bst3) {
     const char* name = "gemm_p3_nt_ln_bwd";
     const int64_t n4 = gte::round_up(n, 4);
     NtLimits lim = {};
     lim.max_ld = 1 << 23; lim.below_2gb = true;
     lim.own_sizes = n <= 0 || op.k1 > INT32_MAX || op.k2 > INT32_MAX;
     lim.unsupported = gte_gemm_p3_nt_ln_bwd_supported(n) ? nullptr : "needs n <= 256";
-    lim.own_null = !z || !stats || !gamma || !beta || (!dz && !dzp3) || !workspace;
-    lim.own_ld = ldz < n4 || (dz && lddz < n4) || (dzp3 && (ldp3 < p3::row_bytes(n) || ldp3 % 16 != 0));
+    lim.own_null = !z || !stats || !gamma || !beta || (!dz && !dzp3 && !dzt3) || !workspace;
+    lim.own_ld = ldz < n4 || (dz && lddz < n4) || (dzp3 && (ldp3 < p3::row_bytes(n) || ldp3 % 16 != 0)) ||
+                 (dzt3 && (bst3 < n * 96 || bst3 % 16 != 0 || (reinterpret_cast<uintptr_t>(dzt3) & 15)));
     P3Gemm p = {};
     int rc = nt_prepare(name, op, m, n, lim, p);
     if (rc != GTE_OK || p.M == 0) return rc;
@@ -1683,6 +1817,7 @@
         return gte::fail(GTE_ERR_WORKSPACE_TOO_SMALL, "%s: needs %lld workspace bytes, got %lld", name, (long long)need, (long long)workspace_bytes);
     p.ln_z = z; p.ln_ldz = ldz; p.ln_stats = stats; p.ln_gamma = gamma; p.ln_beta = beta; p.ln_relu = relu;
     p.ln_dz = dz; p.ln_lddz = lddz; p.ln_dzp3 = reinterpret_cast<char*>(dzp3); p.ln_ldp3 = ldp3;
+    p.ln_dzt3 = reinterpret_cast<char*>(dzt3); p.ln_bst3 = bst3;
     p.ln_part = reinterpret_cast<float*>(workspace);
     hipStream_t s = gte::as_stream(stream);
     const NtPick k = nt_pick(p, n % 16 == 0 ? 1 : 3);
@@ -1698,6 +1833,15 @@
                                      void* stream) {
     return gte::gemm_p3_nt_ln_bwd({a1, lda1, k1, a2, lda2, k2, b, ldb, nullptr, 0}, z, ldz, stats, gamma, beta, relu, dz, lddz, dzp3, ldp3,
                                   dgamma, dbeta, dbias, m, n, workspace, workspace_bytes, stream);
+}
+
+extern "C" int gte_gemm_p3_nt_ln_bwd_t(const void* a1, int64_t lda1, int64_t k1, const void* a2, int64_t lda2, int64_t k2, const void* b,
+                                       int64_t ldb, const float* z, int64_t ldz, const float* stats, const float* gamma,
+                                       const float* beta, int relu, float* dz, int64_t lddz, void* dzp3, int64_t ldp3, void* dzt3,
+                                       int64_t bst3, float* dgamma, float* dbeta, float* dbias, int64_t m, int64_t n, void* workspace,
+                                       int64_t workspace_bytes, void* stream) {
+    return gte::gemm_p3_nt_ln_bwd({a1, lda1, k1, a2, lda2, k2, b, ldb, nullptr, 0}, z, ldz, stats, gamma, beta, relu, dz, lddz, dzp3, ldp3,
+                                  dgamma, dbeta, dbias, m, n, workspace, workspace_bytes, stream, dzt3, bst3);
 }
 
 int gte::gemm_p3_nt_ln_fwd(const P3NtOperands& op, const float* bias, const float* gamma, const float* beta, float eps, int relu, float* z,
@@ -1791,6 +1935,13 @@
                                       stats, relu, dW, lddw, dbias, dgamma, dbeta, m, n, workspace, workspace_bytes, stream);
 }
 
+extern "C" int gte_gemm_p3_tn_plan(int64_t m, int64_t n, int64_t nseg, int64_t k, int* stages_per_split) {
+    if (stages_per_split) *stages_per_split = 0;
+    if (m <= 0 || n <= 0 || k < 0 || nseg < 0) return gte::fail(GTE_ERR_INVALID_ARGUMENT, "gemm_p3_tn_plan: bad sizes");
+    const TnPlan pl = tn_plan(m, n, nseg, k);
+    if (stages_per_split) *stages_per_split = pl.stages_per_split;
+    return pl.splits;
+}
 extern "C" int64_t gte_gemm_p3_tn_workspace_bytes(int64_t m, int64_t n, int64_t nseg, int64_t k) {
     if (m <= 0 || n <= 0) return 256;
     const TnPlan pl = tn_plan(m, n, nseg, k);
@@ -1816,10 +1967,13 @@
         return gte::fail(GTE_ERR_INVALID_ARGUMENT, "%s: bad sizes", name);
     if (!o.a || !o.b || !c) return gte::fail(GTE_ERR_INVALID_ARGUMENT, "%s: null pointer", name);
     const int64_t bcols = nseg > 0 ? nseg : n;
-    if (o.lda < p3::row_bytes(m) || o.ldb < p3::row_bytes(bcols) || (o.a2 && o.lda2 < p3::row_bytes(m)) ||
+    const bool a_t = o.a_bs != 0;
+    if (a_t && (o.a_bs < m * 96 || o.a_bs % 16 != 0 || (reinterpret_cast<uintptr_t>(o.a) & 15)))
+        return gte::fail(GTE_ERR_INVALID_ARGUMENT, "%s: block stride of the transposed image too small or image not 16-byte aligned", name);
+    if ((!a_t && o.lda < p3::row_bytes(m)) || o.ldb < p3::row_bytes(bcols) || (o.a2 && o.lda2 < p3::row_bytes(m)) ||
         (o.b2 && o.ldb2 < p3::row_bytes(bcols)) || ldc < n)
         return gte::fail(GTE_ERR_INVALID_ARGUMENT, "%s: leading dimension too small", name);
-    if (o.lda >= (1 << 23) || o.ldb >= (1 << 23) || o.lda2 >= (1 << 23) || o.ldb2 >= (1 << 23) || (m + 128) * n * 4 >= ((int64_t)1 << 31) ||
+    if ((!a_t && o.lda >= (1 << 23)) || o.ldb >= (1 << 23) || o.lda2 >= (1 << 23) || o.ldb2 >= (1 << 23) || (m + 128) * n * 4 >= ((int64_t)1 << 31) ||
         (m + 128) * ldc * 4 >= ((int64_t)1 << 31))
         return gte::fail(GTE_ERR_UNSUPPORTED, "%s: row strides must be < 8 MB and the output < 2 GB", name);
     hipStream_t s = gte::as_stream(stream);
@@ -1840,6 +1994,11 @@
         p.rowsB = o.rows; p.res_bytes = o.n_res_rows * o.ldb;
         p.rows64 = rows64_needed((o.n_res_rows + 1) * o.ldb);
     }
+    if (a_t) {
+        if (!o.rows || p.rows64 || o.a2 || m * 96 >= ((int64_t)1 << 31))
+            return gte::fail(GTE_ERR_UNSUPPORTED, "%s: the transposed image serves the row-mapped product on 32-bit offsets, one a operand", name);
+        p.a_t = 1; p.bsa1 = o.a_bs;
+    }
     if (pl.splits > 1) {
         const int64_t need = (int64_t)pl.splits * m * n * 4;
         if (!workspace || workspace_bytes < need)
@@ -1849,12 +2008,15 @@
     }
     const int64_t tiles = gte::ceil_div(m, 128) * (nseg > 0 ? 2 * gte::ceil_div(nseg, 128) : gte::ceil_div(n, 128));
     constexpr int shm_small = 3 * 6 * 4 * 1024;
-    static bool configured[3] = {};
+    constexpr int shm_at = 3 * 3 * 4 * 1024;
+    static bool configured[4] = {};
     set_lds_once(configured[0], &gemm_p3_tn_kernel<2, 2, 2>, shm_small);
     set_lds_once(configured[1], &gemm_p3_tn_kernel<2, 2, 2, true>, shm_small);
     set_lds_once(configured[2], &gemm_p3_tn_kernel<2, 2, 2, true, true>, shm_small);
+    set_lds_once(configured[3], &gemm_p3_tn_kernel<2, 2, 2, true, false, true>, shm_at);
     const dim3 grid((unsigned)(tiles * pl.splits));
-    if (p.rowsB && p.rows64) hipLaunchKernelGGL((gemm_p3_tn_kernel<2, 2, 2, true, true>), grid, dim3(256), shm_small, s, p);
+    if (p.a_t) hipLaunchKernelGGL((gemm_p3_tn_kernel<2, 2, 2, true, false, true>), grid, dim3(256), shm_at, s, p);
+    else if (p.rowsB && p.rows64) hipLaunchKernelGGL((gemm_p3_tn_kernel<2, 2, 2, true, true>), grid, dim3(256), shm_small, s, p);
     else if (p.rowsB) hipLaunchKernelGGL((gemm_p3_tn_kernel<2, 2, 2, true>), grid, dim3(256), shm_small, s, p);
     else hipLaunchKernelGGL((gemm_p3_tn_kernel<2, 2, 2>), grid, dim3(256), shm_small, s, p);
     int rc = gte::check_launch("gemm_p3_tn");
@@ -1887,3 +2049,13 @@
     return gte::gemm_p3_tn({a, ldpa, nullptr, 0, b_res, ldpb, b2_res, ldpb2, nseg, b_rows, n_res_rows}, c, ldc, m, n, k, workspace,
                            workspace_bytes, stream, "gemm_p3_tn_rows2");
 }
+
+extern "C" int gte_gemm_p3_tn_rows2_t(const void* a_t, int64_t a_bs, const void* b_res, int64_t ldpb, const void* b2_res, int64_t ldpb2,
+                                      const int32_t* b_rows, int64_t n_res_rows, int64_t nseg, float* c, int64_t ldc, int64_t m, int64_t n,
+                                      int64_t k, void* workspace, int64_t workspace_bytes, void* stream) {
+    if (!b_rows || !b2_res || nseg <= 0 || a_bs <= 0)
+        return gte::fail(GTE_ERR_INVALID_ARGUMENT, "gemm_p3_tn_rows2_t: null row map / second image, nseg <= 0 or block stride <= 0");
+    return gte::gemm_p3_tn({a_t, 0, nullptr, 0, b_res, ldpb, b2_res, ldpb2, nseg, b_rows, n_res_rows, a_bs}, c, ldc, m, n, k, workspace,
+                           workspace_bytes, stream, "gemm_p3_tn_rows2_t");
+}
+bool gte::p3_rows64(int64_t res_bytes) { return rows64_needed(res_bytes) != 0; }
diff --git a/gnn-tableextraction_amd/csrc/gemm_p3_host.h b/gnn-tableextraction_amd/csrc/gemm_p3_host.h
--- a/gnn-tableextraction_amd/csrc/gemm_p3_host.h
+++ b/gnn-tableextraction_amd/csrc/gemm_p3_host.h
@@ -14,6 +14,7 @@
     const void* a; int64_t lda; const void* a2; int64_t lda2;
     const void* b; int64_t ldb; const void* b2; int64_t ldb2; int64_t nseg;
     const int32_t* rows; int64_t n_res_rows;
+    int64_t a_bs;
 };
 
 int gemm_p3_nt(const P3NtOperands& op, const float* bias, int64_t bias_cols, float* c, int64_t ldc, int64_t m, int64_t n, int relu,
@@ -23,7 +24,7 @@
                       const char* name = "gemm_p3_nt_ln_fwd");
 int gemm_p3_nt_ln_bwd(const P3NtOperands& op, const float* z, int64_t ldz, const float* stats, const float* gamma, const float* beta,
                       int relu, float* dz, int64_t lddz, void* dzp3, int64_t ldp3, float* dgamma, float* dbeta, float* dbias, int64_t m,
-                      int64_t n, void* workspace, int64_t workspace_bytes, void* stream);
+                      int64_t n, void* workspace, int64_t workspace_bytes, void* stream, void* dzt3 = nullptr, int64_t bst3 = 0);
 int gemm_p3_nt_smallk_bwd(const P3NtOperands& op, const float* x, int64_t ldx, int64_t k1, const float* ahn, int64_t ldahn, int64_t k2,
                           const float* W, int64_t ldw, const float* bias, const float* gamma, const float* beta, const float* stats,
                           int relu, float* dW, int64_t lddw, float* dbias, float* dgamma, float* dbeta, int64_t m, int64_t n,
@@ -31,4 +32,6 @@
 int gemm_p3_tn(const P3TnOperands& op, float* c, int64_t ldc, int64_t m, int64_t n, int64_t k, void* workspace, int64_t workspace_bytes,
                void* stream, const char* name = "gemm_p3_tn");
 
+bool p3_rows64(int64_t res_bytes);
+
 }
diff --git a/gnn-tableextraction_amd/csrc/step.hip b/gnn-tableextraction_amd/csrc/step.hip
--- a/gnn-tableextraction_amd/csrc/step.hip
+++ b/gnn-tableextraction_amd/csrc/step.hip
@@ -44,8 +44,10 @@
     return {L.dzp, L.ldp_o, two ? nullptr : L.qp, two ? 0 : L.ldp_o, L.hp, L.ldp_h, two ? L.ahnp : nullptr, two ? L.ldp_ahn : 0, L.fin,
             rows_of(L), L.n_res_rows};
 }
-inline int layer_dw(const gte_step_layer& L, int64_t n, void* st) {
-    return gte::gemm_p3_tn(dw_operands(L), L.gW, 2 * L.fin, L.fout, 2 * L.fin, n, L.ws_dw, L.ws_dw_bytes, st);
+inline int layer_dw(const gte_step_layer& L, int64_t n, void* st, bool dzt = false) {
+    gte::P3TnOperands op = dw_operands(L);
+    if (dzt) { op.lda = 0; op.a_bs = L.fout * 96; }
+    return gte::gemm_p3_tn(op, L.gW, 2 * L.fin, L.fout, 2 * L.fin, n, L.ws_dw, L.ws_dw_bytes, st);
 }
 
 int forward_hidden(const gte_step_plan& p, void* st, bool fwd_only = false) {
@@ -147,11 +149,28 @@
            gte_gemm_p3_nt_smallk_bwd_supported(2 * B.fin, L.fin) && ldf(B) == B.fout;
 }
 
+inline bool keep_dz0() {
+    static const bool keep = GTE_MEASURE_INT("GTE_STEP_KEEP_DZ0", 0) != 0;
+    return keep;
+}
+inline bool ln_in_dx1(const gte_step_plan& p) {
+    if (p.n_hidden < 2) return false;
+    const gte_step_layer& B = p.layer[0];
+    const gte_step_layer& L = p.layer[1];
+    return L.kind == GTE_LAYER_PLANES && (p.fuse_ln_dx & 1) && B.kind != GTE_LAYER_SMALLK && gte_gemm_p3_nt_ln_bwd_supported(L.fin) &&
+           (L.fin % 16 == 0 || ldf(B) >= ((L.fin + 3) & ~(int64_t)3));
+}
+thread_local int g_dzt_mode = 1;
+bool dzt_layer0(const gte_step_plan& p) {
+    const gte_step_layer& B = p.layer[0];
+    return g_dzt_mode != 0 && (p.fuse_ln_dx & 32) && ln_in_dx1(p) && B.kind == GTE_LAYER_CACHED && B.dzp && !keep_dz0() && B.h_rows &&
+           B.ldp_ahn == B.ldp_h && !gte::p3_rows64((B.n_res_rows + 1) * B.ldp_h) && B.fout * 96 < ((int64_t)1 << 31);
+}
+
 inline const float* z_of(const gte_step_layer& L) { return L.t; }
 inline int64_t ldz_of(const gte_step_layer& L) { return L.kind == GTE_LAYER_PLANES ? 2 * ldf(L) : ldf(L); }
 
 int backward_a(const gte_step_plan& p, void* st) {
-    static const bool keep_dz0 = GTE_MEASURE_INT("GTE_STEP_KEEP_DZ0", 0) != 0;
     const int64_t n = p.n_nodes, C = p.n_classes, lg = ld_lg(p);
     bool ln_done = false, smallk_done = false;
     const gte_step_layer& T = p.layer[p.n_hidden - 1];
@@ -232,9 +251,11 @@
             break;
         } else if ((p.fuse_ln_dx & 1) && B.kind != GTE_LAYER_SMALLK && gte_gemm_p3_nt_ln_bwd_supported(L.fin) &&
                    (L.fin % 16 == 0 || ldf(B) >= ((L.fin + 3) & ~(int64_t)3))) {
-            GTE_TRY(gte_gemm_p3_nt_ln_bwd(L.dzp, L.ldp_o, L.fout, L.qp, L.ldp_o, L.fout, L.wimg_bwd, L.ldp_wbwd, z_of(B), ldz_of(B), B.stats,
-                                          B.gamma, B.beta, B.relu, (B.kind == GTE_LAYER_CACHED && B.dzp && !keep_dz0) ? nullptr : B.dy, ldf(B), B.dzp, B.ldp_o,
-                                          B.ggamma, B.gbeta, B.gbias, n, L.fin, B.ws_ln, B.ws_ln_bytes, st));
+            const bool dzt = i == 1 && dzt_layer0(p);
+            GTE_TRY(gte_gemm_p3_nt_ln_bwd_t(L.dzp, L.ldp_o, L.fout, L.qp, L.ldp_o, L.fout, L.wimg_bwd, L.ldp_wbwd, z_of(B), ldz_of(B), B.stats,
+                                            B.gamma, B.beta, B.relu, (B.kind == GTE_LAYER_CACHED && B.dzp && !keep_dz0()) ? nullptr : B.dy, ldf(B),
+                                            dzt ? nullptr : B.dzp, B.ldp_o, dzt ? B.dzp : nullptr, dzt ? B.fout * 96 : 0, B.ggamma, B.gbeta,
+                                            B.gbias, n, L.fin, B.ws_ln, B.ws_ln_bytes, st));
             ln_done = true;
         } else {
             GTE_TRY(gte_gemm_p3_nt(L.dzp, L.ldp_o, L.fout, L.qp, L.ldp_o, L.fout, L.wimg_bwd, L.ldp_wbwd, nullptr, 0, B.dy, ldf(B), n, L.fin, 0,
@@ -259,7 +280,7 @@
                                    L.relu, L.gW, 2 * L.fin, L.gbias, L.ggamma, L.gbeta, n, L.fout, L.ws_dw, L.ws_dw_bytes, st);
     if (L.kind == GTE_LAYER_SMALLK)
         return gte_sage_linear_dw(L.dy, L.fout, L.x, L.ldx, L.fin, L.ahn, L.fin, L.fin, L.gW, 2 * L.fin, L.fout, n, L.ws_dw, L.ws_dw_bytes, st);
-    return layer_dw(L, n, st);
+    return layer_dw(L, n, st, dzt_layer0(p));
 }
 
 int flush(const gte_step_plan& p, int* adam_fused) {
@@ -326,6 +347,17 @@
     return mask;
 }
 
+extern "C" int gte_gcnsage_step_set_dzt(int mode) {
+    if (mode != 0 && mode != 1) return gte::fail(GTE_ERR_INVALID_ARGUMENT, "gcnsage_step_set_dzt: mode must be 0 (row-major dz0) or 1 (by plan)");
+    g_dzt_mode = mode;
+    return GTE_OK;
+}
+extern "C" int gte_gcnsage_step_dzt_layers(const gte_step_plan* plan) {
+    if (!plan) return gte::fail(GTE_ERR_INVALID_ARGUMENT, "gcnsage_step_dzt_layers: null plan");
+    if (plan->n_hidden < 1 || plan->n_hidden > 7 || plan->n_nodes < 0) return gte::fail(GTE_ERR_INVALID_ARGUMENT, "gcnsage_step_dzt_layers: bad plan");
+    return dzt_layer0(*plan) ? 1 : 0;
+}
+
 extern "C" int gte_gcnsage_step(const gte_step_plan* plan, int phase, int* adam_fused, void* stream) {
     if (!plan) return gte::fail(GTE_ERR_INVALID_ARGUMENT, "gcnsage_step: null plan");
     const gte_step_plan& p = *plan;
diff --git a/gnn-tableextraction_amd/models/engine.py b/gnn-tableextraction_amd/models/engine.py
--- a/gnn-tableextraction_amd/models/engine.py
+++ b/gnn-tableextraction_amd/models/engine.py
@@ -232,7 +232,8 @@
         b["ahnp"] = [img(cap, dims[i]) if kinds[i] in (LAYER_AGGFIRST, LAYER_DROPOUT) else None for i in range(nh)]
         b["g"] = [z32(cap, 2 * _c16(dims[i])) if (kinds[i] == LAYER_DROPOUT and i > 0) else None for i in range(nh)]
         b["hp"] = [img(cap, dims[i]) if kinds[i] not in (LAYER_SMALLK, LAYER_CACHED) else None for i in range(nh)]
-        b["dzp"] = [img(cap, dims[i + 1]) if kinds[i] != LAYER_SMALLK else None for i in range(nh)]
+        b["dzp"] = [img(_c16(cap) if (i == 0 and kinds[i] == LAYER_CACHED) else cap, dims[i + 1]) if kinds[i] != LAYER_SMALLK else None
+                    for i in range(nh)]
         b["qp"] = [img(cap, dims[i + 1]) if kinds[i] == LAYER_PLANES else None for i in range(nh)]
         b["ws_dw"] = [u8(lib.gte_gemm_p3_tn_workspace_bytes(dims[i + 1], 2 * dims[i], dims[i], cap) if kinds[i] != LAYER_SMALLK
                          else self._ws_dw_bytes(i, dims, cap)) for i in range(nh)]
@@ -476,6 +477,18 @@
         rc = int(self.lib.gte_gcnsage_step_wide_layers(ctypes.addressof(plan)))
         if rc < 0:
             _lib.check(rc, "gte_gcnsage_step_wide_layers")
+        return rc
+
+    def dzt_layers(self, g) -> int:
+        xp = getattr(g, "feat_p3", None)
+        n, f0 = (xp.rows, xp.cols) if xp is not None else g.ndata['feat'].shape
+        kinds = self._plan_kinds(f0, n, self._batch_cached(g))
+        if kinds is None:
+            return 0
+        plan = self._bind_plan(g, kinds, with_adam=bool(self._fuse_adam_req))[0]
+        rc = int(self.lib.gte_gcnsage_step_dzt_layers(ctypes.addressof(plan)))
+        if rc < 0:
+            _lib.check(rc, "gte_gcnsage_step_dzt_layers")
         return rc
 
     def attach_feature_image(self, g) -> bool:
@@ -664,7 +677,7 @@
         plan, _arr, fused = cached
         plan.class_weights = P(self.class_weights)
         plan.fuse_ln_dx = (int(self.fuse_ln_dx) | (2 if self.fuse_ln_narrow else 0) | (8 if self.fuse_smallk_dx else 0)
-                           | (4 if self.fuse_head_gemm else 0) | (16 if self.fuse_ln_fwd else 0))
+                           | (4 if self.fuse_head_gemm else 0) | (16 if self.fuse_ln_fwd else 0) | 32)
         L0 = plan.layer[0]
         if kinds[0] == LAYER_DROPOUT:
             if xp is not None:
diff --git a/include/gte.h b/include/gte.h
--- a/include/gte.h
+++ b/include/gte.h
@@ -179,6 +179,10 @@
                           int64_t ldpb, const float* z, int64_t ldz, const float* stats, const float* gamma, const float* beta,
                           int relu, float* dz, int64_t lddz, void* dzp3, int64_t ldp3, float* dgamma, float* dbeta, float* dbias,
                           int64_t m, int64_t n, void* workspace, int64_t workspace_bytes, void* stream);
+int gte_gemm_p3_nt_ln_bwd_t(const void* a1, int64_t ldpa1, int64_t k1, const void* a2, int64_t ldpa2, int64_t k2, const void* b,
+                            int64_t ldpb, const float* z, int64_t ldz, const float* stats, const float* gamma, const float* beta,
+                            int relu, float* dz, int64_t lddz, void* dzp3, int64_t ldp3, void* dzt3, int64_t bst3, float* dgamma,
+                            float* dbeta, float* dbias, int64_t m, int64_t n, void* workspace, int64_t workspace_bytes, void* stream);
 int gte_gemm_p3_nt_smallk_bwd_supported(int64_t k_total, int64_t n);
 int64_t gte_gemm_p3_nt_smallk_bwd_workspace_bytes(int64_t m, int64_t k_total, int64_t n);
 int gte_gemm_p3_nt_smallk_bwd(const void* a1, int64_t ldpa1, int64_t kg1, const void* a2, int64_t ldpa2, int64_t kg2, const void* b,
@@ -197,6 +201,10 @@
 int gte_gemm_p3_tn_rows2(const void* a, int64_t ldpa, const void* b_res, int64_t ldpb, const void* b2_res, int64_t ldpb2,
                          const int32_t* b_rows, int64_t n_res_rows, int64_t nseg, float* c, int64_t ldc, int64_t m, int64_t n,
                          int64_t k, void* workspace, int64_t workspace_bytes, void* stream);
+int gte_gemm_p3_tn_rows2_t(const void* a_t, int64_t a_bs, const void* b_res, int64_t ldpb, const void* b2_res, int64_t ldpb2,
+                           const int32_t* b_rows, int64_t n_res_rows, int64_t nseg, float* c, int64_t ldc, int64_t m, int64_t n,
+                           int64_t k, void* workspace, int64_t workspace_bytes, void* stream);
+int gte_gemm_p3_tn_plan(int64_t m, int64_t n, int64_t nseg, int64_t k, int* stages_per_split);
 int64_t gte_head_dlq_finish_workspace_bytes(int64_t n_nodes);
 int gte_head_dlq_finish(const int32_t* rindptr, const int32_t* rindices, const float* w_out, const float* dlq, int64_t lddlq,
                         int64_t n_nodes, int64_t n_classes, const void* ce_partial, float grad_scale, float* out3, void* dlqp3,
@@ -282,6 +290,8 @@
     float dropout_p; uint64_t dropout_seed; int rank;
 } gte_step_plan;
 int gte_gcnsage_step_wide_layers(const gte_step_plan* plan);
+int gte_gcnsage_step_dzt_layers(const gte_step_plan* plan);
+int gte_gcnsage_step_set_dzt(int mode);
 int gte_gcnsage_step(const gte_step_plan* plan, int phase, int* adam_fused, void* stream);
 int gte_gcnsage_forward(const gte_step_plan* plan, void* stream);
 
```

Result: slower. 46.50 million (-5.8%).
